# Jackz915/PackPPI

Hardware: AMD Instinct MI355X
Metric: sampled residues/sec at 100 diffusion steps (higher is better)
Workload: dtype f32 (dense layers as split-f16: two f16 per operand, three f16 MFMAs per product, fp32 accumulate); 1 GPU; data/T1124_lig.pdb (L=739, 738 true residues), 1 complex per GPU; diffusion_steps=100, proximal=False, residues_per_gpu=738, residues_rank0=738, residues_total=738, mode=ode

## Files before the change

include/packppi_hip.h:

```cpp
#ifndef PACKPPI_HIP_H
#define PACKPPI_HIP_H

#include <stddef.h>
#include <stdint.h>

#ifdef __cplusplus
extern "C" {
#endif

typedef enum pp_status {
    PP_OK = 0,
    PP_ERR_INVALID = 1,
    PP_ERR_HIP = 2,
    PP_ERR_UNSUPPORTED = 3,
    PP_ERR_NO_DEVICE = 4
} pp_status;

typedef struct pp_plan pp_plan;
typedef struct pp_ctx pp_ctx;

#define PP_N_WEIGHTS 1439172u
#define PP_HIDDEN 128
#define PP_TOP_K 32
#define PP_MODE_ODE 0
// ... 50 lines not shown

pp_status pp_topk_aten_host(const float *values, int n, int k, int32_t *idx_out);

pp_status pp_complex_prepare(pp_plan *plan, const pp_batch *batch, void *stream, pp_ctx **ctx);
void pp_ctx_destroy(pp_ctx *ctx);

pp_status pp_complex_prepare_packed(pp_plan *plan, const pp_batch *batch, const int32_t *seg_offsets, int n_seg,
                                    int min_len, int max_len, void *stream, pp_ctx **ctx);

pp_status pp_ctx_get_graph(pp_ctx *ctx, int64_t *E_idx, float *hE0, void *stream);

pp_status pp_ctx_set_graph(pp_ctx *ctx, const int64_t *E_idx, void *stream);

pp_status pp_score(pp_ctx *ctx, const float *chi, float t, float *score, float *hV, void *stream);

pp_status pp_score_rows(pp_ctx *ctx, const float *chi, const float *t_rows, float *score, float *hV, void *stream);

pp_status pp_sample(pp_ctx *ctx, float *chi, const float *schedule, int n_schedule, int mode,
                    const float *sde_noise, void *stream);

pp_status pp_ctx_set_rng_keys(pp_ctx *ctx, const uint64_t *keys, void *stream);

pp_status pp_noise_seeded(pp_ctx *ctx, uint64_t seed, int step, float *noise, uint32_t *words, void *stream);

pp_status pp_add_noise_seeded(pp_ctx *ctx, const float *chi0, float t, uint64_t seed, float *chi, void *stream);

pp_status pp_sample_seeded(pp_ctx *ctx, float *chi, const float *schedule, int n_schedule, int mode, uint64_t seed,
                           void *stream);

#define PP_FIX_HOLD 0
#define PP_FIX_RENOISE 1
pp_status pp_sample_partial(pp_ctx *ctx, float *chi, const float *chi_ref, const uint8_t *fixed, int fix_mode,
                            const float *schedule, int n_schedule, int mode, uint64_t seed,
                            float *chi_traj , void *stream);

pp_status pp_atom14(pp_ctx *ctx, const float *chi, float *xyz, void *stream);

pp_status pp_clash(pp_ctx *ctx, const float *chi, float *per_res, float *dchi, void *stream);

pp_status pp_proximal(pp_ctx *ctx, const float *chi, float lamda, int num_steps, float *chi_traj,
                      float *chi_last, float *losses, void *stream);

pp_status pp_proximal_packed(pp_ctx *ctx, const float *chi, float lamda, int num_steps, const int32_t *norm_rows,
                             float *chi_traj, float *chi_last, float *chi_accepted, float *losses, void *stream);

pp_status pp_proximal_pinned(pp_ctx *ctx, const float *chi, const uint8_t *fixed , float lamda,
                             int num_steps, const int32_t *norm_rows, float *chi_traj, float *chi_last,
                             float *chi_accepted, float *losses, uint8_t *moved , void *stream);

typedef struct pp_affinity pp_affinity;

#define PP_AFF_N_WEIGHTS 101889u
#define PP_AFF_N_WEIGHTS_LINEAR 33153u

pp_status pp_affinity_create(const float *weights, size_t n_weights, int device, pp_affinity **aff);
void pp_affinity_destroy(pp_affinity *aff);

pp_status pp_affinity_encode(const pp_affinity *aff, pp_ctx *ctx, const int64_t *residue_type, const float *sc_sincos,
                             const int64_t *mut_mask, const float *hV_pret, float *hV, void *stream);

pp_status pp_affinity_predict(const pp_affinity *aff, const float *h_wt, const float *h_mt, const int32_t *seg_offsets,
                              int n_seg, int n_rows, float *ddg, float *ddg_inv, void *stream);

pp_status pp_so2_set_grids(const double *x_grid, const double *sigma_grid, int device);
pp_status pp_so2_score(const float *x, const float *sigma, size_t n, int pi_periodic, float *score, int32_t *idx, int device,
                       void *stream);

pp_status pp_dsm_loss(pp_ctx *ctx, const float *pred_score, const float *target_score, const float *t_rows,
                      const double *score_norm, double *num, double *den, void *stream);

pp_status pp_time_kernel(pp_ctx *ctx, int which, int iters, float *avg_ms, void *stream);

pp_status pp_profile_kernel(pp_ctx *ctx, int which);
pp_status pp_profile_read(pp_ctx *ctx, float *total_ms, int *launches);

int pp_edge_variant(void);

int pp_has_range_check(void);
pp_status pp_range_check(unsigned long long *events, int reset);
pp_status pp_range_check_parts(unsigned long long *edge_events, unsigned long long *node_events, int reset);

pp_status pp_ctx_saturated(pp_ctx *ctx, int *flags, void *stream);

#ifdef PP_DIAG
pp_status pp_debug_edge(pp_ctx *ctx, int layer, void *stream);
pp_status pp_debug_nm(pp_ctx *ctx, int layer, void *stream);
pp_status pp_debug_set_hE(pp_ctx *ctx, const float *src, size_t n);
pp_status pp_debug_buffer(pp_ctx *ctx, int which, float *dst, size_t n);
pp_status pp_debug_score_prefix(pp_ctx *ctx, const float *chi, float t, int n_launches, void *stream);
void pp_debug_set_dbg(float *p);
void pp_debug_set_lds_pad(int bytes);
void pp_debug_set_edge_R(int R);
#endif

#ifdef __cplusplus
}
#endif
#endif
```

packppi_amd/csrc/pp_api.hip:

```cpp
#include <stdio.h>
#include <stdlib.h>

#include <algorithm>
#include <chrono>
#include <cmath>
#include <cstring>
#include <memory>
#include <new>
#include <string>
#include <vector>

#include "pp_internal.h"
#include "pp_pack.h"
#ifdef PP_EDGE_F16
#include "pp_rebalance.h"
#endif
#include "pp_topk_aten.h"

static thread_local std::string g_err;
void pp_set_error(const std::string &msg) { g_err = msg; }

extern "C" const char *pp_last_error(void) { return g_err.c_str(); }
extern "C" int pp_version(void) { return 101; }
#ifndef PP_BUILD_ID
#define PP_BUILD_ID "unstamped-unstamped"
#endif
static const char g_build_id[] = "PP_BUILD_ID=" PP_BUILD_ID;
extern "C" const char *pp_build_id(void) { return g_build_id + 12; }

#define FAIL(code, msg)      \
    do {                     \
        pp_set_error(msg);   \
        return code;         \
    } while (0)

template <typename T>
static pp_status upload(T **dst, const T *src, size_t n) {
    PP_HIP_CHECK(hipMalloc(reinterpret_cast<void **>(dst), n * sizeof(T)));
    PP_HIP_CHECK(hipMemcpy(*dst, src, n * sizeof(T), hipMemcpyHostToDevice));
    return PP_OK;
}

extern "C" int pp_has_range_check(void) {
#ifdef PP_CHECK_RANGE
    return 1;
#else
    return 0;
#endif
}
static pp_status range_check(const char *who, unsigned long long *edge_events, unsigned long long *node_events, int reset) {
#ifdef PP_CHECK_RANGE
    (void)who;
    PP_HIP_CHECK(hipDeviceSynchronize());
    *edge_events = (unsigned long long)pp_edge_range_hits(reset);
    *node_events = (unsigned long long)pp_node_range_hits(reset);
    return PP_OK;
#else
    (void)reset;
    *edge_events = *node_events = 0;
    FAIL(PP_ERR_UNSUPPORTED, std::string(who) + ": this library was built without -DPP_CHECK_RANGE (use libpackppi_hip.chk.so: "
                                                "python -m packppi_amd.rangecheck)");
#endif
}
extern "C" pp_status pp_range_check_parts(unsigned long long *edge_events, unsigned long long *node_events, int reset) {
    if (!edge_events || !node_events) FAIL(PP_ERR_INVALID, "pp_range_check_parts: null argument");
    return range_check("pp_range_check_parts", edge_events, node_events, reset);
}
extern "C" pp_status pp_range_check(unsigned long long *events, int reset) {
    if (!events) FAIL(PP_ERR_INVALID, "pp_range_check: null argument");
    unsigned long long edge = 0, node = 0;
    const pp_status st = range_check("pp_range_check", &edge, &node, reset);
    *events = edge + node;
    return st;
}
__global__ void k_flag_nonfinite(const float *__restrict__ v, int rows, int row_stride, int per_row, const float *__restrict__ rmask,
                                 unsigned *__restrict__ sat) {
    const int i = blockIdx.x * blockDim.x + threadIdx.x;
    if (i >= rows * per_row) return;
    const int r = i / per_row, k = i - r * per_row;
    if (rmask && rmask[r] == 0.f) return;
    const float x = v[(size_t)r * row_stride + k];
    if (!(__builtin_fabsf(x) <= 3.402823466e38f)) atomicOr(sat, 4u);
}
static void flag_nonfinite(pp_ctx *c, const float *v, int row_stride, int per_row, hipStream_t s) {
    const int n = c->N * per_row;
    hipLaunchKernelGGL(k_flag_nonfinite, dim3((n + 255) / 256), dim3(256), 0, s, v, c->N, row_stride, per_row, c->b.residue_mask, c->sat);
}

extern "C" pp_status pp_ctx_saturated(pp_ctx *c, int *flags, void *stream) {
    if (!c || !flags) FAIL(PP_ERR_INVALID, "pp_ctx_saturated: null argument");
    hipStream_t s = static_cast<hipStream_t>(stream);
    unsigned v = 0;
    PP_HIP_CHECK(hipMemcpyAsync(&v, c->sat, sizeof(v), hipMemcpyDeviceToHost, s));
    PP_HIP_CHECK(hipStreamSynchronize(s));
    *flags = (int)v;
    return PP_OK;
}

static void side_chain_extents(const pp_tables *tables, float (&ext)[21]) {
    for (int S = 0; S < 21; S++) {
        float m = 0.f;
        for (int a = 4; a < 14; a++) {
            if (tables->atom14_mask[S * 14 + a] == 0.f) continue;
            const float *lp = tables->lit_positions + (S * 14 + a) * 3;
            float b = std::sqrt(lp[0] * lp[0] + lp[1] * lp[1] + lp[2] * lp[2]);
            const int g = tables->atom14_to_group[S * 14 + a];
            auto tlen = [&](int k) { const float *f = tables->default_frames + ((size_t)S * 8 + k) * 16; return std::sqrt(f[3] * f[3] + f[7] * f[7] + f[11] * f[11]); };
            if (g >= 4) for (int k = 4; k <= g; k++) b += tlen(k);
            else b += tlen(g);
            m = std::max(m, b);
        }
        ext[S] = m * 1.0001f + 1e-3f;
    }
}

struct PlanDeleter { void operator()(pp_plan *p) const { pp_plan_destroy(p); } };
struct CtxDeleter { void operator()(pp_ctx *c) const { pp_ctx_destroy(c); } };

extern "C" pp_status pp_plan_create(const float *weights, size_t n_weights, const pp_tables *tables, int device,
                                    pp_plan **out) {
    if (!tables || !out) FAIL(PP_ERR_INVALID, "pp_plan_create: null argument");
    WeightOff off = pp_weight_offsets();
    const bool has_net = weights != nullptr;
    if (has_net && (n_weights != off.total || off.total != PP_N_WEIGHTS))
        FAIL(PP_ERR_INVALID, "pp_plan_create: expected " + std::to_string(off.total) + " weights, got " +
                                 std::to_string(n_weights));
    if (has_net)
        for (size_t i = 0; i < n_weights; i++)
            if (!(std::fabs(weights[i]) < 65504.f))
                FAIL(PP_ERR_INVALID, "pp_plan_create: weight " + std::to_string(i) + " is not finite or outside the f16 range (" +
                                         std::to_string(weights[i]) + ")");
    int ndev = 0;
    if (hipGetDeviceCount(&ndev) != hipSuccess || ndev <= 0) FAIL(PP_ERR_NO_DEVICE, "pp_plan_create: no HIP device visible");
    if (device < 0 || device >= ndev) FAIL(PP_ERR_INVALID, "pp_plan_create: bad device index");
    PP_HIP_CHECK(hipSetDevice(device));
    hipDeviceProp_t prop;
    PP_HIP_CHECK(hipGetDeviceProperties(&prop, device));
    if (strncmp(prop.gcnArchName, "gfx950", 6) != 0)
        FAIL(PP_ERR_NO_DEVICE, std::string("pp_plan_create: kernels are built for gfx950 only, device is ") + prop.gcnArchName);

    std::unique_ptr<pp_plan, PlanDeleter> p(new (std::nothrow) pp_plan());
    if (!p) FAIL(PP_ERR_INVALID, "out of host memory");
    p->device = device;
    p->off = off;
    p->has_network = has_net;
    p->knn_ties = PP_KNN_TIES_ATEN_CPU;
    p->annealed_temp = 3.0f;
    p->rebalanced_chains = 0;
    pp_status st;
    const float *wpack = weights;
#ifdef PP_EDGE_F16
    std::vector<float> rebalanced, ln_packed;
    if (has_net) {
        LnScales sc;
        p->rebalanced_chains = rewrite_checkpoint(weights, off, rebalanced, ln_packed, sc);
        p->ln_scaled_features = sc.n_scaled;
        for (size_t i = 0; i < off.total; i++)
            if (!(std::fabs(rebalanced[i]) < 65504.f) || !(std::fabs(ln_packed[i]) < 65504.f))
                FAIL(PP_ERR_INVALID, "pp_plan_create: weight " + std::to_string(i) + " leaves the f16 range when its ReLU chain is "
                                     "rebalanced (run this checkpoint on libpackppi_hip.f32.so)");
        weights = rebalanced.data();
        wpack = ln_packed.data();
        if (sc.n_scaled > 0 && (st = upload(&p->ln_scale, &sc.v[0][0], (size_t)5 * 128)) != PP_OK) return st;
    }
#endif
    if (has_net) {
        if ((st = upload(&p->w, weights, off.total)) != PP_OK) return st;
        std::vector<float> arena;
        const PackOff o = pack_network(arena, weights, wpack, off);
        if ((st = upload(&p->wT, arena.data(), arena.size())) != PP_OK) return st;
        const float *wT = p->wT;
        p->node_emb_T = wT + o.node_emb_T;
        p->edge_emb_T = wT + o.edge_emb_T;
        for (int l = 0; l < 3; l++) {
            const LayerPackOff &ol = o.lt[l];
            LayerT &t = p->lt[l];
            t.pts_node_wT = wT + ol.pts_node_wT; t.pts_edge_wT = wT + ol.pts_edge_wT;
            t.nm_A_T = wT + ol.nm_A_T; t.nm_C_T = wT + ol.nm_C_T;
            t.em_A_T = wT + ol.em_A_T; t.em_C_T = wT + ol.em_C_T;
            t.nm_out_T = wT + ol.nm_out_T;
            t.nd_in_T = wT + ol.nd_in_T; t.nd_out_T = wT + ol.nd_out_T;
            t.nm_stream = wT + ol.nm_stream; t.em_stream = wT + ol.em_stream;
            t.em_params = wT + ol.em_params;
            t.nu_stream = wT + ol.nu_stream; t.nu_params = wT + ol.nu_params;
        }
        p->static_stream = wT + o.static_stream;
#ifdef PP_EDGE_F16
        p->embed_stream = wT + o.embed_stream;
#endif
        p->d0_in_T = wT + o.d0_in_T; p->d0_out_T = wT + o.d0_out_T;
        p->d2_in_T = wT + o.d2_in_T; p->d2_out_T = wT + o.d2_out_T;
    }

    if ((st = upload(&p->default_frames, tables->default_frames, 21 * 8 * 16)) != PP_OK) return st;
    if ((st = upload(&p->atom14_to_group, tables->atom14_to_group, 21 * 14)) != PP_OK) return st;
    if ((st = upload(&p->atom14_mask, tables->atom14_mask, 21 * 14)) != PP_OK) return st;
    if ((st = upload(&p->lit_positions, tables->lit_positions, 21 * 14 * 3)) != PP_OK) return st;
    if ((st = upload(&p->between_radius, tables->between_radius, 21 * 14)) != PP_OK) return st;
    float ext[21];
    side_chain_extents(tables, ext);
    if ((st = upload(&p->side_extent, ext, 21)) != PP_OK) return st;
    PP_HIP_CHECK(hipMalloc(reinterpret_cast<void **>(&p->bounds_lower), 21 * 14 * 14 * sizeof(float)));
    PP_HIP_CHECK(hipMalloc(reinterpret_cast<void **>(&p->bounds_upper), 21 * 14 * 14 * sizeof(float)));
    p->clash_params_set = false;
    *out = p.release();
    return PP_OK;
}

extern "C" void pp_plan_destroy(pp_plan *p) {
    if (!p) return;
    void *ptrs[] = {p->w, p->wT, p->default_frames, p->atom14_to_group, p->atom14_mask, p->lit_positions,
                    p->between_radius, p->bounds_lower, p->bounds_upper, p->ln_scale, p->side_extent};
    for (void *q : ptrs) if (q) (void)hipFree(q);
    for (const ArenaSlot &sl : p->arena_pool) {
        (void)hipFree(sl.p);
    }
    delete p;
}

extern "C" pp_status pp_plan_set_knn_ties(pp_plan *p, int mode) {
    if (!p) FAIL(PP_ERR_INVALID, "pp_plan_set_knn_ties: null plan");
    if (mode != PP_KNN_TIES_LOWER_INDEX && mode != PP_KNN_TIES_ATEN_CPU && mode != PP_KNN_TIES_ATEN_MEMBER)
        FAIL(PP_ERR_INVALID, "pp_plan_set_knn_ties: unknown mode " + std::to_string(mode));
    p->knn_ties = mode;
    return PP_OK;
}
// ... 50 lines not shown

extern "C" pp_status pp_plan_set_clash_params(pp_plan *p, float tol, const float *lower, const float *upper, void *stream) {
    if (!p || !lower || !upper) FAIL(PP_ERR_INVALID, "pp_plan_set_clash_params: null argument");
    hipStream_t s = static_cast<hipStream_t>(stream);
    PP_HIP_CHECK(hipStreamSynchronize(s));
    PP_HIP_CHECK(hipMemcpy(p->bounds_lower, lower, 21 * 14 * 14 * sizeof(float), hipMemcpyHostToDevice));
    PP_HIP_CHECK(hipMemcpy(p->bounds_upper, upper, 21 * 14 * 14 * sizeof(float), hipMemcpyHostToDevice));
    p->clash_tol = tol;
    p->clash_params_set = true;
    return PP_OK;
}

extern "C" void pp_ctx_destroy(pp_ctx *c) {
    if (!c) return;
    if (c->arena) {
        pp_plan *p = c->plan;
        std::lock_guard<std::mutex> g(p->pool_mutex);
        if (p->arena_pool.size() < 4) {
            p->arena_pool.push_back({c->arena, c->arena_bytes, c->last_stream});
        } else {
            (void)hipFree(c->arena);
        }
    }
    for (hipEvent_t e : c->prof_ev) (void)hipEventDestroy(e);
    delete c;
}

__global__ void k_seg_uniform(int32_t *__restrict__ off, int n_seg, int L) {
    const int s = blockIdx.x * blockDim.x + threadIdx.x;
    if (s <= n_seg) off[s] = s * L;
}
__global__ void k_fill_seg(int2 *__restrict__ seg, int N, const int32_t *__restrict__ off, int n_seg, int max_len) {
    const int n = blockIdx.x * blockDim.x + threadIdx.x;
    if (n >= N) return;
    int start, len;
    pp_seg_fill(off, n_seg, N, max_len, n, start, len);
    seg[n] = make_int2(start, len);
}

static pp_status prepare_impl(pp_plan *plan, const pp_batch *b, const int32_t *seg_offsets, int n_seg, int min_len,
                              int max_len, void *stream, pp_ctx **out) {
    const bool packed = seg_offsets != nullptr;
    if (!plan || !b || !out) FAIL(PP_ERR_INVALID, "pp_complex_prepare: null argument");
    if (b->B <= 0 || b->L <= 0) FAIL(PP_ERR_INVALID, "pp_complex_prepare: B and L must be positive");
    if ((packed ? max_len : b->L) > 16384) FAIL(PP_ERR_UNSUPPORTED, "pp_complex_prepare: L > 16384 residues per complex is not supported");
    if (packed) {
        if (b->B != 1) FAIL(PP_ERR_INVALID, "pp_complex_prepare_packed: the batch tensors are [1, sum of lengths, ...]");
        if (n_seg < 1 || min_len < 1 || max_len < min_len || (long long)n_seg * min_len > b->L || (long long)n_seg * max_len < b->L)
            FAIL(PP_ERR_INVALID, "pp_complex_prepare_packed: segment count / lengths do not fit the batch");
        if (min_len < PP_TOP_K && min_len != max_len)
            FAIL(PP_ERR_UNSUPPORTED, "pp_complex_prepare_packed: complexes shorter than 32 residues must be prepared on their own");
    }
    if (!b->X || !b->residue_type || !b->BB_D)
        FAIL(PP_ERR_INVALID, "pp_complex_prepare: batch needs at least X, residue_type and BB_D");
    const bool net = plan->has_network;
    if (net && (!b->atom_mask || !b->residue_mask || !b->residue_index || !b->chain_indices || !b->BB_D_sincos ||
                !b->SC_D_mask || !b->chi_1pi_periodic_mask || !b->chi_2pi_periodic_mask))
        FAIL(PP_ERR_INVALID, "pp_complex_prepare: batch has a null tensor pointer");
    PP_HIP_CHECK(hipSetDevice(plan->device));
    std::unique_ptr<pp_ctx, CtxDeleter> owner(new (std::nothrow) pp_ctx());
    if (!owner) FAIL(PP_ERR_INVALID, "out of host memory");
    pp_ctx *c = owner.get();
    c->plan = plan;
    c->b = *b;
    c->packed = packed;
    c->B = packed ? n_seg : b->B;
    c->L = packed ? max_len : b->L;
    c->N = b->B * b->L;
    const int shortest = packed ? min_len : b->L;
    c->K = shortest < PP_TOP_K ? shortest : PP_TOP_K;
    c->shortest = shortest;
    const size_t N = c->N, K = c->K;
    struct Slot { void **p; size_t bytes; };
    std::vector<Slot> slots;
    size_t total = 0;
#define ALLOC(field, n) { const size_t bytes_ = (((n) ? (n) : 1) * sizeof(*c->field) + 255) & ~size_t(255);          \
                          slots.push_back({reinterpret_cast<void **>(&c->field), bytes_}); total += bytes_; }
    if (net) {
        ALLOC(eidx, N * K); ALLOC(mask_att, N * 32); ALLOC(frames, N * 12); ALLOC(bbpos, N * 15);
        ALLOC(hE0, N * K * 128); ALLOC(hE, N * K * 128); ALLOC(Znm, N * K * 128); ALLOC(Zem, N * K * 128); ALLOC(hV, N * 128); ALLOC(hV_alt, N * 128); ALLOC(S, N * 128); ALLOC(msum, N);
        ALLOC(ptsN, N * 48); ALLOC(PAn, N * 128); ALLOC(PCn, N * 128);
        ALLOC(ptsE, N * 48); ALLOC(PAe, N * 128); ALLOC(PCe, N * 128);
        ALLOC(score, N * 4); ALLOC(chi_tmp, N * 4);
    }
    ALLOC(xyz, N * 42); ALLOC(rec, N * 64); ALLOC(axes, N * 24); ALLOC(rec2, N * 64); ALLOC(axes2, N * 24); ALLOC(brad, N); ALLOC(per_res, N); ALLOC(dchi, N * 4);
    ALLOC(px, N * 4); ALLOC(pm, N * 4); ALLOC(pv, N * 4); ALLOC(pz, N * 4); ALLOC(pxeff, N * 4); ALLOC(pmask, N);
    const bool prox = c->B == 1 || packed;
    if (prox) { ALLOC(cand, (size_t)N * 4 * PP_CL_CAP); ALLOC(cand_cnt, N * 4); }
    ALLOC(scal, 64);
    ALLOC(sat, 4);
    ALLOC(seg, N);
    ALLOC(prox_part, (size_t)PP_PROX_CHUNK * N);
    if (prox) { ALLOC(prox_nrows, c->B); ALLOC(prox_seg, c->B); ALLOC(prox_inv, N); }
    ALLOC(seg_off, (size_t)c->B + 1);
    ALLOC(rng_tab, N); ALLOC(rng_keys, c->B);
    c->max_steps = 1 << 20;
#undef ALLOC
    c->last_stream = static_cast<hipStream_t>(stream);
    {
        std::lock_guard<std::mutex> g(plan->pool_mutex);
        int best = -1;
        for (int i = 0; i < (int)plan->arena_pool.size(); i++)
            if (plan->arena_pool[i].bytes >= total && (best < 0 || plan->arena_pool[i].bytes < plan->arena_pool[best].bytes)) best = i;
        if (best >= 0) {
            const ArenaSlot sl = plan->arena_pool[best];
            plan->arena_pool.erase(plan->arena_pool.begin() + best);
            if (sl.stream != c->last_stream) (void)hipStreamSynchronize(sl.stream);
            c->arena = sl.p;
            c->arena_bytes = sl.bytes;
        }
    }
    if (!c->arena && hipMalloc(&c->arena, total) != hipSuccess) {
        c->arena = nullptr;
        FAIL(PP_ERR_HIP, "hipMalloc of the context workspace failed");
    }
    if (!c->arena_bytes) c->arena_bytes = total;
    char *base = static_cast<char *>(c->arena);
    for (const Slot &sl : slots) { *sl.p = base; base += sl.bytes; }
    hipStream_t s_ = static_cast<hipStream_t>(stream);
    if (packed) {
        if (hipMemcpyAsync(c->seg_off, seg_offsets, ((size_t)n_seg + 1) * sizeof(int32_t), hipMemcpyDeviceToDevice, s_) != hipSuccess)
            FAIL(PP_ERR_HIP, "copying the segment offsets failed");
    } else {
        hipLaunchKernelGGL(k_seg_uniform, dim3((c->B + 256) / 256), dim3(256), 0, s_, c->seg_off, c->B, c->L);
    }
    hipLaunchKernelGGL(k_fill_seg, dim3((c->N + 255) / 256), dim3(256), 0, s_, c->seg, c->N, c->seg_off, c->B, c->L);
    if (hipGetLastError() != hipSuccess) FAIL(PP_ERR_HIP, "segment table launch failed");
    if (hipMemsetAsync(c->sat, 0, 4 * sizeof(unsigned), s_) != hipSuccess) FAIL(PP_ERR_HIP, "clearing the saturation word failed");
    if (net) {
        pp_status st;
        flag_nonfinite(c, c->b.X, 42, 12, s_);
        if ((st = pp_launch_prepare(c, s_)) != PP_OK) return st;
        if ((st = pp_launch_edge_static(c, s_)) != PP_OK) return st;
    }
    *out = owner.release();
    return PP_OK;
}

extern "C" pp_status pp_complex_prepare(pp_plan *plan, const pp_batch *b, void *stream, pp_ctx **out) {
    return prepare_impl(plan, b, nullptr, 0, 0, 0, stream, out);
}

extern "C" pp_status pp_complex_prepare_packed(pp_plan *plan, const pp_batch *b, const int32_t *seg_offsets, int n_seg,
                                               int min_len, int max_len, void *stream, pp_ctx **out) {
    if (!seg_offsets) FAIL(PP_ERR_INVALID, "pp_complex_prepare_packed: null segment offsets");
    return prepare_impl(plan, b, seg_offsets, n_seg, min_len, max_len, stream, out);
}

__global__ void k_widen_idx(const int32_t *__restrict__ src, int64_t *__restrict__ dst, size_t n, const int2 *__restrict__ seg, int K) {
    size_t i = (size_t)blockIdx.x * blockDim.x + threadIdx.x;
    if (i < n) {
        size_t node = i / K;
        dst[i] = (int64_t)src[i] - (int64_t)seg[node].x;
    }
}

extern "C" pp_status pp_ctx_get_graph(pp_ctx *c, int64_t *E_idx, float *hE0, void *stream) {
    if (!c) FAIL(PP_ERR_INVALID, "pp_ctx_get_graph: null ctx");
    if (!c->plan->has_network) FAIL(PP_ERR_INVALID, "pp_ctx_get_graph: plan was created without network weights");
    hipStream_t s = static_cast<hipStream_t>(stream);
    size_t n = (size_t)c->N * c->K;
    if (E_idx) hipLaunchKernelGGL(k_widen_idx, dim3((unsigned)((n + 255) / 256)), dim3(256), 0, s, c->eidx, E_idx, n, c->seg, c->K);
    if (hE0) PP_HIP_CHECK(hipMemcpyAsync(hE0, c->hE0, n * 128 * sizeof(float), hipMemcpyDeviceToDevice, s));
    PP_HIP_CHECK(hipGetLastError());
    return PP_OK;
}

extern "C" pp_status pp_ctx_set_graph(pp_ctx *c, const int64_t *E_idx, void *stream) {
    if (c) c->last_stream = static_cast<hipStream_t>(stream);
    if (!c || !E_idx) FAIL(PP_ERR_INVALID, "pp_ctx_set_graph: null argument");
    if (!c->plan->has_network) FAIL(PP_ERR_INVALID, "pp_ctx_set_graph: plan was created without network weights");
    PP_HIP_CHECK(hipSetDevice(c->plan->device));
    hipStream_t s = static_cast<hipStream_t>(stream);
    pp_status st = pp_launch_prepare(c, s, E_idx);
    if (st == PP_OK) st = pp_launch_edge_static(c, s);
    if (st != PP_OK) return st;
    int bad = 0;
    PP_HIP_CHECK(hipMemcpyAsync(&bad, c->scal, sizeof(int), hipMemcpyDeviceToHost, s));
    PP_HIP_CHECK(hipStreamSynchronize(s));
    if (bad) FAIL(PP_ERR_INVALID, "pp_ctx_set_graph: " + std::to_string(bad) + " neighbour indices outside their complex");
    return PP_OK;
}

static float sigma_f32(float t) {
    const double lo = pp_log_sigma_min(), hi = pp_log_sigma_max();
    return expf((float)lo + (float)(hi - lo) * t);
}

static void fill_step(StepParams *sp, float t, float dt, float T) {
    const double PI_D = PP_PI_D, hi = pp_log_sigma_max();
    memset(sp, 0, sizeof(*sp));
    const float ts = t * 10000.0f;
    const float nemb = (float)(-(log(10000.0) / 7.0));
    for (int i = 0; i < 8; i++) {
        float freq = expf((float)i * nemb);
        float arg = ts * freq;
        sp->temb[i] = (float)sin((double)arg);
        sp->temb[8 + i] = (float)cos((double)arg);
    }
    float sigma = sigma_f32(t);
    float g = sigma * (float)sqrt(2.0 * log(PI_D / (0.01 * PI_D)));
    float ratio = sigma / (float)exp(hi);
    float alpha = 1.0f - ratio * ratio;
    sp->w = T != 0.f ? T / (alpha + (1.0f - alpha) * T) : 1.0f;
    sp->c_ode = (0.5f * (g * g)) * dt;
    sp->c_drift = (g * g) * dt;
    sp->c_diff = g * sqrtf(dt);
}

static inline void prof_arm(pp_ctx *c, int which) { c->prof_armed = c->prof_which == which; }
static inline void prof_disarm(pp_ctx *c) { c->prof_armed = false; }
bool pp_prof_take(pp_ctx *c, hipEvent_t *e0, hipEvent_t *e1) {
    c->prof_armed = false;
    while (c->prof_ev.size() < c->prof_n + 2) {
        hipEvent_t e;
        if (hipEventCreate(&e) != hipSuccess) return false;
        c->prof_ev.push_back(e);
    }
    *e0 = c->prof_ev[c->prof_n++];
    *e1 = c->prof_ev[c->prof_n++];
    return true;
}

static pp_status run_network(pp_ctx *c, hipStream_t s, int step, int last_mode, float *chi, int mode, const float *noise,
                             const StepParams *cur, const StepParams *next, const PPRng *rng = nullptr, const PPPin *pin = nullptr) {
    pp_status st;
    for (int l = 0; l < 3; l++) {
        if (l == 0 || !pp_edge_fused()) {
            prof_arm(c, 0);
            st = pp_launch_node_message(c, l, s);
            prof_disarm(c);
            if (st != PP_OK) return st;
        }
        if (l < 2) {
            prof_arm(c, 2);
            st = pp_launch_node_update(c, l, PP_NU_MID, chi, step, mode, noise, nullptr, nullptr, s);
            prof_disarm(c);
            if (st != PP_OK) return st;
            prof_arm(c, 1);
            st = pp_launch_edge_update(c, l, l == 0 || !pp_edge_fused(), s);
            prof_disarm(c);
            if (st != PP_OK) return st;
        } else {
            prof_arm(c, 2);
            st = pp_launch_node_update(c, l, last_mode, chi, step, mode, noise, cur, last_mode == PP_NU_STEP ? next : nullptr, s, rng, pin);
            prof_disarm(c);
            if (st != PP_OK) return st;
        }
    }
    return PP_OK;
}

static pp_status evaluate_and_copy(pp_ctx *c, const StepParams &sp, float *score, float *hV, hipStream_t s) {
    pp_status st;
    if ((st = run_network(c, s, 0, PP_NU_SCORE, nullptr, PP_MODE_ODE, nullptr, &sp, nullptr)) != PP_OK) return st;
    if (score) PP_HIP_CHECK(hipMemcpyAsync(score, c->score, (size_t)c->N * 4 * sizeof(float), hipMemcpyDeviceToDevice, s));
    if (hV) PP_HIP_CHECK(hipMemcpyAsync(hV, c->hV, (size_t)c->N * 128 * sizeof(float), hipMemcpyDeviceToDevice, s));
    return PP_OK;
}

extern "C" pp_status pp_score(pp_ctx *c, const float *chi, float t, float *score, float *hV, void *stream) {
    if (c) c->last_stream = static_cast<hipStream_t>(stream);
    if (!c || !chi || !score) FAIL(PP_ERR_INVALID, "pp_score: null argument");
    if (!c->plan->has_network) FAIL(PP_ERR_INVALID, "pp_score: plan was created without network weights");
    hipStream_t s = static_cast<hipStream_t>(stream);
    PP_HIP_CHECK(hipSetDevice(c->plan->device));
    StepParams sp;
    fill_step(&sp, t, 0.f, c->plan->annealed_temp);
    pp_status st;
    flag_nonfinite(c, chi, 4, 4, s);
    if ((st = pp_launch_node_embed(c, chi, sp, s)) != PP_OK) return st;
    return evaluate_and_copy(c, sp, score, hV, s);
}

extern "C" pp_status pp_score_rows(pp_ctx *c, const float *chi, const float *t_rows, float *score, float *hV, void *stream) {
    if (c) c->last_stream = static_cast<hipStream_t>(stream);
    if (!c || !chi || !t_rows || !score) FAIL(PP_ERR_INVALID, "pp_score_rows: null argument");
    if (!c->plan->has_network) FAIL(PP_ERR_INVALID, "pp_score_rows: plan was created without network weights");
    hipStream_t s = static_cast<hipStream_t>(stream);
    PP_HIP_CHECK(hipSetDevice(c->plan->device));
    StepParams sp;
    fill_step(&sp, 0.f, 0.f, c->plan->annealed_temp);
    pp_status st;
    flag_nonfinite(c, chi, 4, 4, s);
    flag_nonfinite(c, t_rows, 1, 1, s);
    if ((st = pp_launch_node_embed_rows(c, chi, t_rows, s)) != PP_OK) return st;
    return evaluate_and_copy(c, sp, score, hV, s);
}

extern "C" pp_status pp_affinity_encode(const pp_affinity *a, pp_ctx *c, const int64_t *residue_type, const float *sc_sincos,
                                        const int64_t *mut_mask, const float *hV_pret, float *hV, void *stream) {
    if (c) c->last_stream = static_cast<hipStream_t>(stream);
    if (!a || !c || !residue_type || !sc_sincos || !mut_mask || !hV_pret || !hV) FAIL(PP_ERR_INVALID, "pp_affinity_encode: null argument");
    if (!a->network) FAIL(PP_ERR_INVALID, "pp_affinity_encode: the affinity head was created for mode linear (no mutation branch)");
    if (!c->plan->has_network) FAIL(PP_ERR_INVALID, "pp_affinity_encode: plan was created without network weights");
    if (a->device != c->plan->device) FAIL(PP_ERR_INVALID, "pp_affinity_encode: affinity head and ctx are on different devices");
    hipStream_t s = static_cast<hipStream_t>(stream);
    PP_HIP_CHECK(hipSetDevice(c->plan->device));
    StepParams sp;
    fill_step(&sp, 0.f, 0.f, c->plan->annealed_temp);
    pp_status st;
    if ((st = pp_launch_affinity_embed(c, a, residue_type, sc_sincos, mut_mask, hV_pret, s)) != PP_OK) return st;
    return evaluate_and_copy(c, sp, nullptr, hV, s);
}

static pp_status rng_table_ready(pp_ctx *c, hipStream_t s) {
    return c->rng_tab_set ? PP_OK : pp_launch_rng_table(c, false, s);
}

extern "C" pp_status pp_ctx_set_rng_keys(pp_ctx *c, const uint64_t *keys, void *stream) {
    if (c) c->last_stream = static_cast<hipStream_t>(stream);
    if (!c) FAIL(PP_ERR_INVALID, "pp_ctx_set_rng_keys: null ctx");
    hipStream_t s = static_cast<hipStream_t>(stream);
    PP_HIP_CHECK(hipSetDevice(c->plan->device));
    if (keys) PP_HIP_CHECK(hipMemcpyAsync(c->rng_keys, keys, (size_t)c->B * sizeof(uint64_t), hipMemcpyHostToDevice, s));
    return pp_launch_rng_table(c, keys != nullptr, s);
}

extern "C" pp_status pp_noise_seeded(pp_ctx *c, uint64_t seed, int step, float *noise, uint32_t *words, void *stream) {
    if (c) c->last_stream = static_cast<hipStream_t>(stream);
    if (!c || !noise) FAIL(PP_ERR_INVALID, "pp_noise_seeded: null argument");
    if (step < -1 || step >= c->max_steps) FAIL(PP_ERR_INVALID, "pp_noise_seeded: step must be -1 (initial noising) .. 2^20 - 1");
    hipStream_t s = static_cast<hipStream_t>(stream);
    PP_HIP_CHECK(hipSetDevice(c->plan->device));
    pp_status st;
    if ((st = rng_table_ready(c, s)) != PP_OK) return st;
    return pp_launch_noise_seeded(c, seed, step, noise, words, s);
}

extern "C" pp_status pp_add_noise_seeded(pp_ctx *c, const float *chi0, float t, uint64_t seed, float *chi, void *stream) {
    if (c) c->last_stream = static_cast<hipStream_t>(stream);
    if (!c || !chi0 || !chi) FAIL(PP_ERR_INVALID, "pp_add_noise_seeded: null argument");
    if (!c->b.chi_1pi_periodic_mask || !c->b.chi_2pi_periodic_mask) FAIL(PP_ERR_INVALID, "pp_add_noise_seeded: batch lacks the periodic masks");
    hipStream_t s = static_cast<hipStream_t>(stream);
    PP_HIP_CHECK(hipSetDevice(c->plan->device));
    pp_status st;
    if ((st = rng_table_ready(c, s)) != PP_OK) return st;
    return pp_launch_add_noise_seeded(c, chi0, sigma_f32(t), seed, chi, s);
}

struct PartialArgs {
    const float *chi_ref;
    const uint8_t *fixed;
    int fix_mode;
    float *chi_traj;
};

static pp_status sample_impl(const char *who, pp_ctx *c, float *chi, const float *schedule, int n_schedule, int mode,
                             const float *sde_noise, const PPRng *rng, hipStream_t s, const PartialArgs *part = nullptr);

extern "C" pp_status pp_sample(pp_ctx *c, float *chi, const float *schedule, int n_schedule, int mode,
                               const float *sde_noise, void *stream) {
    if (c) c->last_stream = static_cast<hipStream_t>(stream);
    if (c && mode == PP_MODE_SDE && !sde_noise) FAIL(PP_ERR_INVALID, "pp_sample: sde mode needs the per-step noise tensor");
    return sample_impl("pp_sample", c, chi, schedule, n_schedule, mode, sde_noise, nullptr, static_cast<hipStream_t>(stream));
}

extern "C" pp_status pp_sample_seeded(pp_ctx *c, float *chi, const float *schedule, int n_schedule, int mode, uint64_t seed,
                                      void *stream) {
    if (c) c->last_stream = static_cast<hipStream_t>(stream);
    hipStream_t s = static_cast<hipStream_t>(stream);
    if (!c || mode != PP_MODE_SDE)
        return sample_impl("pp_sample_seeded", c, chi, schedule, n_schedule, mode, nullptr, nullptr, s);
    PP_HIP_CHECK(hipSetDevice(c->plan->device));
    pp_status st;
    if ((st = rng_table_ready(c, s)) != PP_OK) return st;
    const PPRng rng = {c->rng_tab, (uint32_t)seed, (uint32_t)(seed >> 32)};
    return sample_impl("pp_sample_seeded", c, chi, schedule, n_schedule, mode, nullptr, &rng, s);
}

extern "C" pp_status pp_sample_partial(pp_ctx *c, float *chi, const float *chi_ref, const uint8_t *fixed, int fix_mode,
                                       const float *schedule, int n_schedule, int mode, uint64_t seed, float *chi_traj,
                                       void *stream) {
    if (c) c->last_stream = static_cast<hipStream_t>(stream);
    hipStream_t s = static_cast<hipStream_t>(stream);
    if (!c || !chi || !chi_ref || !fixed || !schedule) FAIL(PP_ERR_INVALID, "pp_sample_partial: null argument");
    if (chi_ref == chi) FAIL(PP_ERR_INVALID, "pp_sample_partial: chi_ref and chi must be distinct buffers");
    if (fix_mode != PP_FIX_HOLD && fix_mode != PP_FIX_RENOISE) FAIL(PP_ERR_INVALID, "pp_sample_partial: unknown fix_mode");
    if (mode != PP_MODE_ODE && mode != PP_MODE_SDE) FAIL(PP_ERR_INVALID, "pp_sample_partial: unknown mode");
    if (!c->b.chi_1pi_periodic_mask || !c->b.chi_2pi_periodic_mask) FAIL(PP_ERR_INVALID, "pp_sample_partial: batch lacks the periodic masks");
    PP_HIP_CHECK(hipSetDevice(c->plan->device));
    pp_status st;
    if ((st = rng_table_ready(c, s)) != PP_OK) return st;
    const PPRng rng = {c->rng_tab, (uint32_t)seed, (uint32_t)(seed >> 32)};
    const PartialArgs part = {chi_ref, fixed, fix_mode, chi_traj};
    return sample_impl("pp_sample_partial", c, chi, schedule, n_schedule, mode, nullptr, &rng, s, &part);
}

static pp_status sample_impl(const char *who, pp_ctx *c, float *chi, const float *schedule, int n_schedule, int mode,
                             const float *sde_noise, const PPRng *rng, hipStream_t s, const PartialArgs *part) {
    const std::string w(who);
    if (!c || !chi || !schedule) FAIL(PP_ERR_INVALID, w + ": null argument");
    if (!c->plan->has_network) FAIL(PP_ERR_INVALID, w + ": plan was created without network weights");
    if (n_schedule < 2) FAIL(PP_ERR_INVALID, w + ": schedule needs at least 2 times");
    if (n_schedule - 1 > c->max_steps) FAIL(PP_ERR_UNSUPPORTED, w + ": more than 2^20 steps");
    if (mode != PP_MODE_ODE && mode != PP_MODE_SDE) FAIL(PP_ERR_INVALID, w + ": unknown mode");
    PP_HIP_CHECK(hipSetDevice(c->plan->device));
    const int nsteps = n_schedule - 1;
    std::vector<StepParams> steps((size_t)nsteps);
    for (int j = 0; j < nsteps; j++) fill_step(&steps[j], schedule[j], schedule[j] - schedule[j + 1], c->plan->annealed_temp);
    pp_status st;
    flag_nonfinite(c, chi, 4, 4, s);
    if ((st = pp_launch_node_embed(c, chi, steps[0], s)) != PP_OK) return st;
    static const bool dbg = PP_GETENV("PP_DEBUG") != nullptr;
    const auto h0 = std::chrono::steady_clock::now();
    for (int j = 0; j < nsteps; j++) {
        PPPin pin = {nullptr, nullptr, nullptr, 0.f, 0};
        if (part) {
            pin.fixed = part->fixed;
            pin.chi_ref = part->chi_ref;
            pin.traj = part->chi_traj ? part->chi_traj + (size_t)j * c->N * 4 : nullptr;
            pin.sigma = sigma_f32(schedule[j + 1]);
            pin.renoise = part->fix_mode == PP_FIX_RENOISE && j + 1 < nsteps ? 1 : 0;
        }
        if ((st = run_network(c, s, j, PP_NU_STEP, chi, mode, sde_noise, &steps[j], j + 1 < nsteps ? &steps[j + 1] : nullptr, rng,
                              part ? &pin : nullptr)) != PP_OK) return st;
    }
    if (dbg) {
        const double us = std::chrono::duration<double, std::micro>(std::chrono::steady_clock::now() - h0).count();
        fprintf(stderr, "[pp] pp_sample: host enqueue of %d steps took %.0f us (%.1f us per step)\n", nsteps, us, us / nsteps);
    }
    return PP_OK;
}

extern "C" pp_status pp_atom14(pp_ctx *c, const float *chi, float *xyz, void *stream) {
    if (c) c->last_stream = static_cast<hipStream_t>(stream);
    if (!c || !chi || !xyz) FAIL(PP_ERR_INVALID, "pp_atom14: null argument");
    PP_HIP_CHECK(hipSetDevice(c->plan->device));
    return pp_launch_atom14(c, chi, xyz, static_cast<hipStream_t>(stream));
}

extern "C" pp_status pp_clash(pp_ctx *c, const float *chi, float *per_res, float *dchi, void *stream) {
    if (c) c->last_stream = static_cast<hipStream_t>(stream);
    if (!c || !chi || !per_res) FAIL(PP_ERR_INVALID, "pp_clash: null argument");
    if (!c->plan->clash_params_set) FAIL(PP_ERR_INVALID, "pp_clash: call pp_plan_set_clash_params first");
    if (!c->b.atom_mask || !c->b.residue_index) FAIL(PP_ERR_INVALID, "pp_clash: batch lacks atom_mask / residue_index");
    PP_HIP_CHECK(hipSetDevice(c->plan->device));
    hipStream_t s = static_cast<hipStream_t>(stream);
    pp_status st;
    if ((st = pp_launch_atom14(c, chi, c->xyz, s)) != PP_OK) return st;
    return pp_launch_clash(c, c->xyz, per_res, dchi, s);
}

extern "C" pp_status pp_proximal(pp_ctx *c, const float *chi, float lamda, int num_steps, float *chi_traj,
                                 float *chi_last, float *losses, void *stream) {
    if (c) c->last_stream = static_cast<hipStream_t>(stream);
    if (!c || !chi || !losses) FAIL(PP_ERR_INVALID, "pp_proximal: null argument");
    if (c->B != 1) FAIL(PP_ERR_INVALID, "pp_proximal: batch.num_proteins must be 1 (optimize.py:27); optimise the complexes of a packed or padded batch one by one");
    if (num_steps < 1) FAIL(PP_ERR_INVALID, "pp_proximal: num_steps must be >= 1");
    if (!c->plan->clash_params_set) FAIL(PP_ERR_INVALID, "pp_proximal: call pp_plan_set_clash_params first");
    if (!c->b.atom_mask || !c->b.residue_index) FAIL(PP_ERR_INVALID, "pp_proximal: batch lacks atom_mask / residue_index");
    PP_HIP_CHECK(hipSetDevice(c->plan->device));
    return pp_launch_proximal(c, chi, lamda, num_steps, chi_traj, chi_last, losses, static_cast<hipStream_t>(stream));
}

static pp_status proximal_packed_impl(const char *who, pp_ctx *c, const float *chi, const uint8_t *fixed, float lamda, int num_steps,
                                      const int32_t *norm_rows, float *chi_traj, float *chi_last, float *chi_accepted, float *losses,
                                      uint8_t *moved, void *stream) {
    const std::string w(who);
    if (!c->packed && c->B != 1)
        FAIL(PP_ERR_INVALID, w + ": needs a context from pp_complex_prepare_packed (or a B = 1 one), not a padded B > 1 batch");
    if (num_steps < 1) FAIL(PP_ERR_INVALID, w + ": num_steps must be >= 1");
    if (!c->plan->clash_params_set) FAIL(PP_ERR_INVALID, w + ": call pp_plan_set_clash_params first");
    if (!c->b.atom_mask || !c->b.residue_index) FAIL(PP_ERR_INVALID, w + ": batch lacks atom_mask / residue_index");
    const int shortest = c->shortest;
    if (norm_rows)
        for (int s = 0; s < c->B; s++)
            if (norm_rows[s] < shortest)
                FAIL(PP_ERR_INVALID, w + ": norm_rows[" + std::to_string(s) + "] = " + std::to_string(norm_rows[s]) +
                                         " is below the shortest complex (" + std::to_string(shortest) + " rows)");
    PP_HIP_CHECK(hipSetDevice(c->plan->device));
    hipStream_t s = static_cast<hipStream_t>(stream);
    if (norm_rows) PP_HIP_CHECK(hipMemcpyAsync(c->prox_nrows, norm_rows, (size_t)c->B * sizeof(int32_t), hipMemcpyHostToDevice, s));
    return pp_launch_proximal_packed(c, chi, lamda, num_steps, norm_rows != nullptr, chi_traj, chi_last, chi_accepted, losses, s, fixed,
                                     moved);
}

extern "C" pp_status pp_proximal_packed(pp_ctx *c, const float *chi, float lamda, int num_steps, const int32_t *norm_rows,
                                        float *chi_traj, float *chi_last, float *chi_accepted, float *losses, void *stream) {
    if (c) c->last_stream = static_cast<hipStream_t>(stream);
    if (!c || !chi || !chi_last || !chi_accepted || !losses) FAIL(PP_ERR_INVALID, "pp_proximal_packed: null argument");
    return proximal_packed_impl("pp_proximal_packed", c, chi, nullptr, lamda, num_steps, norm_rows, chi_traj, chi_last, chi_accepted,
                                losses, nullptr, stream);
}

extern "C" pp_status pp_proximal_pinned(pp_ctx *c, const float *chi, const uint8_t *fixed, float lamda, int num_steps,
                                        const int32_t *norm_rows, float *chi_traj, float *chi_last, float *chi_accepted,
                                        float *losses, uint8_t *moved, void *stream) {
    if (c) c->last_stream = static_cast<hipStream_t>(stream);
    if (!c || !chi || !fixed || !chi_last || !chi_accepted || !losses) FAIL(PP_ERR_INVALID, "pp_proximal_pinned: null argument");
    return proximal_packed_impl("pp_proximal_pinned", c, chi, fixed, lamda, num_steps, norm_rows, chi_traj, chi_last, chi_accepted,
                                losses, moved, stream);
}

extern "C" pp_status pp_time_kernel(pp_ctx *c, int which, int iters, float *avg_ms, void *stream) {
    if (!c || !avg_ms || iters < 1) FAIL(PP_ERR_INVALID, "pp_time_kernel: bad argument");
    if (!c->plan->has_network) FAIL(PP_ERR_INVALID, "pp_time_kernel: plan was created without network weights");
    hipStream_t s = static_cast<hipStream_t>(stream);
    PP_HIP_CHECK(hipSetDevice(c->plan->device));
// ... 95 lines not shown
```

packppi_amd/csrc/pp_edge.hip:

```cpp
#include "pp_internal.h"

unsigned int pp_edge_range_hits(int) { return 0; }

#include "pp_edge_tile.h"

#define ET 256
#define CH32 (128 * 32)
#define XBUF_FLOATS (4 * 4 * 64 * 4)
#define PARAM_FLOATS 1152

#define MFMA(a, b, c) __builtin_amdgcn_mfma_f32_32x32x2f32((a), (b), (c), 0, 0, 0)

struct EdgeArgs {
    int N, K;
    float inv_K;
    const float *rmask;
    const int32_t *eidx;
    const float *mask_att;
    const float *frames;
    const float *pts;
    const float *PA, *PC;
    const float *hE_in;
    float *hE_out;
    float *S, *msum;
    const float *wstream;
    const float *params;
    const float *g3, *be3;
    const float *b_mid;
    const float *Z;
    const float *pts2, *PA2, *PC2, *b_mid2;
    float *Znm, *Zem;
};
enum { P_BMID = 0, P_BOUT = 128, P_FOB = 256, P_G2 = 384, P_BE2 = 512, P_FIB = 640 };

__device__ __forceinline__ void dma_chunk(const float *sbase, unsigned &laneoff, unsigned lds_dst) {
    asm volatile("s_waitcnt lgkmcnt(0)\n\t"
                 "s_mov_b32 m0, %2\n\t"
                 "s_mov_b64 s[98:99], %1\n\ts_nop 0\n\t"
                 "global_load_lds_dwordx4 %0, s[98:99]\n\t"
                 "global_load_lds_dwordx4 %0, s[98:99] offset:1024\n\t"
                 "global_load_lds_dwordx4 %0, s[98:99] offset:2048\n\t"
                 "global_load_lds_dwordx4 %0, s[98:99] offset:3072"
                 : "+v"(laneoff) : "s"(sbase), "s"(lds_dst) : "memory", "s98", "s99");
}
__device__ __forceinline__ void dma_tile(const float *sbase, unsigned &rowoff, unsigned lds_dst) {
    asm volatile("s_waitcnt lgkmcnt(0)\n\t"
                 "s_mov_b32 m0, %2\n\t"
                 "s_mov_b64 s[90:91], %1\n\t"
                 "s_sub_u32 s92, s90, 992\n\ts_subb_u32 s93, s91, 0\n\t"
                 "s_sub_u32 s94, s90, 1984\n\ts_subb_u32 s95, s91, 0\n\t"
                 "s_sub_u32 s96, s90, 2976\n\ts_subb_u32 s97, s91, 0\n\ts_nop 0\n\t"
                 "global_load_lds_dwordx4 %0, s[90:91]\n\t"
                 "global_load_lds_dwordx4 %0, s[92:93] offset:1024\n\t"
                 "global_load_lds_dwordx4 %0, s[94:95] offset:2048\n\t"
                 "global_load_lds_dwordx4 %0, s[96:97] offset:3072"
                 : "+v"(rowoff) : "s"(sbase), "s"(lds_dst)
                 : "memory", "scc", "s90", "s91", "s92", "s93", "s94", "s95", "s96", "s97");
}
template <int N>
__device__ __forceinline__ void wait_vm(unsigned laneoff, unsigned rowoff) {
    asm volatile("s_waitcnt vmcnt(%0)" ::"n"(N), "v"(laneoff), "v"(rowoff) : "memory");
}

template <bool SWAP>
__device__ __forceinline__ void mfma_tile32(const float *wslot, const f32x16 &x, f32x16 &acc, int lane) {
#pragma unroll
    for (int q = 0; q < 4; q++) {
        f32x4v a = *reinterpret_cast<const f32x4v *>(wslot + (q * 64 + lane) * 4);
#pragma unroll
        for (int p = 0; p < 4; p++) {
            if (SWAP) acc = MFMA(x[4 * q + p], a[p], acc);
            else acc = MFMA(a[p], x[4 * q + p], acc);
        }
    }
}

__device__ __forceinline__ void mfma_tile24(const float *wslot, const float (&g)[12], f32x16 &acc, int lane) {
#pragma unroll
    for (int q = 0; q < 3; q++) {
        f32x4v a = *reinterpret_cast<const f32x4v *>(wslot + (q * 64 + lane) * 4);
#pragma unroll
        for (int p = 0; p < 4; p++) acc = MFMA(a[p], g[4 * q + p], acc);
    }
}

__device__ __forceinline__ void edge_geometry(const float *__restrict__ pts_i, const float *__restrict__ fr,
                                              const float *__restrict__ pts_j, int h, float (&g)[3][12]) {
    float geom[72];
    float R[9], tr[3];
#pragma unroll
    for (int k = 0; k < 9; k++) R[k] = fr[k];
#pragma unroll
    for (int k = 0; k < 3; k++) tr[k] = fr[9 + k];
#pragma unroll
    for (int q = 0; q < 8; q++) {
        float lx = pts_i[3 * q], ly = pts_i[3 * q + 1], lz = pts_i[3 * q + 2];
        float gx = pts_i[24 + 3 * q], gy = pts_i[24 + 3 * q + 1], gz = pts_i[24 + 3 * q + 2];
        float jx = pts_j[24 + 3 * q], jy = pts_j[24 + 3 * q + 1], jz = pts_j[24 + 3 * q + 2];
        geom[3 * q] = lx; geom[3 * q + 1] = ly; geom[3 * q + 2] = lz;
// ... 59 lines not shown
__global__ void __launch_bounds__(ET, 3)
k_node_message(EdgeArgs A) {
    extern __shared__ __attribute__((aligned(16))) float smem[];
    float *xbuf = smem + 4 * S * 1024;
    const int tid = threadIdx.x, lane = tid & 63;
    const int wave = __builtin_amdgcn_readfirstlane(tid >> 6);
    const int j = lane & 31, h = lane >> 5;
    const int n = blockIdx.x;
    const int K = A.K;
    if (A.rmask[n] == 0.f) {
        if (tid < 128) A.S[(size_t)n * 128 + tid] = 0.f;
        if (tid == 0) A.msum[n] = 0.f;
        return;
    }
    constexpr int C0 = ST0 ? 0 : 4;
    constexpr int NCH = C0 + 7;
    PROLOGUE_PIPE()

    f32x16 x[4], acc;
    float g[3][12];
    const int jj = j < K ? j : K - 1;
    const int nbr = A.eidx[(size_t)n * K + jj];
    const float bmid = A.b_mid[32 * wave + j];
    float m16[16];
    {
        const float *mrow = A.mask_att + (size_t)n * 32;
#pragma unroll
        for (int q = 0; q < 4; q++) {
            f32x4v mm = *reinterpret_cast<const f32x4v *>(mrow + 8 * q + 4 * h);
            m16[4 * q] = mm[0]; m16[4 * q + 1] = mm[1]; m16[4 * q + 2] = mm[2]; m16[4 * q + 3] = mm[3];
        }
    }
    edge_geometry(A.pts + (size_t)n * 48, A.frames + (size_t)n * 12, A.pts + (size_t)nbr * 48, h, g);
    {
        const float *hrow = A.hE_in + ((size_t)n * K + jj) * 128;
        if constexpr (!ST0) {
#pragma unroll
            for (int t = 0; t < 4; t++) load_tile(hrow + 32 * t, h, x[t]);
        }
        load_tile(A.PA + (size_t)n * 128 + 32 * wave, h, acc);
        add_tile(A.PC + (size_t)nbr * 128 + 32 * wave, h, acc);
        if constexpr (ST0) add_tile(A.Z + ((size_t)n * K + jj) * 128 + 32 * wave, h, acc);
    }
    FIRST_LAYER(NCH)
    {
#pragma unroll
        for (int t = 0; t < 4; t++) xbuf_get(xbuf, t, lane, x[t]);
#pragma unroll
        for (int r = 0; r < 16; r++) acc[r] = bmid;
    }
    WSTAGE(C0 + 3, NCH, mfma_tile32<true>(wslot, x[0], acc, lane))
    WSTAGE(C0 + 4, NCH, mfma_tile32<true>(wslot, x[1], acc, lane))
    WSTAGE(C0 + 5, NCH, mfma_tile32<true>(wslot, x[2], acc, lane))
    WSTAGE(C0 + 6, NCH, mfma_tile32<true>(wslot, x[3], acc, lane))
    {
        float s = 0.f, ms = 0.f;
#pragma unroll
        for (int r = 0; r < 16; r++) {
            s = fmaf(fmaxf(acc[r], 0.f), m16[r], s);
            ms += m16[r];
        }
        s += __shfl_xor(s, 32);
        ms += __shfl_xor(ms, 32);
        if (h == 0) A.S[(size_t)n * 128 + 32 * wave + j] = s * A.inv_K;
        if (tid == 0) A.msum[n] = ms * A.inv_K;
    }
}

#define FFN_BLOCK(c)                                                                                         \
    load_tile(prm + P_FIB + 128 * (c) + 32 * wave, h, acc);                                                  \
    WSTAGE(C0 + 11 + 8 * (c) + 0, NCH, mfma_tile32<false>(wslot, x[0], acc, lane))                                \
    WSTAGE(C0 + 11 + 8 * (c) + 1, NCH, mfma_tile32<false>(wslot, x[1], acc, lane))                                \
    WSTAGE(C0 + 11 + 8 * (c) + 2, NCH, mfma_tile32<false>(wslot, x[2], acc, lane))                                \
    WSTAGE(C0 + 11 + 8 * (c) + 3, NCH, mfma_tile32<false>(wslot, x[3], acc, lane))                                \
    relu_tile(acc);                                                                                          \
    __syncthreads();                                  \
    xbuf_put(xbuf, wave, lane, acc);                                                                         \
    __syncthreads();                                                                                         \
    WSTAGE(C0 + 11 + 8 * (c) + 4, NCH, xbuf_get(xbuf, 0, lane, acc); mfma_tile32<false>(wslot, acc, out, lane))   \
    WSTAGE(C0 + 11 + 8 * (c) + 5, NCH, xbuf_get(xbuf, 1, lane, acc); mfma_tile32<false>(wslot, acc, out, lane))   \
    WSTAGE(C0 + 11 + 8 * (c) + 6, NCH, xbuf_get(xbuf, 2, lane, acc); mfma_tile32<false>(wslot, acc, out, lane))   \
    WSTAGE(C0 + 11 + 8 * (c) + 7, NCH, xbuf_get(xbuf, 3, lane, acc); mfma_tile32<false>(wslot, acc, out, lane))

template <int S, bool ST0, bool FUSE, bool WB = true>
__global__ void __launch_bounds__(ET, PP_EU_WGS)
k_edge_update(EdgeArgs A) {
    extern __shared__ __attribute__((aligned(16))) float smem[];
    float *xbuf = smem + 4 * S * 1024, *prm = xbuf + XBUF_FLOATS;
    const int tid = threadIdx.x, lane = tid & 63;
    const int wave = __builtin_amdgcn_readfirstlane(tid >> 6);
    const int j = lane & 31, h = lane >> 5;
    const int n = blockIdx.x;
    const int K = A.K;
    const int jj = j < K ? j : K - 1;
    if (A.rmask[n] == 0.f) {
        if (WB && j < K) {
            f32x4v z = {0.f, 0.f, 0.f, 0.f};
            float *orow = A.hE_out + ((size_t)n * K + j) * 128 + 32 * wave;
#pragma unroll
            for (int q = 0; q < 4; q++) *reinterpret_cast<f32x4v *>(orow + 8 * q + 4 * h) = z;
        }
        if constexpr (FUSE) {
            if (tid < 128) A.S[(size_t)n * 128 + tid] = 0.f;
            if (tid == 0) A.msum[n] = 0.f;
        }
        return;
    }
    constexpr int C0 = ST0 ? 0 : 4;
    constexpr int NEU = C0 + 43;
    constexpr int NCH = NEU + (FUSE ? 11 : 0);
    PROLOGUE_PIPE()

    f32x16 x[4], acc, out;
    float g[3][12];
    const float *hrow = A.hE_in + ((size_t)n * K + jj) * 128;
    const int nbr = A.eidx[(size_t)n * K + jj];
    const float me = A.mask_att[(size_t)n * 32 + jj];
#pragma unroll
    for (int it = 0; it < (PARAM_FLOATS / 4 + ET - 1) / ET; it++) {
        const int i = min(tid + it * ET, PARAM_FLOATS / 4 - 1);
        *reinterpret_cast<f32x4v *>(prm + 4 * i) = *reinterpret_cast<const f32x4v *>(A.params + 4 * i);
    }
    edge_geometry(A.pts + (size_t)n * 48, A.frames + (size_t)n * 12, A.pts + (size_t)nbr * 48, h, g);
    __builtin_amdgcn_sched_barrier(0);
    {
        if constexpr (!ST0) {
#pragma unroll
            for (int t = 0; t < 4; t++) load_tile(hrow + 32 * t, h, x[t]);
        }
        load_tile(A.PA + (size_t)n * 128 + 32 * wave, h, acc);
        add_tile(A.PC + (size_t)nbr * 128 + 32 * wave, h, acc);
        if constexpr (ST0) add_tile(A.Z + ((size_t)n * K + jj) * 128 + 32 * wave, h, acc);
    }
    FIRST_LAYER(NCH)
    {
#pragma unroll
        for (int t = 0; t < 4; t++) xbuf_get(xbuf, t, lane, x[t]);
        load_tile(prm + P_BMID + 32 * wave, h, acc);
    }
    WSTAGE(C0 + 3, NCH, mfma_tile32<false>(wslot, x[0], acc, lane))
    WSTAGE(C0 + 4, NCH, mfma_tile32<false>(wslot, x[1], acc, lane))
    WSTAGE(C0 + 5, NCH, mfma_tile32<false>(wslot, x[2], acc, lane))
    WSTAGE(C0 + 6, NCH, mfma_tile32<false>(wslot, x[3], acc, lane))
    relu_tile(acc);
    __syncthreads();
    xbuf_put(xbuf, wave, lane, acc);
    __syncthreads();
    {
#pragma unroll
        for (int t = 0; t < 4; t++) xbuf_get(xbuf, t, lane, x[t]);
        load_tile(prm + P_BOUT + 32 * wave, h, acc);
    }
    __syncthreads();
    rowoff = (unsigned)((((size_t)n * K + jj) * 128 + 32 * wave + 4 * h) * sizeof(float));
    dma_tile(A.hE_in, rowoff, (unsigned)(size_t)(xbuf + wave * 1024));
    WSTAGE(C0 + 7, NCH, mfma_tile32<false>(wslot, x[0], acc, lane))
    WSTAGE(C0 + 8, NCH, mfma_tile32<false>(wslot, x[1], acc, lane))
    WSTAGE(C0 + 9, NCH, mfma_tile32<false>(wslot, x[2], acc, lane))
    WSTAGE(C0 + 10, NCH, mfma_tile32<false>(wslot, x[3], acc, lane))
    xbuf_get(xbuf, wave, lane, out);
#pragma unroll
    for (int r = 0; r < 16; r++) out[r] = fmaf(acc[r], me, out[r]);
    xbuf_put(xbuf, wave, lane, out);
    __syncthreads();
    {
#pragma unroll
        for (int t = 0; t < 4; t++) xbuf_get(xbuf, t, lane, x[t]);
        float mean;
        float rstd = ln_center(x, mean);
#pragma unroll
        for (int t = 0; t < 4; t++) {
            if (t == 0) asm volatile("" : "+v"(rstd) : : "memory");
            else asm volatile("" : "+v"(x[t > 0 ? t - 1 : 0][15]) : : "memory");
            ln_affine_tile(x[t], rstd, prm + P_G2 + 32 * t, prm + P_BE2 + 32 * t, h);
        }
        load_tile(prm + P_FOB + 32 * wave, h, out);
    }
    FFN_BLOCK(0)
// ... 61 lines not shown
                sacc = fmaf(fmaxf(acc[4 * q + pq], 0.f), mm[pq], sacc);
                ms += mm[pq];
            }
        }
        sacc += __shfl_xor(sacc, 32);
        ms += __shfl_xor(ms, 32);
        if (h == 0) A.S[(size_t)n * 128 + 32 * wave + j] = sacc * A.inv_K;
        if (tid == 0) A.msum[n] = ms * A.inv_K;
    }
}

template <int S>
__global__ void __launch_bounds__(ET, 3)
k_edge_static(EdgeArgs A) {
    extern __shared__ __attribute__((aligned(16))) float smem[];
    const int tid = threadIdx.x, lane = tid & 63;
    const int wave = __builtin_amdgcn_readfirstlane(tid >> 6);
    const int j = lane & 31, h = lane >> 5;
    const int n = blockIdx.x;
    const int K = A.K;
    if (A.rmask[n] == 0.f) return;
    constexpr int NCH = 8;
    PROLOGUE_PIPE()
    f32x16 x[4], acc;
    const int jj = j < K ? j : K - 1;
    const float *hrow = A.hE_in + ((size_t)n * K + jj) * 128;
#pragma unroll
    for (int t = 0; t < 4; t++) load_tile(hrow + 32 * t, h, x[t]);
#pragma unroll
    for (int r = 0; r < 16; r++) acc[r] = 0.f;
    WSTAGE(0, NCH, mfma_tile32<false>(wslot, x[0], acc, lane))
    WSTAGE(1, NCH, mfma_tile32<false>(wslot, x[1], acc, lane))
    WSTAGE(2, NCH, mfma_tile32<false>(wslot, x[2], acc, lane))
    WSTAGE(3, NCH, mfma_tile32<false>(wslot, x[3], acc, lane))
    store_tile(A.Znm + ((size_t)n * K + jj) * 128 + 32 * wave, h, acc);
#pragma unroll
    for (int r = 0; r < 16; r++) acc[r] = 0.f;
    WSTAGE(4, NCH, mfma_tile32<false>(wslot, x[0], acc, lane))
    WSTAGE(5, NCH, mfma_tile32<false>(wslot, x[1], acc, lane))
    WSTAGE(6, NCH, mfma_tile32<false>(wslot, x[2], acc, lane))
    WSTAGE(7, NCH, mfma_tile32<false>(wslot, x[3], acc, lane))
    store_tile(A.Zem + ((size_t)n * K + jj) * 128 + 32 * wave, h, acc);
}

static EdgeArgs edge_args(pp_ctx *c, int layer, bool edge) {
    const pp_plan *p = c->plan;
    const LayerOff &o = p->off.layer[layer];
    EdgeArgs A;
    A.N = c->N; A.K = c->K; A.inv_K = 1.0f / (float)c->K;
    A.rmask = c->b.residue_mask;
    A.eidx = c->eidx; A.mask_att = c->mask_att; A.frames = c->frames;
    A.pts = edge ? c->ptsE : c->ptsN;
    A.PA = edge ? c->PAe : c->PAn;
    A.PC = edge ? c->PCe : c->PCn;
    A.hE_in = layer == 0 ? c->hE0 : c->hE;
    A.hE_out = c->hE;
    A.S = c->S; A.msum = c->msum;
    A.wstream = edge ? p->lt[layer].em_stream : p->lt[layer].nm_stream;
    A.params = p->lt[layer].em_params;
    A.g3 = p->w + o.norm_g[3]; A.be3 = p->w + o.norm_b[3];
    A.b_mid = p->w + o.nm_mid_b;
    A.Z = edge ? c->Zem : c->Znm;
    A.Znm = c->Znm; A.Zem = c->Zem;
    A.pts2 = c->ptsN; A.PA2 = c->PAn; A.PC2 = c->PCn;
    A.b_mid2 = p->w + p->off.layer[layer < 2 ? layer + 1 : 2].nm_mid_b;
    return A;
}

static const size_t NM_SMEM = (4 * PP_NM_SLOTS * 1024 + XBUF_FLOATS) * sizeof(float);
static const size_t EU_SMEM = (4 * PP_EU_SLOTS * 1024 + XBUF_FLOATS + PARAM_FLOATS) * sizeof(float);
static const size_t ST_SMEM = (4 * 2 * 1024) * sizeof(float);

static bool edge_attrs() {
    static bool done = false, ok = false;
    if (!done) {
        done = true;
        auto set = [](const void *f, size_t bytes) {
            return hipFuncSetAttribute(f, hipFuncAttributeMaxDynamicSharedMemorySize, (int)bytes) == hipSuccess;
        };
        ok = set(reinterpret_cast<const void *>(k_node_message<PP_NM_SLOTS, false>), NM_SMEM) &&
             set(reinterpret_cast<const void *>(k_node_message<PP_NM_SLOTS, true>), NM_SMEM) &&
             set(reinterpret_cast<const void *>(k_edge_update<PP_EU_SLOTS, false, true>), EU_SMEM) &&
             set(reinterpret_cast<const void *>(k_edge_update<PP_EU_SLOTS, true, true>), EU_SMEM) &&
             set(reinterpret_cast<const void *>(k_edge_update<PP_EU_SLOTS, false, true, false>), EU_SMEM);
    }
    return ok;
}

void pp_edge_occupancy(int *node_msg, int *edge_upd) {
    edge_attrs();
    (void)hipOccupancyMaxActiveBlocksPerMultiprocessor(node_msg, reinterpret_cast<const void *>(k_node_message<PP_NM_SLOTS, false>), ET, NM_SMEM);
    (void)hipOccupancyMaxActiveBlocksPerMultiprocessor(edge_upd, reinterpret_cast<const void *>(k_edge_update<PP_EU_SLOTS, false, true>), ET, EU_SMEM);
}

#define EDGE_ATTR_CHECK()                                                                                   \
    if (!edge_attrs()) {                                                                                    \
        pp_set_error("hipFuncSetAttribute(MaxDynamicSharedMemorySize) failed for the edge kernels");        \
        return PP_ERR_HIP;                                                                                  \
    }

extern "C" int pp_edge_variant(void) { return 0; }
bool pp_edge_fused() { return true; }

pp_status pp_launch_edge_static(pp_ctx *c, hipStream_t s) {
    EDGE_ATTR_CHECK()
    EdgeArgs A = edge_args(c, 0, false);
    A.wstream = c->plan->static_stream;
    hipLaunchKernelGGL(k_edge_static<2>, dim3(c->N), dim3(ET), ST_SMEM, s, A);
    PP_HIP_CHECK(hipGetLastError());
    return PP_OK;
}

pp_status pp_launch_node_message(pp_ctx *c, int layer, hipStream_t s) {
    EDGE_ATTR_CHECK()
    EdgeArgs A = edge_args(c, layer, false);
    if (layer == 0) PP_LAUNCH(c, (k_node_message<PP_NM_SLOTS, true>), dim3(c->N), dim3(ET), NM_SMEM, s, A);
    else PP_LAUNCH(c, (k_node_message<PP_NM_SLOTS, false>), dim3(c->N), dim3(ET), NM_SMEM, s, A);
    PP_HIP_CHECK(hipGetLastError());
    return PP_OK;
}

pp_status pp_launch_edge_update(pp_ctx *c, int layer, bool keep_hE, hipStream_t s) {
    EDGE_ATTR_CHECK()
    if (layer < 0 || layer > 1) { pp_set_error("pp_launch_edge_update: layer must be 0 or 1"); return PP_ERR_INVALID; }
    EdgeArgs A = edge_args(c, layer, true);
    if (layer == 0) PP_LAUNCH(c, (k_edge_update<PP_EU_SLOTS, true, true>), dim3(c->N), dim3(ET), EU_SMEM, s, A);
    else if (keep_hE) PP_LAUNCH(c, (k_edge_update<PP_EU_SLOTS, false, true>), dim3(c->N), dim3(ET), EU_SMEM, s, A);
    else PP_LAUNCH(c, (k_edge_update<PP_EU_SLOTS, false, true, false>), dim3(c->N), dim3(ET), EU_SMEM, s, A);
    PP_HIP_CHECK(hipGetLastError());
    return PP_OK;
}
```

packppi_amd/csrc/pp_edge_f16.hip:

```cpp
#include "pp_internal.h"

PP_RANGE_COUNTER
PP_RANGE_READER(pp_edge_range_hits)

#include "pp_edge_tile.h"
typedef _Float16 h8 __attribute__((ext_vector_type(8)));

struct HT {
    h8 hi[2], lo[2];
};
typedef float f32x2v __attribute__((ext_vector_type(2)));
typedef _Float16 h2v __attribute__((ext_vector_type(2)));
typedef __fp16 fp16x2_t __attribute__((ext_vector_type(2)));
__device__ __forceinline__ h2v cvt2(f32x2v x) {
    const fp16x2_t r = __builtin_amdgcn_cvt_pkrtz(x[0], x[1]);
    return __builtin_bit_cast(h2v, r);
}
__device__ __forceinline__ f32x2v split_residual(h2v hh, f32x2v x) {
    const unsigned hp = __builtin_bit_cast(unsigned, hh);
    float d0, d1;
    asm("v_fma_mix_f32 %0, %1, -1.0, %2 op_sel_hi:[1,0,0]" : "=v"(d0) : "v"(hp), "v"(x[0]));
    asm("v_fma_mix_f32 %0, %1, -1.0, %2 op_sel:[1,0,0] op_sel_hi:[1,0,0]" : "=v"(d1) : "v"(hp), "v"(x[1]));
    return f32x2v{d0, d1};
}
typedef unsigned short us2v __attribute__((ext_vector_type(2)));
template <bool RELU>
__device__ __forceinline__ void split_tile(const f32x16 &v, HT &o, unsigned &sat) {
#pragma unroll
    for (int s = 0; s < 2; s++)
#pragma unroll
        for (int i = 0; i < 8; i += 2) {
            f32x2v x = {v[8 * s + i], v[8 * s + i + 1]};
            PP_RANGE(RELU ? fmaxf(x[0], 0.f) : x[0]) PP_RANGE(RELU ? fmaxf(x[1], 0.f) : x[1])
            if (RELU) {
                x[0] = __builtin_amdgcn_fmed3f(x[0], 0.f, 65504.f);
                x[1] = __builtin_amdgcn_fmed3f(x[1], 0.f, 65504.f);
            }
            const h2v hh = cvt2(x);
#ifndef PP_X_NOSAT
            if (RELU)
#else
            if (false)
#endif
                sat = __builtin_bit_cast(unsigned, __builtin_elementwise_max(__builtin_bit_cast(us2v, sat), __builtin_bit_cast(us2v, hh)));
            const f32x2v d = split_residual(hh, x);
            const h2v ll = cvt2(d);
            o.hi[s][i] = hh[0]; o.hi[s][i + 1] = hh[1];
            o.lo[s][i] = ll[0]; o.lo[s][i + 1] = ll[1];
        }
}
__device__ __forceinline__ void join_tile(const HT &t, f32x16 &v) {
#pragma unroll
    for (int s = 0; s < 2; s++)
#pragma unroll
        for (int i = 0; i < 8; i++) v[8 * s + i] = (float)t.hi[s][i] + (float)t.lo[s][i];
}

#define ET 256
#define CH32 (128 * 32)
#define XBUF_FLOATS (4 * 4 * 64 * 4)
#define PARAM_FLOATS 1152
#define PARAM_LDS 640

#define MFMA(a, b, c) __builtin_amdgcn_mfma_f32_32x32x2f32((a), (b), (c), 0, 0, 0)

struct EdgeArgs {
    int N, K;
    float inv_K;
    const float *rmask;
    const int32_t *eidx;
    const float *mask_att;
    const float *frames;
    const float *pts;
    const float *PA, *PC;
    const float *hE_in;
    float *hE_out;
    float *S, *msum;
    const float *wstream;
    const float *params;
    const float *g3, *be3;
    const float *b_mid;
    const float *Z;
    const float *pts2, *PA2, *PC2, *b_mid2;
    float *Znm, *Zem;
    const float *ls_in, *ls_x1, *ls_out;
    unsigned *sat;
    float *dbg;
    int n_pairs;
    int mix_mode;
};
enum { P_BMID = 0, P_BOUT = 128, P_FOB = 256, P_G2 = 384, P_BE2 = 512, P_FIB = 640 };

#ifndef PP_WDEPTH
#define PP_WDEPTH 2
#endif
#ifndef PP_WDEPTH_R1
#define PP_WDEPTH_R1 2
#endif
#define WDEPTH_ (R == 1 ? PP_WDEPTH_R1 : PP_WDEPTH)
#if defined(PP_X_TS) && defined(PP_X_TS_FINE)
#define TSF(k) if constexpr ((k) >= PP_X_TS_FINE && (k) < PP_X_TS_FINE + 16) tsf[(k) - PP_X_TS_FINE] = (int)(__builtin_readcyclecounter() - ts0f);
#else
#define TSF(k)
#endif
#ifndef PP_WGS2
#define PP_WGS2 2
#endif
#ifndef PP_WGS
#define PP_WGS 3
#endif
#define NRING (WDEPTH_ + 1)
#ifdef PP_X_NOWLOAD
#define PP_X_NOWLOAD_ true
#else
#define PP_X_NOWLOAD_ false
#endif

#ifdef PP_X_E_NOMFMA
#define MFMA16(a, b, c) (c)
#else
#define MFMA16(a, b, c) __builtin_amdgcn_mfma_f32_32x32x16_f16((a), (b), (c), 0, 0, 0)
#endif

struct AOp {
    h8 r[4];
};
__device__ __forceinline__ void gload_A(const h8 *__restrict__ wq, int chunk, AOp &a) {
    int off = chunk * 1024;
    asm volatile("" : "+s"(off));
    const h8 *p = wq + off;
    a.r[0] = p[0]; a.r[1] = p[64]; a.r[2] = p[128]; a.r[3] = p[192];
}
template <int R, int T, bool SWAP>
__device__ __forceinline__ void mfma_x(const AOp &a, const HT (&x)[R][4], f32x16 (&acc)[R]) {
#pragma unroll
    for (int s = 0; s < 2; s++) {
        if (SWAP) {
#pragma unroll
            for (int r = 0; r < R; r++) acc[r] = MFMA16(x[r][T].hi[s], a.r[2 * s], acc[r]);
#pragma unroll
            for (int r = 0; r < R; r++) acc[r] = MFMA16(x[r][T].lo[s], a.r[2 * s], acc[r]);
#pragma unroll
            for (int r = 0; r < R; r++) acc[r] = MFMA16(x[r][T].hi[s], a.r[2 * s + 1], acc[r]);
        } else {
#pragma unroll
            for (int r = 0; r < R; r++) acc[r] = MFMA16(a.r[2 * s], x[r][T].hi[s], acc[r]);
#pragma unroll
            for (int r = 0; r < R; r++) acc[r] = MFMA16(a.r[2 * s], x[r][T].lo[s], acc[r]);
#pragma unroll
            for (int r = 0; r < R; r++) acc[r] = MFMA16(a.r[2 * s + 1], x[r][T].hi[s], acc[r]);
        }
    }
// ... 111 lines not shown
    h8 vh, vl;
    h2v dh, dl;
#pragma unroll
    for (int i = 0; i < 10; i += 2) {
        const f32x2v x = {v[i], v[i + 1]};
        PP_RANGE(x[0]) PP_RANGE(x[1])
        const h2v hh = cvt2(x);
        const f32x2v d = split_residual(hh, x);
        const h2v ll = cvt2(d);
        if (i < 8) { vh[i] = hh[0]; vh[i + 1] = hh[1]; vl[i] = ll[0]; vl[i + 1] = ll[1]; }
        else { dh = hh; dl = ll; }
    }
    h8 *gv = reinterpret_cast<h8 *>(gbuf);
    gv[(2 * q) * 64 + lane] = vh;
    gv[(2 * q + 1) * 64 + lane] = vl;
    _Float16 *gh = reinterpret_cast<_Float16 *>(gbuf);
    gh[((2 * 4) * 64 + lane) * 8 + q] = dh[0];
    gh[((2 * 4 + 1) * 64 + lane) * 8 + q] = dl[0];
    if (wave == 0) {
        const f32x2v z = {0.f, 0.f};
        *reinterpret_cast<f32x2v *>(gh + ((2 * 4) * 64 + lane) * 8 + 4) = z;
        *reinterpret_cast<f32x2v *>(gh + ((2 * 4 + 1) * 64 + lane) * 8 + 4) = z;
    }
}

#define WSTAGE(k, NCH, ACC, BODY)                                                                              \
    {                                                                                                          \
        __builtin_amdgcn_sched_barrier(0);                                                                     \
        if constexpr ((k) + WDEPTH_ < (NCH) && !PP_X_NOWLOAD_)                                                 \
            gload_A(wq, (k) + WDEPTH_, AR[((k) + WDEPTH_) % NRING]);                                           \
        const AOp &AK = AR[(k) % NRING];                                                                       \
        BODY;                                                                                                  \
        _Pragma("unroll") for (int r_ = 0; r_ < R; r_++) asm volatile("" ::"v"(ACC[r_][0]));                   \
        TSF(k)                                                                                                 \
    }

#define ROT(p) ((wave + (p)) & 3)
#define BT_FETCH(BUF, t, set)                                                     \
    _Pragma("unroll") for (int r = 0; r < R; r++) xbuf_get_h((BUF) + r * XBUF_FLOATS, t, lane, bt[set][r]);
#define ACC_FENCE(ACC) _Pragma("unroll") for (int r_ = 0; r_ < R; r_++) asm volatile("" ::"v"(ACC[r_][0]));
#define RSTAGE(k, NCH, ACC, BUF, P, SWAP, BAR, FETCH_LATE)                                                  \
    WSTAGE(k, NCH, ACC, {                                                                                   \
        if constexpr ((P) < 3 && !(FETCH_LATE)) { BT_FETCH(BUF, ROT((P) + 1), ((P) + 1) & 1) }   \
        (mfma_hs<R, SWAP, 0>(AK, bt[(P) & 1], ACC));                                                        \
        if constexpr (BAR) { ACC_FENCE(ACC) __syncthreads(); }                                              \
        if constexpr ((P) < 3 && (FETCH_LATE)) { BT_FETCH(BUF, ROT((P) + 1), ((P) + 1) & 1) }    \
        (mfma_hs<R, SWAP, 1>(AK, bt[(P) & 1], ACC));                                                        \
    })
#define RLAYER_OWN(k0, NCH, ACC, BUF, SWAP, BAR_A)                                \
    RSTAGE((k0) + 0, NCH, ACC, BUF, 0, SWAP, true, true)                          \
    RSTAGE((k0) + 1, NCH, ACC, BUF, 1, SWAP, false, false)                        \
    RSTAGE((k0) + 2, NCH, ACC, BUF, 2, SWAP, false, false)                        \
    RSTAGE((k0) + 3, NCH, ACC, BUF, 3, SWAP, BAR_A, false)
#define RLAYER_BUF(k0, NCH, ACC, BUF, SWAP, BAR_A)                                \
    BT_FETCH(BUF, ROT(0), 0)                                                      \
    RSTAGE((k0) + 0, NCH, ACC, BUF, 0, SWAP, false, false)                        \
    RSTAGE((k0) + 1, NCH, ACC, BUF, 1, SWAP, false, false)                        \
    RSTAGE((k0) + 2, NCH, ACC, BUF, 2, SWAP, false, false)                        \
    RSTAGE((k0) + 3, NCH, ACC, BUF, 3, SWAP, BAR_A, false)
#define PUBLISH_OWN(RELU, SRC, BUF)                                               \
    _Pragma("unroll") for (int r = 0; r < R; r++) {                               \
        split_tile<RELU>(SRC[r], bt[0][r], sat);                                  \
        xbuf_put_h((BUF) + r * XBUF_FLOATS, wave, lane, bt[0][r]);                \
    }

#define FIRST_LAYER(K0, NCH)                                                      \
    if constexpr (!ST0) {                                                         \
        RLAYER_OWN((K0) + 0, NCH, acc, xbuf, false, false)                        \
    }                                                                             \
    WSTAGE((K0) + C0 + 0, NCH, acc, (mfma_geo<R, 0>(AK, gbuf, lane, acc)))        \
    WSTAGE((K0) + C0 + 1, NCH, acc, (mfma_geo<R, 1>(AK, gbuf, lane, acc)))        \
    if constexpr (!ST0) { __syncthreads(); }                                      \
    WSTAGE((K0) + C0 + 2, NCH, acc, (mfma_geo<R, 2>(AK, gbuf, lane, acc)))        \
    PUBLISH_OWN(true, acc, xbuf)

#define PROLOGUE_PIPE(NCH)                                                                                     \
    const h8 *wq = reinterpret_cast<const h8 *>(A.wstream) + wave * 256 + lane;     \
    AOp AR[NRING];                                                                                             \
    _Pragma("unroll") for (int pk = 0; pk < WDEPTH_ && pk < (NCH); pk++) gload_A(wq, pk, AR[pk]);

#define GROUP_SETUP()                                                                          \
    int n[R];                                                                                  \
    bool live[R], inr[R];                                                                      \
    float rm_[R];                                                                              \
    int first = -1;                                                                            \
    _Pragma("unroll") for (int r = 0; r < R; r++) {                                            \
        const int nr = res0 + r;                                                               \
        inr[r] = nr < A.N;                                                                     \
        n[r] = inr[r] ? nr : A.N - 1;                                                          \
        rm_[r] = A.rmask[n[r]];                                                                \
    }                                                                                          \
    _Pragma("unroll") for (int r = 0; r < R; r++) {                                            \
        live[r] = inr[r] && rm_[r] != 0.f;                                                     \
        if (live[r] && first < 0) first = n[r];                                                \
    }

__device__ __forceinline__ void ln_partial(const f32x16 &v, float *st, int wave, int j, int h) {
    float s = 0.f;
#pragma unroll
    for (int q = 0; q < 16; q++) s += v[q];
    s += __shfl_xor(s, 32);
    const float m = s * (1.f / 32.f);
    float q2 = 0.f;
#pragma unroll
    for (int q = 0; q < 16; q++) {
        const float d = v[q] - m;
        q2 = fmaf(d, d, q2);
    }
    q2 += __shfl_xor(q2, 32);
    if (h == 0) {
        f32x2v o = {m, q2};
        *reinterpret_cast<f32x2v *>(st + (wave * 32 + j) * 2) = o;
    }
}
__device__ __forceinline__ float ln_merge(const float *st, int j, float &mean_out) {
    f32x2v p[4];
#pragma unroll
    for (int w = 0; w < 4; w++) p[w] = *reinterpret_cast<const f32x2v *>(st + (w * 32 + j) * 2);
    const float mean = 0.25f * ((p[0][0] + p[1][0]) + (p[2][0] + p[3][0]));
    float m2 = (p[0][1] + p[1][1]) + (p[2][1] + p[3][1]);
#pragma unroll
    for (int w = 0; w < 4; w++) {
        const float d = p[w][0] - mean;
        m2 = fmaf(32.f * d, d, m2);
    }
    mean_out = mean;
    return 1.f / sqrtf(m2 * (1.f / 128.f) + 1e-5f);
}
#define STAT_FLOATS 256

template <int R, bool ST0>
__device__ __forceinline__ void node_message_body(const EdgeArgs &A, const int res0, float *smem) {
    float *const xbuf = smem;
    const int tid = threadIdx.x, lane = tid & 63;
    const int wave = __builtin_amdgcn_readfirstlane(tid >> 6);
    const int j = lane & 31, h = lane >> 5;
    const int K = A.K;
    unsigned sat = 0;
    GROUP_SETUP()
#pragma unroll
    for (int r = 0; r < R; r++)
        if (inr[r] && !live[r]) {
            if (tid < 128) A.S[(size_t)n[r] * 128 + tid] = 0.f;
            if (tid == 0) A.msum[n[r]] = 0.f;
        }
    if (first < 0) return;
#pragma unroll
    for (int r = 0; r < R; r++)
        if (!live[r]) n[r] = first;
    constexpr int C0 = ST0 ? 0 : 4;
    constexpr int NCH = C0 + 7;
#if defined(PP_X_TS) && defined(PP_X_TS_FINE)
    const unsigned long long ts0f = __builtin_readcyclecounter();
    int tsf[16] = {0};
#endif
    HT bt[2][R];
    f32x16 acc[R];
    float *gbuf = smem + R * XBUF_FLOATS;
    const int jj = j < K ? j : K - 1;
    int nbr[R];
#pragma unroll
    for (int r = 0; r < R; r++) nbr[r] = A.eidx[(size_t)n[r] * K + jj];
    GeoI gi0[R];
    float pj[R][3];
    f32x16 hin[R];
#pragma unroll
    for (int r = 0; r < R; r++) {
        geo_load_i(A.pts + (size_t)n[r] * 48, A.frames + (size_t)n[r] * 12, h, wave, gi0[r]);
        if constexpr (!ST0) load_tile(A.hE_in + ((size_t)n[r] * K + jj) * 128 + 32 * wave, h, hin[r]);
    }
    const float bmid = A.b_mid[32 * wave + j];
    PROLOGUE_PIPE(NCH)
    TileQ pc[R], zt[R];
#pragma unroll
    for (int r = 0; r < R; r++) {
        geo_load_j(A.pts + (size_t)nbr[r] * 48, h, wave, pj[r]);
        load_tile(A.PA + (size_t)n[r] * 128 + 32 * wave, h, acc[r]);
        load_tile_q(A.PC + (size_t)nbr[r] * 128 + 32 * wave, h, pc[r]);
        if constexpr (ST0) load_tile_q(A.Z + ((size_t)n[r] * K + jj) * 128 + 32 * wave, h, zt[r]);
    }
    if constexpr (!ST0) { PUBLISH_OWN(false, hin, xbuf) }
#pragma unroll
    for (int r = 0; r < R; r++) {
        geometry_put(gi0[r], pj[r], wave, lane, gbuf + r * GBUF_FLOATS);
        add_tile_q(pc[r], acc[r]);
        if constexpr (ST0) add_tile_q(zt[r], acc[r]);
    }
    if constexpr (ST0) __syncthreads();
    FIRST_LAYER(0, NCH)
    f32x4v mmv[R][4];
#pragma unroll
    for (int r = 0; r < R; r++) {
        const float *mrow = A.mask_att + (size_t)n[r] * 32 + 4 * h;
#pragma unroll
        for (int q = 0; q < 4; q++) mmv[r][q] = *reinterpret_cast<const f32x4v *>(mrow + 8 * q);
    }
#pragma unroll
    for (int r = 0; r < R; r++)
#pragma unroll
        for (int q = 0; q < 16; q++) acc[r][q] = bmid;
    RLAYER_OWN(C0 + 3, NCH, acc, xbuf, true, false)
#pragma unroll
    for (int r = 0; r < R; r++) {
        float s = 0.f, ms = 0.f;
#pragma unroll
        for (int q = 0; q < 4; q++) {
            const f32x4v mm = mmv[r][q];
#pragma unroll
            for (int pq = 0; pq < 4; pq++) {
                s = fmaf(fmaxf(acc[r][4 * q + pq], 0.f), mm[pq], s);
                ms += mm[pq];
            }
        }
        s += __shfl_xor(s, 32);
        ms += __shfl_xor(ms, 32);
        if (live[r]) {
            if (h == 0) A.S[(size_t)n[r] * 128 + 32 * wave + j] = s * A.inv_K;
            if (tid == 0) A.msum[n[r]] = ms * A.inv_K;
        }
    }
    if (pp_sat_hit(sat)) atomicOr(A.sat, 1u);
}

#ifndef PP_NM_WGS2
#define PP_NM_WGS2 3
#endif
template <int R, bool ST0>
__global__ void __launch_bounds__(ET, R == 1 ? PP_WGS : PP_NM_WGS2)
k_node_message(EdgeArgs A) {
    extern __shared__ __attribute__((aligned(16))) float smem[];
    node_message_body<R, ST0>(A, blockIdx.x * R, smem);
}

#define FFN_BIAS_FETCH(c) load_tile(A.params + P_FIB + 128 * (c) + 32 * wave, h, fib);
#define FFN_BLOCK(c)                                                                                         \
    _Pragma("unroll") for (int r = 0; r < R; r++) acc[r] = fib;                                              \
    if constexpr ((c) == 0) { RLAYER_OWN(C0 + 11 + 8 * (c), NCH, acc, x1buf, false, false) }                 \
    else { RLAYER_BUF(C0 + 11 + 8 * (c), NCH, acc, x1buf, false, true) }                                     \
    PUBLISH_OWN(true, acc, xbuf)                                                                             \
    if constexpr ((c) < 3) { FFN_BIAS_FETCH((c) + 1) }                                                       \
    RLAYER_OWN(C0 + 11 + 8 * (c) + 4, NCH, out, xbuf, false, false)

#ifdef PP_X_TS
#define TS(i) { tsv[i] = (int)(__builtin_readcyclecounter() - ts0); }
#else
#define TS(i)
#endif
template <int R, bool ST0, bool FUSE, bool LNS = false, bool WB = true>
__device__ __forceinline__ void edge_update_body(const EdgeArgs &A, const int res0, float *smem) {
    float *const xbuf = smem, *const x1buf = smem + R * XBUF_FLOATS, *const stat = x1buf + R * XBUF_FLOATS,
                 *const prm = stat + R * STAT_FLOATS;
    const int tid = threadIdx.x, lane = tid & 63;
    const int wave = __builtin_amdgcn_readfirstlane(tid >> 6);
    const int j = lane & 31, h = lane >> 5;
    const int K = A.K;
    const int jj = j < K ? j : K - 1;
    unsigned sat = 0;
    GROUP_SETUP()
#pragma unroll
    for (int r = 0; r < R; r++)
        if (inr[r] && !live[r]) {
            if (WB && j < K) {
                f32x4v z = {0.f, 0.f, 0.f, 0.f};
                float *orow = A.hE_out + ((size_t)n[r] * K + j) * 128 + 32 * wave;
#pragma unroll
                for (int q = 0; q < 4; q++) *reinterpret_cast<f32x4v *>(orow + 8 * q + 4 * h) = z;
            }
            if constexpr (FUSE) {
                if (tid < 128) A.S[(size_t)n[r] * 128 + tid] = 0.f;
                if (tid == 0) A.msum[n[r]] = 0.f;
            }
        }
    if (first < 0) return;
#pragma unroll
    for (int r = 0; r < R; r++)
        if (!live[r]) n[r] = first;
    constexpr int C0 = ST0 ? 0 : 4;
    constexpr int NEU = C0 + 43;
    constexpr int NCH = NEU + (FUSE ? 11 : 0);
#ifdef PP_X_TS
    const unsigned long long ts0 = __builtin_readcyclecounter();
    int tsv[24];
#endif
#if defined(PP_X_TS) && defined(PP_X_TS_FINE)
    const unsigned long long ts0f = __builtin_readcyclecounter();
    int tsf[16] = {0};
#endif
    HT bt[2][R];
    f32x16 acc[R], out[R];
    float *gbuf = x1buf;
    int nbr[R];
    float me[R];
    GeoI gi0[R];
    float pj[R][3];
#pragma unroll
    for (int r = 0; r < R; r++) {
        nbr[r] = A.eidx[(size_t)n[r] * K + jj];
        me[r] = A.mask_att[(size_t)n[r] * 32 + jj];
    }
    constexpr int PRM_IT = (PARAM_LDS / 4 + ET - 1) / ET;
    f32x4v prv[PRM_IT], prg;
#pragma unroll
    for (int it = 0; it < PRM_IT; it++) prv[it] = *reinterpret_cast<const f32x4v *>(A.params + 4 * min(tid + it * ET, PARAM_LDS / 4 - 1));
    {
        const int t64 = min(tid, 63);
        prg = *reinterpret_cast<const f32x4v *>((t64 < 32 ? A.g3 + 4 * t64 : A.be3 + 4 * (t64 - 32)));
    }
#pragma unroll
    for (int r = 0; r < R; r++) {
        geo_load_i(A.pts + (size_t)n[r] * 48, A.frames + (size_t)n[r] * 12, h, wave, gi0[r]);
        load_tile(A.hE_in + ((size_t)n[r] * K + jj) * 128 + 32 * wave, h, out[r]);
    }
    PROLOGUE_PIPE(NCH)
#pragma unroll
    for (int r = 0; r < R; r++) geo_load_j(A.pts + (size_t)nbr[r] * 48, h, wave, pj[r]);
    TileQ pc[R], zt[R];
#pragma unroll
    for (int r = 0; r < R; r++) {
        load_tile(A.PA + (size_t)n[r] * 128 + 32 * wave, h, acc[r]);
        load_tile_q(A.PC + (size_t)nbr[r] * 128 + 32 * wave, h, pc[r]);
        if constexpr (ST0) load_tile_q(A.Z + ((size_t)n[r] * K + jj) * 128 + 32 * wave, h, zt[r]);
    }
#pragma unroll
    for (int it = 0; it < PRM_IT; it++) *reinterpret_cast<f32x4v *>(prm + 4 * min(tid + it * ET, PARAM_LDS / 4 - 1)) = prv[it];
    if (tid < 64) *reinterpret_cast<f32x4v *>(prm + PARAM_LDS + 4 * tid) = prg;
#pragma unroll
    for (int r = 0; r < R; r++) geometry_put(gi0[r], pj[r], wave, lane, gbuf + r * GBUF_FLOATS);
    if constexpr (!ST0) { PUBLISH_OPERAND(out, xbuf, A.ls_in) }
#pragma unroll
    for (int r = 0; r < R; r++) {
        add_tile_q(pc[r], acc[r]);
        if constexpr (ST0) add_tile_q(zt[r], acc[r]);
    }
    if constexpr (ST0) __syncthreads();
    TS(0)
    FIRST_LAYER(0, NCH)
    TS(1)
#pragma unroll
    for (int r = 0; r < R; r++) load_tile(prm + P_BMID + 32 * wave, h, acc[r]);
    RLAYER_OWN(C0 + 3, NCH, acc, xbuf, false, true)
    TS(2)
    PUBLISH_OWN(true, acc, xbuf)
    TS(3)
#pragma unroll
// ... 42 lines not shown
        for (int q = 0; q < 16; q++) out[r][q] -= mean3;
        ln_affine_tile(out[r], rstd, prm + PARAM_LDS + 32 * wave, prm + PARAM_LDS + 128 + 32 * wave, h);
#pragma unroll
        for (int q = 0; q < 16; q++) out[r][q] *= me[r];
        if (WB && live[r]) store_tile(A.hE_out + ((size_t)n[r] * K + jj) * 128 + 32 * wave, h, out[r]);
    }
    TS(12)
    if constexpr (FUSE) {
        GeoI gi_[R];
        float pj2[R][3];
#pragma unroll
        for (int r = 0; r < R; r++) {
            asm volatile("" : "+v"(nbr[r]));
            geo_load_i(A.pts2 + (size_t)n[r] * 48, A.frames + (size_t)n[r] * 12, h, wave, gi_[r]);
            geo_load_j(A.pts2 + (size_t)nbr[r] * 48, h, wave, pj2[r]);
            load_tile(A.PA2 + (size_t)n[r] * 128 + 32 * wave, h, acc[r]);
        }
        __builtin_amdgcn_sched_barrier(0);
        PUBLISH_OPERAND(out, xbuf, A.ls_out)
        __builtin_amdgcn_sched_barrier(0);
        TileQ pc2[R];
#pragma unroll
        for (int r = 0; r < R; r++) load_tile_q(A.PC2 + (size_t)nbr[r] * 128 + 32 * wave, h, pc2[r]);
#pragma unroll
        for (int r = 0; r < R; r++) geometry_put(gi_[r], pj2[r], wave, lane, gbuf + r * GBUF_FLOATS);
        const float bmid = A.b_mid2[32 * wave + j];
        TS(13)
        RLAYER_OWN(NEU + 0, NCH, acc, xbuf, false, false)
        WSTAGE(NEU + 4, NCH, acc, (mfma_geo<R, 0>(AK, gbuf, lane, acc)))
        WSTAGE(NEU + 5, NCH, acc, (mfma_geo<R, 1>(AK, gbuf, lane, acc)))
        __syncthreads();
        WSTAGE(NEU + 6, NCH, acc, (mfma_geo<R, 2>(AK, gbuf, lane, acc)))
#pragma unroll
        for (int r = 0; r < R; r++) add_tile_q(pc2[r], acc[r]);
        TS(14)
        PUBLISH_OWN(true, acc, xbuf)
        f32x4v mmv[R][4];
#pragma unroll
        for (int r = 0; r < R; r++) {
            const float *mrow = A.mask_att + (size_t)n[r] * 32 + 4 * h;
#pragma unroll
            for (int q = 0; q < 4; q++) mmv[r][q] = *reinterpret_cast<const f32x4v *>(mrow + 8 * q);
        }
#pragma unroll
        for (int r = 0; r < R; r++)
#pragma unroll
            for (int q = 0; q < 16; q++) acc[r][q] = bmid;
        TS(15)
        RLAYER_OWN(NEU + 7, NCH, acc, xbuf, true, false)
        TS(16)
#pragma unroll
        for (int r = 0; r < R; r++) {
            float sacc = 0.f, ms = 0.f;
#pragma unroll
            for (int q = 0; q < 4; q++) {
                const f32x4v mm = mmv[r][q];
#pragma unroll
                for (int pq = 0; pq < 4; pq++) {
                    sacc = fmaf(fmaxf(acc[r][4 * q + pq], 0.f), mm[pq], sacc);
                    ms += mm[pq];
                }
            }
            sacc += __shfl_xor(sacc, 32);
            ms += __shfl_xor(ms, 32);
            if (live[r]) {
                if (h == 0) A.S[(size_t)n[r] * 128 + 32 * wave + j] = sacc * A.inv_K;
                if (tid == 0) A.msum[n[r]] = ms * A.inv_K;
            }
        }
    }
    if (pp_sat_hit(sat)) atomicOr(A.sat, 1u);
#ifdef PP_X_TS
    TS(17)
    if (A.dbg && tid == 0)
        for (int q = 0; q < 18; q++) A.dbg[(size_t)n[0] * 24 + q] = (float)tsv[q];
    if (A.dbg && tid == 0) A.dbg[(size_t)n[0] * 24 + 18] = (float)((ts0 >> 6) & 0xFFFFF);
#ifdef PP_X_TS_FINE
    if (A.dbg && tid == 0)
        for (int q = 0; q < 16; q++) A.dbg[(size_t)n[0] * 24 + q] = (float)tsf[q];
#endif
#endif
}

template <int R, bool ST0, bool FUSE, bool LNS = false, bool WB = true>
__global__ void __launch_bounds__(ET, R == 1 ? PP_WGS : PP_WGS2)
k_edge_update(EdgeArgs A) {
    extern __shared__ __attribute__((aligned(16))) float smem[];
    edge_update_body<R, ST0, FUSE, LNS, WB>(A, blockIdx.x * R, smem);
}

template <bool ST0, bool FUSE, bool LNS = false, bool WB = true>
__global__ void __launch_bounds__(ET, 2)
k_edge_update_mix(EdgeArgs A) {
    extern __shared__ __attribute__((aligned(16))) float smem[];
    const int b = blockIdx.x;
    int pair = -1, single = -1;
    if (A.mix_mode == 2) {
        const int ns = gridDim.x - A.n_pairs;
        if (b < 2 * ns) { if (b & 1) single = b >> 1; else pair = b >> 1; }
        else pair = b - ns;
    } else if (A.mix_mode == 3) {
        const int ns = gridDim.x - A.n_pairs;
        if (b < ns) single = b; else pair = b - ns;
    } else {
        if (b < A.n_pairs) pair = b; else single = b - A.n_pairs;
    }
    if (pair >= 0) edge_update_body<2, ST0, FUSE, LNS, WB>(A, 2 * pair, smem);
    else edge_update_body<1, ST0, FUSE, LNS, WB>(A, 2 * A.n_pairs + single, smem);
}

template <bool ST0>
__global__ void __launch_bounds__(ET, 2)
k_node_message_mix(EdgeArgs A) {
    extern __shared__ __attribute__((aligned(16))) float smem[];
    const int b = blockIdx.x;
    const int ns = gridDim.x - A.n_pairs;
    if (b < ns) node_message_body<1, ST0>(A, 2 * A.n_pairs + b, smem);
    else node_message_body<2, ST0>(A, 2 * (b - ns), smem);
}

template <bool LNS>
__global__ void __launch_bounds__(ET, 1)
k_edge_static(EdgeArgs A) {
    extern __shared__ __attribute__((aligned(16))) float smem[];
    constexpr int R = 1;
    const int tid = threadIdx.x, lane = tid & 63;
    const int wave = __builtin_amdgcn_readfirstlane(tid >> 6);
    const int j = lane & 31, h = lane >> 5;
    const int n = blockIdx.x;
    const int K = A.K;
    if (A.rmask[n] == 0.f) return;
    constexpr int NCH = 8;
#if defined(PP_X_TS) && defined(PP_X_TS_FINE)
    const unsigned long long ts0f = __builtin_readcyclecounter();
    int tsf[16] = {0};
#endif
    PROLOGUE_PIPE(NCH)
    HT x[1][4];
    f32x16 acc[1];
    const int jj = j < K ? j : K - 1;
    const float *hrow = A.hE_in + ((size_t)n * K + jj) * 128;
#pragma unroll
    for (int t = 0; t < 4; t++) {
        load_tile(hrow + 32 * t, h, acc[0]);
        if constexpr (LNS) scale_tile(A.ls_in + 32 * t, h, acc[0], acc[0]);
        unsigned nosat = 0;
        split_tile<false>(acc[0], x[0][t], nosat);
    }
#pragma unroll
    for (int r = 0; r < 16; r++) acc[0][r] = 0.f;
    WSTAGE(0, NCH, acc, (mfma_x<1, 0, false>(AK, x, acc)))
    WSTAGE(1, NCH, acc, (mfma_x<1, 1, false>(AK, x, acc)))
    WSTAGE(2, NCH, acc, (mfma_x<1, 2, false>(AK, x, acc)))
    WSTAGE(3, NCH, acc, (mfma_x<1, 3, false>(AK, x, acc)))
    store_tile(A.Znm + ((size_t)n * K + jj) * 128 + 32 * wave, h, acc[0]);
#pragma unroll
    for (int r = 0; r < 16; r++) acc[0][r] = 0.f;
    WSTAGE(4, NCH, acc, (mfma_x<1, 0, false>(AK, x, acc)))
    WSTAGE(5, NCH, acc, (mfma_x<1, 1, false>(AK, x, acc)))
    WSTAGE(6, NCH, acc, (mfma_x<1, 2, false>(AK, x, acc)))
    WSTAGE(7, NCH, acc, (mfma_x<1, 3, false>(AK, x, acc)))
    store_tile(A.Zem + ((size_t)n * K + jj) * 128 + 32 * wave, h, acc[0]);
}

__device__ __forceinline__ float dist_eps_nc(const float *a, const float *b, float eps) {
#pragma clang fp contract(off)
    float dx = a[0] - b[0], dy = a[1] - b[1], dz = a[2] - b[2];
    float s = dx * dx;
    s = s + dy * dy;
    s = s + dz * dz;
    return sqrtf(s + eps);
}
template <int C>
__device__ __forceinline__ void emb_step(const AOp &a, const float *gb, int lane, f32x16 &acc) {
#pragma unroll
    for (int s2 = 0; s2 < 2; s2++) {
        if (2 * C + s2 < 25) {
            const h8 *gp = reinterpret_cast<const h8 *>(gb) + (2 * (2 * C + s2)) * 64 + lane;
// ... 105 lines not shown
}
static const size_t EMB_SMEM = (EMB_GB_FLOATS + STAT_FLOATS) * sizeof(float);
pp_status pp_launch_edge_embed_f16(pp_ctx *c, hipStream_t s) {
    static bool attr_done = false;
    if (!attr_done) {
        PP_HIP_CHECK(hipFuncSetAttribute(reinterpret_cast<const void *>(k_edge_embed_f16),
                                         hipFuncAttributeMaxDynamicSharedMemorySize, (int)EMB_SMEM));
        attr_done = true;
    }
    const pp_plan *p = c->plan;
    EmbedArgs A;
    A.N = c->N; A.K = c->K;
    A.bbpos = c->bbpos; A.eidx = c->eidx; A.res_index = c->b.residue_index; A.chain = c->b.chain_indices;
    A.WT = p->edge_emb_T; A.bias = p->w + p->off.edge_emb_b;
    A.ln_g = p->w + p->off.norm_edges_g; A.ln_b = p->w + p->off.norm_edges_b;
    A.wstream = p->embed_stream; A.hE0 = c->hE0;
    hipLaunchKernelGGL(k_edge_embed_f16, dim3(c->N), dim3(ET), EMB_SMEM, s, A);
    PP_HIP_CHECK(hipGetLastError());
    return PP_OK;
}

static float *g_dbg = nullptr;
#ifdef PP_DIAG
extern "C" void pp_debug_set_dbg(float *p) { g_dbg = p; }
#endif
static EdgeArgs edge_args(pp_ctx *c, int layer, bool edge) {
    const pp_plan *p = c->plan;
    const LayerOff &o = p->off.layer[layer];
    EdgeArgs A;
    A.N = c->N; A.K = c->K; A.inv_K = 1.0f / (float)c->K;
    A.n_pairs = 0;
    A.mix_mode = 0;
    A.rmask = c->b.residue_mask;
    A.eidx = c->eidx; A.mask_att = c->mask_att; A.frames = c->frames;
    A.pts = edge ? c->ptsE : c->ptsN;
    A.PA = edge ? c->PAe : c->PAn;
    A.PC = edge ? c->PCe : c->PCn;
    A.hE_in = layer == 0 ? c->hE0 : c->hE;
    A.hE_out = c->hE;
    A.S = c->S; A.msum = c->msum;
    A.wstream = edge ? p->lt[layer].em_stream : p->lt[layer].nm_stream;
    A.params = p->lt[layer].em_params;
    A.g3 = p->w + o.norm_g[3]; A.be3 = p->w + o.norm_b[3];
    A.b_mid = p->w + o.nm_mid_b;
    A.Z = edge ? c->Zem : c->Znm;
    A.Znm = c->Znm; A.Zem = c->Zem;
    A.pts2 = c->ptsN; A.PA2 = c->PAn; A.PC2 = c->PCn;
    A.b_mid2 = p->w + p->off.layer[layer < 2 ? layer + 1 : 2].nm_mid_b;
    A.dbg = g_dbg;
    A.sat = c->sat;
    const float *ls = p->ln_scale;
    A.ls_in = ls ? ls + 128 * (layer == 0 ? PP_LN_E0 : PP_LN_E(layer - 1)) : nullptr;
    A.ls_x1 = ls ? ls + 128 * PP_LN_X1(layer < 2 ? layer : 1) : nullptr;
    A.ls_out = ls ? ls + 128 * PP_LN_E(layer < 2 ? layer : 1) : nullptr;
    return A;
}

#ifdef PP_NO_FUSE_NM
#define PP_FUSED false
#else
#define PP_FUSED true
#endif
#define PP_RMAX 2

#ifndef PP_LDS_PAD
#define PP_LDS_PAD 0
#endif
static size_t g_lds_pad = PP_LDS_PAD;
#ifdef PP_DIAG
extern "C" void pp_debug_set_lds_pad(int bytes) { g_lds_pad = (size_t)bytes; }
#endif
static size_t pad_smem(size_t b) { return b > g_lds_pad ? b : g_lds_pad; }
static size_t nm_smem(int R) { return pad_smem((R * XBUF_FLOATS + R * GBUF_FLOATS) * sizeof(float)); }
static size_t eu_smem(int R) {
    return pad_smem((2 * R * XBUF_FLOATS + R * STAT_FLOATS + PARAM_LDS + 256) * sizeof(float));
}
#define ST_SMEM pad_smem(0)
#define MAX_SMEM (160 * 1024)

typedef void (*edge_kernel_t)(EdgeArgs);
template <int R> static edge_kernel_t nm_kernel(bool st0) {
    return st0 ? k_node_message<R, true> : k_node_message<R, false>;
}
template <int R> static edge_kernel_t eu_kernel(bool st0, bool lns, bool wb) {
    if (!wb && !st0) return lns ? k_edge_update<R, false, PP_FUSED, true, false> : k_edge_update<R, false, PP_FUSED, false, false>;
    if (lns) return st0 ? k_edge_update<R, true, PP_FUSED, true> : k_edge_update<R, false, PP_FUSED, true>;
    return st0 ? k_edge_update<R, true, PP_FUSED> : k_edge_update<R, false, PP_FUSED>;
}
static edge_kernel_t mix_kernel(bool st0, bool lns, bool wb) {
    if (!wb && !st0) return lns ? k_edge_update_mix<false, PP_FUSED, true, false> : k_edge_update_mix<false, PP_FUSED, false, false>;
    if (lns) return st0 ? k_edge_update_mix<true, PP_FUSED, true> : k_edge_update_mix<false, PP_FUSED, true>;
    return st0 ? k_edge_update_mix<true, PP_FUSED> : k_edge_update_mix<false, PP_FUSED>;
}

static edge_kernel_t nm_kernel_r(int R, bool st0) {
    return R == 1 ? nm_kernel<1>(st0) : nm_kernel<2>(st0);
}
static edge_kernel_t eu_kernel_r(int R, bool st0, bool lns = false, bool wb = true) {
    return R == 1 ? eu_kernel<1>(st0, lns, wb) : eu_kernel<2>(st0, lns, wb);
}


static int g_num_cu = 0;
static bool edge_attrs() {
    static bool done = false, ok = false;
    if (!done) {
        done = true;
        auto set = [](const void *f, size_t bytes) {
            return hipFuncSetAttribute(f, hipFuncAttributeMaxDynamicSharedMemorySize, (int)bytes) == hipSuccess;
        };
        ok = set(reinterpret_cast<const void *>(k_edge_static<false>), MAX_SMEM) && set(reinterpret_cast<const void *>(k_edge_static<true>), MAX_SMEM);
        for (int R = 1; R <= PP_RMAX && ok; R++)
            for (int st0 = 0; st0 < 2 && ok; st0++)
                ok = set(reinterpret_cast<const void *>(nm_kernel_r(R, st0)), MAX_SMEM) &&
                     set(reinterpret_cast<const void *>(eu_kernel_r(R, st0, false, true)), MAX_SMEM) &&
                     set(reinterpret_cast<const void *>(eu_kernel_r(R, st0, true, true)), MAX_SMEM) &&
                     set(reinterpret_cast<const void *>(eu_kernel_r(R, st0, false, false)), MAX_SMEM) &&
                     set(reinterpret_cast<const void *>(eu_kernel_r(R, st0, true, false)), MAX_SMEM);
        for (int st0 = 0; st0 < 2 && ok; st0++)
            for (int lns = 0; lns < 2 && ok; lns++)
                ok = set(reinterpret_cast<const void *>(mix_kernel(st0, lns, true)), MAX_SMEM) &&
                     set(reinterpret_cast<const void *>(mix_kernel(st0, lns, false)), MAX_SMEM);
        ok = ok && set(reinterpret_cast<const void *>(k_node_message_mix<true>), MAX_SMEM) &&
             set(reinterpret_cast<const void *>(k_node_message_mix<false>), MAX_SMEM);
        int dev = 0;
        hipDeviceProp_t prop;
        if (hipGetDevice(&dev) == hipSuccess && hipGetDeviceProperties(&prop, dev) == hipSuccess)
            g_num_cu = prop.multiProcessorCount;
        if (g_num_cu <= 0) g_num_cu = 256;
    }
    return ok;
}

static int g_forced_R = -1;
#ifdef PP_DIAG
extern "C" void pp_debug_set_edge_R(int R) { g_forced_R = R; }
#endif
static int pick_R(int N) {
    if (g_forced_R < 0) {
        const char *e = PP_GETENV("PP_EDGE_R");
        g_forced_R = e ? atoi(e) : 0;
    }
    if (g_forced_R >= 1 && g_forced_R <= PP_RMAX) return g_forced_R;
    return N > PP_WGS * g_num_cu ? 2 : 1;
}

static int g_mix = -1;
static bool use_mix(int N) {
    if (g_mix < 0) {
        const char *e = PP_GETENV("PP_EDGE_MIX");
        g_mix = e ? atoi(e) : 3;
    }
    if (g_forced_R >= 1 || !g_mix) return false;
    return N > 2 * g_num_cu && N <= 3 * g_num_cu;
}

void pp_edge_occupancy(int *node_msg, int *edge_upd) {
    edge_attrs();
    (void)hipOccupancyMaxActiveBlocksPerMultiprocessor(node_msg, reinterpret_cast<const void *>(nm_kernel_r(1, false)), ET, nm_smem(1));
    (void)hipOccupancyMaxActiveBlocksPerMultiprocessor(edge_upd, reinterpret_cast<const void *>(eu_kernel_r(1, false)), ET, eu_smem(1));
}

#define EDGE_ATTR_CHECK()                                                                                   \
    if (!edge_attrs()) {                                                                                    \
        pp_set_error("hipFuncSetAttribute(MaxDynamicSharedMemorySize) failed for the edge kernels");        \
        return PP_ERR_HIP;                                                                                  \
    }

pp_status pp_launch_edge_static(pp_ctx *c, hipStream_t s) {
    EDGE_ATTR_CHECK()
    EdgeArgs A = edge_args(c, 0, false);
    A.wstream = c->plan->static_stream;
    if (c->plan->ln_scale) hipLaunchKernelGGL(k_edge_static<true>, dim3(c->N), dim3(ET), ST_SMEM, s, A);
    else hipLaunchKernelGGL(k_edge_static<false>, dim3(c->N), dim3(ET), ST_SMEM, s, A);
    PP_HIP_CHECK(hipGetLastError());
    return PP_OK;
}

pp_status pp_launch_node_message(pp_ctx *c, int layer, hipStream_t s) {
    EDGE_ATTR_CHECK()
    EdgeArgs A = edge_args(c, layer, false);
    static const char *nm_env = PP_GETENV("PP_NM_R");
    static const int nm_R = nm_env ? atoi(nm_env) : 0;
    const int R = (nm_R >= 1 && nm_R <= PP_RMAX) ? nm_R : pick_R(c->N);
    static const char *nmix_env = PP_GETENV("PP_NM_MIX");
    static const bool nmix = !(nmix_env && atoi(nmix_env) == 0);
    if (nmix && !(nm_R >= 1 && nm_R <= PP_RMAX) && use_mix(c->N)) {
        A.n_pairs = (c->N + 2) / 3;
        const int singles = c->N - 2 * A.n_pairs > 0 ? c->N - 2 * A.n_pairs : 0;
        PP_LAUNCH(c, (layer == 0 ? k_node_message_mix<true> : k_node_message_mix<false>), dim3(A.n_pairs + singles), dim3(ET),
                  nm_smem(2), s, A);
        PP_HIP_CHECK(hipGetLastError());
        return PP_OK;
    }
    PP_LAUNCH(c, nm_kernel_r(R, layer == 0), dim3((c->N + R - 1) / R), dim3(ET), nm_smem(R), s, A);
    PP_HIP_CHECK(hipGetLastError());
    return PP_OK;
}

extern "C" int pp_edge_variant(void) { return 1; }
bool pp_edge_fused() { return PP_FUSED; }

pp_status pp_launch_edge_update(pp_ctx *c, int layer, bool keep_hE, hipStream_t s) {
    EDGE_ATTR_CHECK()
    if (layer < 0 || layer > 1) { pp_set_error("pp_launch_edge_update: layer must be 0 or 1"); return PP_ERR_INVALID; }
    EdgeArgs A = edge_args(c, layer, true);
    const int R = pick_R(c->N);
    const bool lns = c->plan->ln_scale != nullptr;
    if (lns && !PP_FUSED) { pp_set_error("pp_launch_edge_update: a plan with LayerNorm operand scales needs the fused build"); return PP_ERR_UNSUPPORTED; }
    if (use_mix(c->N)) {
        A.n_pairs = (c->N + 2) / 3;
        A.mix_mode = g_mix;
        const int singles = c->N - 2 * A.n_pairs > 0 ? c->N - 2 * A.n_pairs : 0;
        PP_LAUNCH(c, mix_kernel(layer == 0, lns, keep_hE), dim3(A.n_pairs + singles), dim3(ET), eu_smem(2) > eu_smem(1) ? eu_smem(2) : eu_smem(1), s, A);
        PP_HIP_CHECK(hipGetLastError());
        return PP_OK;
    }
    PP_LAUNCH(c, eu_kernel_r(R, layer == 0, lns, keep_hE), dim3((c->N + R - 1) / R), dim3(ET), eu_smem(R), s, A);
    PP_HIP_CHECK(hipGetLastError());
    return PP_OK;
}
```

packppi_amd/csrc/pp_internal.h:

```cpp
#pragma once
#include <hip/hip_runtime.h>
#include <hip/hip_ext.h>
#include <cmath>
#include <vector>
#include <mutex>
#include <stdint.h>
#include <string>

#include "../../include/packppi_hip.h"

#if defined(PP_LAB) && !defined(PP_DIAG)
#define PP_DIAG
#endif
#if !defined(PP_LAB) &&                                                                                                       \
    (defined(PP_X_TS) || defined(PP_X_TS_FINE) || defined(PP_X_NOWLOAD) || defined(PP_X_E_NOMFMA) || defined(PP_X_NOSAT) ||      \
     defined(PP_WDEPTH) || defined(PP_WDEPTH_R1) || defined(PP_NXB_R1) || defined(PP_WGS2) || defined(PP_WGS) ||                 \
     defined(PP_NM_WGS2) ||                                                                                                  \
     defined(PP_LDS_PAD) || defined(PP_NO_FUSE_NM) || defined(PP_NU_DEPTH))
#error "PP_X_* / tuning switches compile laboratory variants (most give wrong results): add -DPP_LAB and build a TAGGED library (python -m packppi_amd.build --tag NAME -DPP_LAB -DPP_X_...)"
#endif
#ifdef PP_DIAG
#define PP_GETENV(name) getenv(name)
#else
#define PP_GETENV(name) ((const char *)nullptr)
#endif

#define PP_H 128
#define PP_MSG_IN 456
#define PP_NPTS 8
#define PP_PROX_CHUNK 64
#define PP_CL_CAP 96

#include "pp_weights.h"
#include "pp_rng.h"
#include "pp_segments.h"

struct LayerT {
    const float *pts_node_wT, *pts_edge_wT;
    const float *nm_A_T, *nm_C_T, *em_A_T, *em_C_T;
    const float *nm_out_T;
    const float *nd_in_T;
    const float *nd_out_T;
    const float *nm_stream, *em_stream;
    const float *em_params;
    const float *nu_stream;
    const float *nu_params;
};

#define PP_NU_WAVES 8
#define PP_NU_SLOT_FLOATS 512
#define PP_NU_SLOTS_MID 56
#define PP_NU_SLOTS_LAST 59
#define PP_NU_LO_SCALE 2048.0f
enum {
    NU_P_OUTB = 0, NU_P_G0 = 128, NU_P_B0 = 256, NU_P_FIB = 384, NU_P_FOB = 896, NU_P_G1 = 1024, NU_P_B1 = 1152,
    NU_P_PAE_B = 1280, NU_P_PAN_B = 1408, NU_P_PTS_B = 1536, NU_P_MID_TOTAL = 1600,
    NU_P_DB0 = 1280, NU_P_DB1 = 1344, NU_P_DB2 = 1376, NU_P_DB3 = 1392, NU_P_PAN0_B = 1408, NU_P_PTS0_B = 1536,
    NU_P_EMB_B = 1568, NU_P_EMB_G = 1696, NU_P_EMB_BETA = 1824, NU_P_LAST_TOTAL = 1952
};

struct ArenaSlot {
    void *p;
    size_t bytes;
    hipStream_t stream;
};
struct pp_plan {
    int device;
    std::vector<ArenaSlot> arena_pool;
    std::mutex pool_mutex;
    bool has_network;
    int knn_ties;
    float annealed_temp;
    int rebalanced_chains;
    float *ln_scale = nullptr;
    int ln_scaled_features = 0;
    float *w;
    WeightOff off;
    float *wT;
    LayerT lt[3];
    const float *node_emb_T;
    const float *edge_emb_T;
    const float *d0_in_T, *d0_out_T, *d2_in_T, *d2_out_T;
    const float *static_stream;
    const float *embed_stream;
    float *default_frames;
    int32_t *atom14_to_group;
    float *atom14_mask;
    float *lit_positions;
    float *between_radius;
    float *side_extent;
    float *bounds_lower, *bounds_upper;
    float clash_tol;
    bool clash_params_set;
};

#define PP_PI_D 3.14159265358979323846
static inline double pp_log_sigma_min() { return log(0.01 * PP_PI_D); }
static inline double pp_log_sigma_max() { return log(PP_PI_D); }

struct StepParams {
    float temb[16];
    float c_ode;
    float w;
    float c_drift;
    float c_diff;
    float pad[12];
};

struct pp_ctx {
    pp_plan *plan;
    pp_batch b;
    int B, L, K, N;
    bool packed = false;
    int shortest = 0;
    int32_t *seg_off;
    int2 *seg;
    int32_t *eidx;
    float *mask_att;
    float *frames;
    float *bbpos;
    float *hE0;
    float *Znm, *Zem;
    float *hE;
    float *hV;
    float *hV_alt;
    float *S;
    float *msum;
    float *ptsN, *PAn, *PCn;
    float *ptsE, *PAe, *PCe;
    float *score;
    float *chi_tmp;
    void *arena = nullptr;
    size_t arena_bytes = 0;
    hipStream_t last_stream = nullptr;
    int max_steps;
    float *xyz;
    float *rec;
    float *axes;
    float *rec2, *axes2;
    float *brad;
    float *per_res;
    float *dchi;
    float *px, *pm, *pv, *pz, *pxeff;
    uint8_t *pmask;
    int32_t *cand;
    int32_t *cand_cnt;
    float *prox_part;
    int32_t *prox_nrows;
    float2 *prox_seg;
    float *prox_inv;
    float *scal;
    pp_rng_row *rng_tab;
    uint64_t *rng_keys;
    bool rng_tab_set = false;
    unsigned *sat;
    int prof_which = -1;
    bool prof_armed = false;
    std::vector<hipEvent_t> prof_ev;
    size_t prof_n = 0;
};

void pp_set_error(const std::string &msg);
#define PP_HIP_CHECK(expr)                                                                   \
    do {                                                                                     \
        hipError_t _e = (expr);                                                              \
        if (_e != hipSuccess) {                                                              \
            pp_set_error(std::string(#expr) + ": " + hipGetErrorString(_e));                 \
            return PP_ERR_HIP;                                                               \
        }                                                                                    \
    } while (0)

#ifdef PP_CHECK_RANGE
#define PP_RANGE_COUNTER static __device__ unsigned int g_range_hits;
#define PP_RANGE(x)                                                                                    \
    {                                                                                                  \
        const float rx_ = (x);                                                                         \
        if (!(__builtin_fabsf(rx_) < 65504.f)) atomicAdd(&g_range_hits, 1u);                           \
    }
#define PP_RANGE_READER(name)                                                                          \
    unsigned int name(int reset) {                                                                     \
        unsigned int v = 0, z = 0;                                                                     \
        (void)hipMemcpyFromSymbol(&v, HIP_SYMBOL(g_range_hits), sizeof(v));                            \
        if (reset) (void)hipMemcpyToSymbol(HIP_SYMBOL(g_range_hits), &z, sizeof(z));                   \
        return v;                                                                                      \
    }
#else
#define PP_RANGE_COUNTER
#define PP_RANGE(x)
#define PP_RANGE_READER(name) \
    unsigned int name(int) { return 0; }
#endif
__device__ __forceinline__ bool pp_sat_hit(unsigned packed_max) {
    return (packed_max & 0xffffu) >= 0x7bffu || (packed_max >> 16) >= 0x7bffu;
}
unsigned int pp_edge_range_hits(int reset);
unsigned int pp_node_range_hits(int reset);

bool pp_prof_take(pp_ctx *c, hipEvent_t *e0, hipEvent_t *e1);
#define PP_LAUNCH(c, kernel, grid, block, shmem, s, ...)                                              \
    do {                                                                                               \
        hipEvent_t e0_ = nullptr, e1_ = nullptr;                                                       \
        if ((c)->prof_armed && pp_prof_take((c), &e0_, &e1_))                                          \
            hipExtLaunchKernelGGL(kernel, grid, block, shmem, s, e0_, e1_, 0, __VA_ARGS__);            \
        else                                                                                           \
            hipLaunchKernelGGL(kernel, grid, block, shmem, s, __VA_ARGS__);                            \
    } while (0)

#ifdef __HIPCC__
__device__ __forceinline__ void pp_cross_t(const float *a, const float *b, float *o) {
#pragma clang fp contract(off)
    const float q0 = a[2] * b[1], q1 = a[0] * b[2], q2 = a[1] * b[0];
    o[0] = __builtin_fmaf(a[1], b[2], -q0);
    o[1] = __builtin_fmaf(a[2], b[0], -q1);
    o[2] = __builtin_fmaf(a[0], b[1], -q2);
}
__device__ __forceinline__ float pp_dot_t(const float *a, const float *b) {
#pragma clang fp contract(off)
    const float p0 = a[0] * b[0], p1 = a[1] * b[1], p2 = a[2] * b[2];
    return (p0 + p1) + p2;
}
__device__ __forceinline__ void pp_unit_t(float *v) {
#pragma clang fp contract(off)
    const float x2 = v[0] * v[0];
    const float n = sqrtf(__builtin_fmaf(v[2], v[2], __builtin_fmaf(v[1], v[1], x2)));
    for (int k = 0; k < 3; k++) {
        const float q = v[k] / n;
        v[k] = (q != q) ? 0.f : q;
    }
}
__device__ __forceinline__ float pp_pair_dihedral_t(const float *p0, const float *p1, const float *p2, const float *p3) {
#pragma clang fp contract(off)
    float u0[3], u1[3], u2[3], n1[3], n2[3], c12[3];
    for (int k = 0; k < 3; k++) { u0[k] = p2[k] - p1[k]; u1[k] = p0[k] - p1[k]; u2[k] = p3[k] - p2[k]; }
    pp_cross_t(u0, u1, n1); pp_unit_t(n1);
    pp_cross_t(u0, u2, n2); pp_unit_t(n2);
    pp_cross_t(u1, u2, c12);
    const float sg = pp_dot_t(c12, u0);
    const float sgn = (sg > 0.f) ? 1.f : ((sg < 0.f) ? -1.f : 0.f);
    const float ang = sgn * acosf(pp_dot_t(n1, n2));
    return (ang != ang) ? 0.f : ang;
}
#endif

struct pp_affinity {
    int device;
    bool network;
    float *buf;
    const float *mut_bias, *seq_emb;
    const float *f0T, *f0_b, *f2T, *f2_b;
    const float *d0T, *d0_b, *d2T, *d2_b, *d4_w, *d4_b;
};

struct PPRng {
    const pp_rng_row *tab;
    uint32_t seed_lo, seed_hi;
};

struct PPPin {
    const uint8_t *fixed;
    const float *chi_ref;
    float *traj;
    float sigma;
    int renoise;
};

pp_status pp_launch_rng_table(pp_ctx *c, bool keys_set, hipStream_t s);
pp_status pp_launch_noise_seeded(pp_ctx *c, uint64_t seed, int step, float *noise, uint32_t *words, hipStream_t s);
pp_status pp_launch_add_noise_seeded(pp_ctx *c, const float *chi0, float sigma, uint64_t seed, float *chi, hipStream_t s);
pp_status pp_launch_affinity_embed(pp_ctx *c, const pp_affinity *a, const int64_t *rtype, const float *sc_sincos,
                                   const int64_t *mut_mask, const float *hV_pret, hipStream_t s);
pp_status pp_launch_prepare(pp_ctx *c, hipStream_t s, const int64_t *E_idx = nullptr);
pp_status pp_launch_node_embed(pp_ctx *c, const float *chi, const StepParams &sp, hipStream_t s);
pp_status pp_launch_node_embed_rows(pp_ctx *c, const float *chi, const float *t_rows, hipStream_t s);
pp_status pp_launch_node_update(pp_ctx *c, int layer, int last_mode, float *chi, int step, int mode,
                                const float *noise, const StepParams *cur, const StepParams *next, hipStream_t s,
                                const PPRng *rng = nullptr, const PPPin *pin = nullptr);
pp_status pp_launch_edge_static(pp_ctx *c, hipStream_t s);
#ifdef PP_EDGE_F16
pp_status pp_launch_edge_embed_f16(pp_ctx *c, hipStream_t s);
#endif
pp_status pp_launch_node_message(pp_ctx *c, int layer, hipStream_t s);
bool pp_edge_fused();
pp_status pp_launch_edge_update(pp_ctx *c, int layer, bool keep_hE, hipStream_t s);
pp_status pp_launch_atom14(pp_ctx *c, const float *chi, float *xyz, hipStream_t s);
pp_status pp_launch_clash(pp_ctx *c, const float *xyz, float *per_res, float *dchi, hipStream_t s, bool use_candidates = false);
pp_status pp_launch_proximal(pp_ctx *c, const float *chi, float lamda, int nsteps, float *traj,
                             float *chi_last, float *losses, hipStream_t s);
pp_status pp_launch_proximal_packed(pp_ctx *c, const float *chi, float lamda, int nsteps, bool norm_given, float *traj,
                                    float *chi_last, float *chi_accepted, float *losses, hipStream_t s,
                                    const uint8_t *fixed = nullptr, uint8_t *moved = nullptr);

void pp_edge_occupancy(int *node_msg, int *edge_upd);

#define PP_NU_MID 0
#define PP_NU_SCORE 1
#define PP_NU_STEP 2
```

packppi_amd/csrc/pp_node.hip:

```cpp
#include <string.h>

#include "pp_internal.h"
#include <utility>

PP_RANGE_COUNTER
PP_RANGE_READER(pp_node_range_hits)

#define NT 512
#ifndef PP_NODE_GROUPS
#define PP_NODE_GROUPS 1
#endif
#define NG PP_NODE_GROUPS
#define NB (4 * NG)

struct NodeArgs {
    int N;
    const float *rmask;
    const int64_t *rtype;
    const float *bb_sincos;
    const float *sc_mask;
    const uint8_t *m1pi, *m2pi;
    const float *frames;
    const float *embT, *emb_b, *emb_g, *emb_beta;
    float *hV, *S, *msum;
// ... 482 lines not shown
            rrow = rng.tab[nc];
        } else if (sde) {
            const size_t NN = (size_t)N * 4;
            const float *nz = noise + (size_t)step * 2 * NN + (size_t)nc * 4 + g;
            nz1 = nz[0];
            nz2 = nz[NN];
        }
        rt = (int)A.rtype[nc];
    }
    nf4 tailv = {0.f, 0.f, 0.f, 0.f};
    nf4 ev[4] = {tailv, tailv, tailv, tailv};
    const int erow = tid & 15, ern = n0 + erow < N ? n0 + erow : N - 1;
    const bool e_bb = MODE == PP_NU_STEP && tid >= 128 && tid < 144, e_te = MODE == PP_NU_STEP && tid >= 192 && tid < 208;
    {
        const int t48 = tid % 48, row = t48 / 3, rn = n0 + row < N ? n0 + row : N - 1;
        tailv = *reinterpret_cast<const nf4 *>(A.frames + (size_t)rn * 12 + 4 * (t48 - 3 * row));
    }
    nf2 bb0 = {0.f, 0.f}, bb1 = bb0, bb2 = bb0;
    if constexpr (MODE == PP_NU_STEP) {
        const nf2 *bp = reinterpret_cast<const nf2 *>(A.bb_sincos + (size_t)ern * 6);
        bb0 = bp[0]; bb1 = bp[1]; bb2 = bp[2];
    }
    constexpr int NPV = (NPAR / 4 + 511) / 512;
    nf4 pv[NPV];
#pragma unroll
    for (int i = 0; i < NPV; i++) {
        const int q = tid + 512 * i;
        pv[i] = reinterpret_cast<const nf4 *>(A.params)[q < NPAR / 4 ? q : 0];
    }
    const nh8 *wq = reinterpret_cast<const nh8 *>(A.wstream) + (size_t)wv * NSLOT * 128 + lane;
    AOpN AR[NU_NRING];
#pragma unroll
    for (int k = 0; k < NU_ND; k++) gload_N(wq, k, AR[k]);
    __builtin_amdgcn_sched_barrier(0);
    if constexpr (SEEDED) {
        if (wv == 0) {
            const pp_rng_words w = pp_rng_draw(rng.seed_lo, rng.seed_hi, rrow, g, step);
            nz1 = pp_rng_normal(w.o[0], w.o[1]);
            nz2 = pp_rng_normal(w.o[2], w.o[3]);
            if constexpr (PINNED) {
                if (pin.renoise) cref = pp_noised_angle(cref, nz1, nz2, pin.sigma, m1raw != 0, m2raw != 0);
                const bool fx = fixraw != 0;
                chi1 = fx ? cref : chi1;
                m1raw = fx ? 2 : (m1raw != 0 ? 1 : 0);
                m2raw = fx ? 0 : m2raw;
            }
        }
        asm volatile("" : "+v"(nz1), "+v"(nz2));
        if constexpr (PINNED) {
            unsigned mw = m1raw | ((unsigned)m2raw << 8);
            asm volatile("" : "+v"(chi1), "+v"(mw));
            m1raw = (unsigned char)mw;
            m2raw = (unsigned char)(mw >> 8);
        }
    }
#pragma unroll
    for (int i = 0; i < NPV; i++) {
        const int q = tid + 512 * i;
        if (q < NPAR / 4) reinterpret_cast<nf4 *>(sm.par)[q] = pv[i];
    }
    nf4 oh4 = {0.f, 0.f, 0.f, 0.f};
    if constexpr (MODE == PP_NU_STEP) {
        oh4 = *reinterpret_cast<const nf4 *>(A.embT + (size_t)rt * 128 + fc);
    }
    if (e_te) {
#pragma unroll
        for (int k = 0; k < 16; k++) ev[k >> 2][k & 3] = te_next.v[k];
    } else {
        ev[0] = nf4{bb0[0], bb0[1], bb1[0], bb1[1]};
        ev[1] = nf4{bb2[0], bb2[1], 0.f, 0.f};
    }
    if (tid < 48) reinterpret_cast<nf4 *>(&sm.fr[0][0])[tid] = tailv;
    else if (e_bb) {
        publish4(sm.e_hi, sm.e_lo, erow * NU_S32, ev[0]);
        publish4(sm.e_hi, sm.e_lo, erow * NU_S32 + 4, ev[1]);
    } else if (e_te) {
        publish4(sm.e_hi, sm.e_lo, erow * NU_S32 + 12, nf4{0.f, 0.f, ev[0][0], ev[0][1]});
        publish4(sm.e_hi, sm.e_lo, erow * NU_S32 + 16, nf4{ev[0][2], ev[0][3], ev[1][0], ev[1][1]});
        publish4(sm.e_hi, sm.e_lo, erow * NU_S32 + 20, nf4{ev[1][2], ev[1][3], ev[2][0], ev[2][1]});
        publish4(sm.e_hi, sm.e_lo, erow * NU_S32 + 24, nf4{ev[2][2], ev[2][3], ev[3][0], ev[3][1]});
        publish4(sm.e_hi, sm.e_lo, erow * NU_S32 + 28, nf4{ev[3][2], ev[3][3], 0.f, 0.f});
    }
    publish4(sm.a_hi, sm.a_lo, srow * NU_S128 + scol, s4);
    __syncthreads();

    nh8 bh[4], bl[4];
    nf4 cH, cL;
    float satm = 0.f;
    const nf4 zero4 = zero4i;
    LDB4(sm.a_hi, sm.a_lo)
    cH = zero4; cL = zero4;
    NTILE4(0, cH, cL)
    nf4 x = fold(cH, cL) + *reinterpret_cast<const nf4 *>(par + NU_P_OUTB + fc) * ms + hv4;
    const nf4 h1 = ln128(sm.stats[0], wv, r, g, x, *reinterpret_cast<const nf4 *>(par + NU_P_G0 + fc),
                         *reinterpret_cast<const nf4 *>(par + NU_P_B0 + fc));
    publish4(sm.b_hi, sm.b_lo, r * NU_S128 + fc, h1);
    __syncthreads();
    LDB4(sm.b_hi, sm.b_lo)
#define FFN_IN_TILE(c)                                                                                     \
    cH = zero4; cL = zero4;                                                                                \
    NTILE4(4 + 4 * (c), cH, cL)                                                                            \
    publish4(sm.c_hi, sm.c_lo, r * NU_S512 + 16 * (4 * wv + (c)) + 4 * g,                                  \
             relu_sat(fold(cH, cL) + *reinterpret_cast<const nf4 *>(par + NU_P_FIB + 16 * (4 * wv + (c)) + 4 * g), satm));
    FFN_IN_TILE(0) FFN_IN_TILE(1) FFN_IN_TILE(2) FFN_IN_TILE(3)
    if (!(satm < 65504.f)) atomicOr(A.sat, 2u);
    __syncthreads();
    nh8 fh[2], fl[2];
    ldB(sm.c_hi, sm.c_lo, r * NU_S512 + 8 * g, 0, fh[0], fl[0]);
    cH = zero4; cL = zero4;
    FOSTAGE(0) FOSTAGE(1) FOSTAGE(2) FOSTAGE(3) FOSTAGE(4) FOSTAGE(5) FOSTAGE(6) FOSTAGE(7)
    FOSTAGE(8) FOSTAGE(9) FOSTAGE(10) FOSTAGE(11) FOSTAGE(12) FOSTAGE(13) FOSTAGE(14) FOSTAGE(15)
    x = fold(cH, cL) + *reinterpret_cast<const nf4 *>(par + NU_P_FOB + fc) + h1;
    const nf4 h2 = ln128(sm.stats[1], wv, r, g, x, *reinterpret_cast<const nf4 *>(par + NU_P_G1 + fc),
                         *reinterpret_cast<const nf4 *>(par + NU_P_B1 + fc)) * rm;
    if (live && clq == 0 && (MODE != PP_NU_STEP || !embed_next)) *reinterpret_cast<nf4 *>(A.hV_out + (size_t)n * 128 + fc) = h2;
    publish4(sm.a_hi, sm.a_lo, r * NU_S128 + fc, h2);
    __syncthreads();
    LDB4(sm.a_hi, sm.a_lo)

    if constexpr (!LAST) {
        constexpr int NPJ = 4 / CL;
#define NU_PROJ(i)                                                                                                     \
        if constexpr ((i) < NPJ) {                                                                                     \
            cH = zero4; cL = zero4;                                                                                    \
            NTILE4(36 + 4 * (i), cH, cL)                                                                               \
            const int pj = NPJ * clq + (i);                                                                            \
            float *dst = pj == 0 ? A.PAe : pj == 1 ? A.PCe : pj == 2 ? A.PAn : A.PCn;                                  \
            nf4 v = fold(cH, cL);                                                                                      \
            if (pj == 0) v = v + *reinterpret_cast<const nf4 *>(par + NU_P_PAE_B + fc);                                \
            else if (pj == 2) v = v + *reinterpret_cast<const nf4 *>(par + NU_P_PAN_B + fc);                           \
            if (live) *reinterpret_cast<nf4 *>(dst + (size_t)n * 128 + fc) = v;                                        \
        }
        NU_PROJ(0) NU_PROJ(1) NU_PROJ(2) NU_PROJ(3)
#undef NU_PROJ
        if (CL > 1 && clq != 0) return;
        cH = zero4; cL = zero4;
        NTILE4_IF(36 + 4 * NPJ, wv < 3, cH, cL)
        if (wv < 3) {
            const nf4 p = fold(cH, cL) + *reinterpret_cast<const nf4 *>(par + NU_P_PTS_B + fc);
            *reinterpret_cast<nf4 *>(&sm.pts[r][fc]) = p;
            if (live) {
                if (fc < 24) *reinterpret_cast<nf4 *>(A.ptsE + (size_t)n * 48 + fc) = p;
                else *reinterpret_cast<nf4 *>(A.ptsN + (size_t)n * 48 + fc - 24) = p;
            }
        }
        __syncthreads();
        if (tid < 256) {
            const int mm = tid >> 7, q = (tid >> 4) & 7, i = tid & 15, ni = n0 + i;
            if (ni < N) {
                float *pts = mm == 0 ? A.ptsE : A.ptsN;
                const float *fr = sm.fr[i];
                const float px = sm.pts[i][24 * mm + 3 * q], py = sm.pts[i][24 * mm + 3 * q + 1], pz = sm.pts[i][24 * mm + 3 * q + 2];
#pragma unroll
                for (int rr = 0; rr < 3; rr++)
                    pts[(size_t)ni * 48 + 24 + 3 * q + rr] = (fr[3 * rr] * px + fr[3 * rr + 1] * py + fr[3 * rr + 2] * pz) + fr[9 + rr];
            }
        }
        return;
    } else {
        cH = zero4; cL = zero4;
        NTILE4_IF(36, wv < 4, cH, cL)
        if (wv < 4) {
            publish4(sm.c_hi, sm.c_lo, r * NU_S512 + fc, relu_sat(fold(cH, cL) + *reinterpret_cast<const nf4 *>(par + NU_P_DB0 + fc), satm));
        }
        __syncthreads();
        const bool w0 = wv == 0;
        {
            nh8 dh[2], dl[2];
            if (w0) {
                ldB(sm.c_hi, sm.c_lo, r * NU_S512 + 8 * g, 0, dh[0], dl[0]);
                ldB(sm.c_hi, sm.c_lo, r * NU_S512 + 8 * g, 1, dh[1], dl[1]);
            }
            nf4 eH = zero4, eL = zero4;
            cH = zero4; cL = zero4;
            NSTAGE_IF(40, w0, cH, mm3(AK, dh[0], dl[0], cH, cL))
            NSTAGE_IF(41, w0, cH, mm3(AK, dh[1], dl[1], cH, cL))
            NSTAGE_IF(42, w0, eH, mm3(AK, dh[0], dl[0], eH, eL))
            NSTAGE_IF(43, w0, eH, mm3(AK, dh[1], dl[1], eH, eL))
            if (w0) {
                publish4(sm.c_hi, sm.c_lo, r * NU_S512 + 64 + 4 * g, relu_sat(fold(cH, cL) + *reinterpret_cast<const nf4 *>(par + NU_P_DB1 + 4 * g), satm));
                publish4(sm.c_hi, sm.c_lo, r * NU_S512 + 80 + 4 * g, relu_sat(fold(eH, eL) + *reinterpret_cast<const nf4 *>(par + NU_P_DB1 + 16 + 4 * g), satm));
                asm volatile("s_waitcnt lgkmcnt(0)" ::: "memory");
                ldB(sm.c_hi, sm.c_lo, r * NU_S512 + 8 * g, 2, dh[0], dl[0]);
            }
            cH = zero4; cL = zero4;
            NSTAGE_IF(44, w0, cH, mm3(AK, dh[0], dl[0], cH, cL))
            if (w0) {
                publish4(sm.c_hi, sm.c_lo, r * NU_S512 + 96 + 4 * g, relu_sat(fold(cH, cL) + *reinterpret_cast<const nf4 *>(par + NU_P_DB2 + 4 * g), satm));
                asm volatile("s_waitcnt lgkmcnt(0)" ::: "memory");
                ldB(sm.c_hi, sm.c_lo, r * NU_S512 + 8 * g, 3, dh[0], dl[0]);
            }
            cH = zero4; cL = zero4;
            NSTAGE_IF(45, w0, cH, mm3(AK, dh[0], dl[0], cH, cL))
        }
        if (w0) {
            if (!(satm < 65504.f)) atomicOr(A.sat, 2u);
            const nf4 sc = fold(cH, cL) + *reinterpret_cast<const nf4 *>(par + NU_P_DB3);
            if (g == 0 && live) *reinterpret_cast<nf4 *>(A.score + (size_t)n * 4) = sc;
            if constexpr (MODE == PP_NU_STEP) {
                const float s0 = __shfl(sc[0], r), s1 = __shfl(sc[1], r), s2 = __shfl(sc[2], r), s3 = __shfl(sc[3], r);
                const float sg = g == 0 ? s0 : g == 1 ? s1 : g == 2 ? s2 : s3;
                const float sp_c_ode = spv[0], sp_w = spv[1], sp_c_drift = spv[2], sp_c_diff = spv[3];
                const float sw = sg * sp_w;
#define NU_M1ON (PINNED ? m1raw == 1 : m1raw != 0)
                float yk = chi1;
                if (!sde) {
                    if (NU_M1ON || m2raw != 0) yk = chi1 + sp_c_ode * sw;
                } else {
                    if (NU_M1ON) yk = chi1 + (sp_c_drift * sw + sp_c_diff * nz1);
                    if (m2raw != 0) yk = yk + (sp_c_drift * sw + sp_c_diff * nz2);
                }
#undef NU_M1ON
                float y = wrap_pi(yk) * scm1;
                if constexpr (PINNED) {
                    if (m1raw == 2) y = chi1;
                }
                if (live) chi[(size_t)n * 4 + g] = y;
                if constexpr (PINNED) {
                    if (pin.traj != nullptr && live) pin.traj[(size_t)n * 4 + g] = y;
                }
                if (embed_next) {
                    unsigned hp, lp;
                    split2(sinf(y) * scm1, cosf(y) * scm1, hp, lp);
                    *reinterpret_cast<unsigned *>(sm.e_hi + r * NU_S32 + 6 + 2 * g) = hp;
                    *reinterpret_cast<unsigned *>(sm.e_lo + r * NU_S32 + 6 + 2 * g) = lp;
                }
            }
        }
        if constexpr (MODE != PP_NU_STEP) return;
        if (!embed_next) return;
        __syncthreads();
        nh8 eh, el;
        eh = *reinterpret_cast<const nh8 *>(sm.e_hi + r * NU_S32 + 8 * g);
        el = *reinterpret_cast<const nh8 *>(sm.e_lo + r * NU_S32 + 8 * g);
        cH = zero4; cL = zero4;
        NSTAGE(46, cH, mm3(AK, eh, el, cH, cL))
        const nf4 e0 = fold(cH, cL) + (*reinterpret_cast<const nf4 *>(par + NU_P_EMB_B + fc) + oh4);
        const nf4 h0 = ln128(sm.stats[2], wv, r, g, e0, *reinterpret_cast<const nf4 *>(par + NU_P_EMB_G + fc),
                             *reinterpret_cast<const nf4 *>(par + NU_P_EMB_BETA + fc));
        if (live) *reinterpret_cast<nf4 *>(A.hV_out + (size_t)n * 128 + fc) = h0;
        publish4(sm.b_hi, sm.b_lo, r * NU_S128 + fc, h0);
        __syncthreads();
        LDB4(sm.b_hi, sm.b_lo)
        cH = zero4; cL = zero4;
        NTILE4(47, cH, cL)
        if (live) *reinterpret_cast<nf4 *>(A.PAn + (size_t)n * 128 + fc) = fold(cH, cL) + *reinterpret_cast<const nf4 *>(par + NU_P_PAN0_B + fc);
        cH = zero4; cL = zero4;
        NTILE4(51, cH, cL)
        if (live) *reinterpret_cast<nf4 *>(A.PCn + (size_t)n * 128 + fc) = fold(cH, cL);
        if (wv < 2) {
            cH = zero4; cL = zero4;
            NTILE4(55, cH, cL)
            if (fc < 24) {
                const nf4 p = fold(cH, cL) + *reinterpret_cast<const nf4 *>(par + NU_P_PTS0_B + fc);
                *reinterpret_cast<nf4 *>(&sm.pts[r][fc]) = p;
                if (live) *reinterpret_cast<nf4 *>(A.ptsN + (size_t)n * 48 + fc) = p;
            }
        }
        __syncthreads();
        if (tid < 128) {
            const int q = tid >> 4, i = tid & 15, ni = n0 + i;
            if (ni < N) {
                const float *fr = sm.fr[i];
                const float px = sm.pts[i][3 * q], py = sm.pts[i][3 * q + 1], pz = sm.pts[i][3 * q + 2];
#pragma unroll
                for (int rr = 0; rr < 3; rr++)
                    A.ptsN[(size_t)ni * 48 + 24 + 3 * q + rr] = (fr[3 * rr] * px + fr[3 * rr + 1] * py + fr[3 * rr + 2] * pz) + fr[9 + rr];
            }
        }
    }
}

#ifndef PP_EDGE_F16
struct UpdW {
    const float *outT, *out_b;
    const float *g0, *b0, *g1, *b1;
    const float *ffn_inT, *ffn_in_b, *ffn_outT, *ffn_out_b;
    PreW pre_edge, pre_next;
    const float *d0_inT, *d0_in_b, *d0_outT, *d0_out_b, *d2_inT, *d2_in_b, *d2_outT, *d2_out_b;
// ... 684 lines not shown
```

packppi_amd/csrc/pp_prepare.hip:

```cpp
#include "pp_internal.h"
#include "pp_topk_aten.h"

#define KNN_THREADS 256
#define KNN_PAR_MAX 2047

#pragma clang fp contract(off)

__device__ __forceinline__ float dist_eps(const float *a, const float *b, float eps) {
    float dx = a[0] - b[0], dy = a[1] - b[1], dz = a[2] - b[2];
    float s = dx * dx;
    s = s + dy * dy;
    s = s + dz * dz;
    return sqrtf(s + eps);
}

__global__ void k_frames(const float *__restrict__ X, int N, float *__restrict__ frames,
                         float *__restrict__ bbpos) {
    int n = blockIdx.x * blockDim.x + threadIdx.x;
    if (n >= N) return;
    const float *x = X + (size_t)n * 42;
    float Nn[3], CA[3], C[3], O[3];
    for (int k = 0; k < 3; k++) { Nn[k] = x[k]; CA[k] = x[3 + k]; C[k] = x[6 + k]; O[k] = x[9 + k]; }
    float a[3], b[3];
    for (int k = 0; k < 3; k++) { a[k] = C[k] - CA[k]; b[k] = Nn[k] - CA[k]; }
// ... 246 lines not shown
#pragma unroll
        for (int e = 0; e < 32; e++) {
            float4 r = *reinterpret_cast<const float4 *>(rbf + e * EF_STRIDE + m);
            acc[e] = fmaf(w0, r.x, acc[e]);
            acc[e] = fmaf(w1, r.y, acc[e]);
            acc[e] = fmaf(w2, r.z, acc[e]);
            acc[e] = fmaf(w3, r.w, acc[e]);
        }
    }
    __syncthreads();
    float *pre = rbf;
    const float bf = bias[f], w465 = WT[(size_t)465 * 128 + f], w466 = WT[(size_t)466 * 128 + f],
                w467 = WT[(size_t)467 * 128 + f];
#pragma unroll
    for (int e = 0; e < 32; e++) {
        if (e < K) {
            int rp = (int)s_extra[e][0];
            float v = acc[e] + bf + WT[(size_t)rp * 128 + f];
            v = fmaf(w465, s_extra[e][1], v);
            v = fmaf(w466, s_extra[e][2], v);
            v = fmaf(w467, s_extra[e][3], v);
            pre[e * 128 + f] = v;
        }
    }
    __syncthreads();
    const int lane = tid & 63, wid = tid >> 6;
    for (int e = wid; e < K; e += EF_THREADS / 64) {
        float v0 = pre[e * 128 + lane], v1 = pre[e * 128 + 64 + lane];
        float s = v0 + v1;
        for (int o = 32; o > 0; o >>= 1) s += __shfl_xor(s, o);
        float mean = s * (1.f / 128.f);
        float d0 = v0 - mean, d1 = v1 - mean;
        float q = d0 * d0 + d1 * d1;
        for (int o = 32; o > 0; o >>= 1) q += __shfl_xor(q, o);
        float rstd = 1.f / sqrtf(q * (1.f / 128.f) + 1e-5f);
        float *o = hE0 + ((size_t)n * K + e) * 128;
        o[lane] = d0 * rstd * ln_g[lane] + ln_b[lane];
        o[64 + lane] = d1 * rstd * ln_g[64 + lane] + ln_b[64 + lane];
    }
}

__global__ void k_import_graph(const int64_t *__restrict__ E_idx, const int2 *__restrict__ seg,
                               const float *__restrict__ rmask, int N, int K, int32_t *__restrict__ eidx,
                               float *__restrict__ mask_att, int *__restrict__ bad) {
    const int t = blockIdx.x * blockDim.x + threadIdx.x;
    if (t >= N * 32) return;
    const int n = t >> 5, k = t & 31;
    if (k >= K) { mask_att[(size_t)n * 32 + k] = 0.f; return; }
    const int64_t j = E_idx[(size_t)n * K + k];
    const int2 sg = seg[n];
    if (j < 0 || j >= sg.y) { atomicAdd(bad, 1); eidx[(size_t)n * K + k] = n; mask_att[(size_t)n * 32 + k] = 0.f; return; }
    eidx[(size_t)n * K + k] = sg.x + (int)j;
    mask_att[(size_t)n * 32 + k] = rmask[n] * rmask[sg.x + (int)j];
}

pp_status pp_launch_prepare(pp_ctx *c, hipStream_t s, const int64_t *E_idx) {
    const int N = c->N;
    if (E_idx) {
        PP_HIP_CHECK(hipMemsetAsync(c->scal, 0, sizeof(int), s));
        hipLaunchKernelGGL(k_import_graph, dim3((N * 32 + 255) / 256), dim3(256), 0, s, E_idx, c->seg, c->b.residue_mask, N, c->K,
                           c->eidx, c->mask_att, reinterpret_cast<int *>(c->scal));
    } else {
    hipLaunchKernelGGL(k_frames, dim3((N + 127) / 128), dim3(128), 0, s, c->b.X, N, c->frames, c->bbpos);
    const size_t smem = (size_t)c->L * sizeof(pp_tk_pair) + 2 * (KNN_PAR_MAX + 1) * sizeof(short);
    if (smem > 64 * 1024) {
        PP_HIP_CHECK(hipFuncSetAttribute(reinterpret_cast<const void *>(k_knn),
                                         hipFuncAttributeMaxDynamicSharedMemorySize, (int)smem));
    }
    hipLaunchKernelGGL(k_knn, dim3(N), dim3(KNN_THREADS), smem, s, c->b.X, c->b.residue_mask, c->seg, c->K,
                       c->plan->knn_ties, c->L, c->eidx, c->mask_att);
    }
#ifdef PP_EDGE_F16
    return pp_launch_edge_embed_f16(c, s);
#else
    const pp_plan *p = c->plan;
    size_t smem2 = (size_t)32 * EF_STRIDE * sizeof(float);
    hipLaunchKernelGGL(k_edge_embed, dim3(N), dim3(EF_THREADS), smem2, s, c->bbpos, c->eidx, c->b.residue_index,
                       c->b.chain_indices, c->K, p->edge_emb_T, p->w + p->off.edge_emb_b,
                       p->w + p->off.norm_edges_g, p->w + p->off.norm_edges_b, c->hE0);
    PP_HIP_CHECK(hipGetLastError());
    return PP_OK;
#endif
}
```

packppi_amd/lib.py:

```python
import ctypes as C
import os

import numpy as np
import torch

from . import constants as rc
from .weights import check_state_dict

_LIB_PATH = os.environ.get("PACKPPI_LIB") or os.path.join(os.path.dirname(os.path.abspath(__file__)), "csrc", "libpackppi_hip.so")
_lib = None

SYMBOLS = ("pp_version", "pp_last_error", "pp_build_id", "pp_plan_set_knn_ties", "pp_plan_set_annealed_temp", "pp_plan_rebalanced_chains", "pp_rebalance_weights_host", "pp_plan_ln_scaled_features", "pp_ln_operand_scales_host", "pp_topk_aten_host", "pp_plan_create", "pp_plan_destroy", "pp_plan_set_clash_params",
           "pp_complex_prepare", "pp_complex_prepare_packed", "pp_ctx_destroy", "pp_ctx_get_graph", "pp_ctx_set_graph", "pp_score", "pp_sample", "pp_atom14",
           "pp_clash", "pp_proximal", "pp_proximal_packed", "pp_time_kernel", "pp_profile_kernel", "pp_profile_read", "pp_edge_variant", "pp_has_range_check", "pp_range_check", "pp_range_check_parts", "pp_ctx_saturated",
           "pp_affinity_create", "pp_affinity_destroy", "pp_affinity_encode", "pp_affinity_predict",
           "pp_score_rows", "pp_so2_set_grids", "pp_so2_score", "pp_dsm_loss",
           "pp_ctx_set_rng_keys", "pp_noise_seeded", "pp_add_noise_seeded", "pp_sample_seeded",
           "pp_sample_partial", "pp_proximal_pinned")


FIX_MODES = {"hold": 0, "renoise": 1}
KNN_TIES = {"lower_index": 0, "aten_cpu": 1, "aten_member": 2}


class PPTables(C.Structure):
    _fields_ = [("default_frames", C.c_void_p), ("atom14_to_group", C.c_void_p), ("atom14_mask", C.c_void_p),
                ("lit_positions", C.c_void_p), ("between_radius", C.c_void_p)]


class PPBatch(C.Structure):
    _fields_ = [("B", C.c_int32), ("L", C.c_int32), ("X", C.c_void_p), ("atom_mask", C.c_void_p),
                ("residue_type", C.c_void_p), ("residue_mask", C.c_void_p), ("residue_index", C.c_void_p),
                ("chain_indices", C.c_void_p), ("BB_D", C.c_void_p), ("BB_D_sincos", C.c_void_p),
                ("SC_D", C.c_void_p), ("SC_D_mask", C.c_void_p), ("chi_1pi_periodic_mask", C.c_void_p),
                ("chi_2pi_periodic_mask", C.c_void_p)]


def load():
    global _lib
    if _lib is not None:
        return _lib
    if not os.path.exists(_LIB_PATH):
        raise RuntimeError(f"{_LIB_PATH} is missing: build it with `python -m packppi_amd.build` "
                           "(hipcc --offload-arch=gfx950); there is no CPU fallback")
    lib = C.CDLL(_LIB_PATH)
    vp, f, i = C.c_void_p, C.c_float, C.c_int
    try:
        lib.pp_build_id.restype = C.c_char_p
    except AttributeError:
        raise RuntimeError(f"{_LIB_PATH} is stale: it predates the build stamp (no pp_build_id); rebuild with "
                           "`python -m packppi_amd.build` (or `python __graft_entry__.py`)") from None
    if not os.environ.get("PACKPPI_SKIP_BUILD_CHECK"):
        from .build import product_flag_stamps, source_hash
        have, _, have_flags = lib.pp_build_id().decode().partition("-")
        want = source_hash()
        if have != want:
            raise RuntimeError(f"{_LIB_PATH} is stale: built from sources {have}, csrc/ is now {want}; rebuild with "
                               "`python -m packppi_amd.build` (or `python __graft_entry__.py`)")
        if have_flags not in product_flag_stamps() and not os.environ.get("PACKPPI_ALLOW_LAB_LIBRARY"):
            raise RuntimeError(f"{_LIB_PATH} was built with flags (stamp {have_flags}) that are none of the product sets "
                               f"{sorted(product_flag_stamps().values())}: a laboratory variant; set PACKPPI_ALLOW_LAB_LIBRARY=1 "
                               "to load it for a measurement")
    lib.pp_plan_set_knn_ties.argtypes = [vp, i]
    lib.pp_plan_set_annealed_temp.argtypes = [vp, f]
    lib.pp_plan_rebalanced_chains.argtypes = [vp]
    lib.pp_rebalance_weights_host.argtypes = [vp, C.c_size_t, vp, C.POINTER(C.c_int)]
    lib.pp_plan_rebalanced_chains.restype = C.c_int
    lib.pp_plan_ln_scaled_features.argtypes = [vp]
    lib.pp_plan_ln_scaled_features.restype = C.c_int
    lib.pp_ln_operand_scales_host.argtypes = [vp, C.c_size_t, vp, C.POINTER(C.c_int)]
    lib.pp_topk_aten_host.argtypes = [vp, i, i, vp]
    lib.pp_version.restype = C.c_int
    lib.pp_last_error.restype = C.c_char_p
    lib.pp_plan_create.argtypes = [vp, C.c_size_t, C.POINTER(PPTables), i, C.POINTER(vp)]
    lib.pp_plan_destroy.argtypes = [vp]
    lib.pp_plan_destroy.restype = None
    lib.pp_plan_set_clash_params.argtypes = [vp, f, vp, vp, vp]
    lib.pp_complex_prepare.argtypes = [vp, C.POINTER(PPBatch), vp, C.POINTER(vp)]
    lib.pp_complex_prepare_packed.argtypes = [vp, C.POINTER(PPBatch), vp, i, i, i, vp, C.POINTER(vp)]
    lib.pp_ctx_destroy.argtypes = [vp]
    lib.pp_ctx_destroy.restype = None
    lib.pp_ctx_get_graph.argtypes = [vp, vp, vp, vp]
    lib.pp_ctx_set_graph.argtypes = [vp, vp, vp]
    lib.pp_score.argtypes = [vp, vp, f, vp, vp, vp]
    lib.pp_sample.argtypes = [vp, vp, vp, i, i, vp, vp]
    lib.pp_atom14.argtypes = [vp, vp, vp, vp]
    lib.pp_clash.argtypes = [vp, vp, vp, vp, vp]
    lib.pp_proximal.argtypes = [vp, vp, f, i, vp, vp, vp, vp]
    lib.pp_proximal_packed.argtypes = [vp, vp, f, i, vp, vp, vp, vp, vp, vp]
    lib.pp_time_kernel.argtypes = [vp, i, i, C.POINTER(C.c_float), vp]
    lib.pp_profile_kernel.argtypes = [vp, i]
    lib.pp_profile_read.argtypes = [vp, C.POINTER(C.c_float), C.POINTER(C.c_int)]
    lib.pp_edge_variant.argtypes = []
    lib.pp_has_range_check.argtypes = []
    lib.pp_has_range_check.restype = C.c_int
    lib.pp_range_check.argtypes = [C.POINTER(C.c_ulonglong), i]
    lib.pp_range_check_parts.argtypes = [C.POINTER(C.c_ulonglong), C.POINTER(C.c_ulonglong), i]
    lib.pp_ctx_saturated.argtypes = [vp, C.POINTER(C.c_int), vp]
    lib.pp_edge_variant.restype = C.c_int
    lib.pp_affinity_create.argtypes = [vp, C.c_size_t, i, C.POINTER(vp)]
    lib.pp_affinity_destroy.argtypes = [vp]
    lib.pp_affinity_destroy.restype = None
    lib.pp_affinity_encode.argtypes = [vp, vp, vp, vp, vp, vp, vp, vp]
    lib.pp_affinity_predict.argtypes = [vp, vp, vp, vp, i, i, vp, vp, vp]
    lib.pp_score_rows.argtypes = [vp, vp, vp, vp, vp, vp]
    lib.pp_so2_set_grids.argtypes = [vp, vp, i]
    lib.pp_so2_score.argtypes = [vp, vp, C.c_size_t, i, vp, vp, i, vp]
    lib.pp_dsm_loss.argtypes = [vp, vp, vp, vp, vp, vp, vp, vp]
    lib.pp_ctx_set_rng_keys.argtypes = [vp, vp, vp]
    lib.pp_noise_seeded.argtypes = [vp, C.c_uint64, i, vp, vp, vp]
    lib.pp_add_noise_seeded.argtypes = [vp, vp, f, C.c_uint64, vp, vp]
    lib.pp_sample_seeded.argtypes = [vp, vp, vp, i, i, C.c_uint64, vp]
    lib.pp_sample_partial.argtypes = [vp, vp, vp, vp, i, vp, i, i, C.c_uint64, vp, vp]
    lib.pp_proximal_pinned.argtypes = [vp, vp, vp, f, i, vp, vp, vp, vp, vp, vp, vp]
    _lib = lib
    return lib


def _check(status, what):
    if status != 0:
        msg = load().pp_last_error()
        raise RuntimeError(f"{what} failed (pp_status {status}): {msg.decode() if msg else ''}")


def _stream(device):
    return C.c_void_p(torch.cuda.current_stream(device).cuda_stream)


def _ptr(t):
    return C.c_void_p(t.data_ptr()) if t is not None else C.c_void_p(0)


def _seed64(seed) -> int:
    return int(seed) & 0xFFFFFFFFFFFFFFFF


def ln_operand_scales(state_dict):
    lib = load()
    sd = check_state_dict(state_dict)
    flat = np.ascontiguousarray(torch.cat([v.reshape(-1) for v in sd.values()]).numpy(), dtype=np.float32)
    out = np.empty((5, 128), np.float32)
    n = C.c_int(0)
    _check(lib.pp_ln_operand_scales_host(flat.ctypes.data, flat.size, out.ctypes.data, C.byref(n)), "pp_ln_operand_scales_host")
    return torch.from_numpy(out), int(n.value)


def rebalanced_state_dict(state_dict):
    lib = load()
    sd = check_state_dict(state_dict)
    flat = np.ascontiguousarray(torch.cat([v.reshape(-1) for v in sd.values()]).numpy(), dtype=np.float32)
    out = np.empty_like(flat)
    n = C.c_int(0)
    _check(lib.pp_rebalance_weights_host(flat.ctypes.data, flat.size, out.ctypes.data, C.byref(n)), "pp_rebalance_weights_host")
    res, at = {}, 0
    for k, v in sd.items():
        res[k] = torch.from_numpy(out[at:at + v.numel()].reshape(tuple(v.shape)).copy())
        at += v.numel()
    return res, int(n.value)


class Plan:

    def __init__(self, state_dict, device):
        lib = load()
        self.device = torch.device(device)
        if self.device.type != "cuda":
            raise RuntimeError("packppi_amd runs on an MI355X HIP device only (got device '%s')" % device)
        if self.device.index is None:
            self.device = torch.device("cuda", torch.cuda.current_device())
        self.has_network = state_dict is not None
        if self.has_network:
            sd = check_state_dict(state_dict)
            flat = np.ascontiguousarray(torch.cat([v.reshape(-1) for v in sd.values()]).numpy(), dtype=np.float32)
            wptr, wn = flat.ctypes.data, flat.size
        else:
            wptr, wn = None, 0
        self._keep = [
            np.ascontiguousarray(rc.default_frames, np.float32), np.ascontiguousarray(rc.atom14_to_group, np.int32),
            np.ascontiguousarray(rc.atom14_mask, np.float32), np.ascontiguousarray(rc.lit_positions, np.float32),
            np.ascontiguousarray(rc.between_radius, np.float32)]
        tab = PPTables(*[a.ctypes.data for a in self._keep])
        h = C.c_void_p()
        _check(lib.pp_plan_create(wptr, wn, C.byref(tab), self.device.index, C.byref(h)), "pp_plan_create")
        self.handle = h
        self._clash_params = None
        self.knn_ties = "aten_cpu"
        if os.environ.get("PACKPPI_KNN_TIES"):
            self.set_knn_ties(os.environ["PACKPPI_KNN_TIES"])

    def set_knn_ties(self, mode):
        if mode not in KNN_TIES:
            raise ValueError(f"knn ties mode must be one of {sorted(KNN_TIES)}")
        _check(load().pp_plan_set_knn_ties(self.handle, KNN_TIES[mode]), "pp_plan_set_knn_ties")
        self.knn_ties = mode

    def rebalanced_chains(self) -> int:
        return int(load().pp_plan_rebalanced_chains(self.handle))
# ... 199 lines not shown
                                _ptr(nz), _stream(self.plan.device)), "pp_sample")
        return chi

    def sample_partial(self, chi, chi_ref, fixed, schedule, mode, seed, fix_mode="renoise", trajectory=False):
        if mode not in ("ode", "sde"):
            raise NotImplementedError(mode)
        if fix_mode not in FIX_MODES:
            raise ValueError(f"fix_mode must be one of {sorted(FIX_MODES)}")
        chi = self._chi(chi).clone()
        ref = self._chi(chi_ref)
        fx = torch.as_tensor(fixed).to(device=self.plan.device)
        if fx.numel() != self.n_rows:
            raise ValueError(f"fixed has {fx.numel()} elements, this context has {self.n_rows} rows")
        fx = (fx != 0).to(torch.uint8).reshape(-1).contiguous()
        sched = np.ascontiguousarray(torch.as_tensor(schedule, dtype=torch.float32).cpu().numpy())
        traj = self._new(max(len(sched) - 1, 0), self.B, self.L, 4) if trajectory else None
        _check(load().pp_sample_partial(self.handle, _ptr(chi), _ptr(ref), _ptr(fx), FIX_MODES[fix_mode], sched.ctypes.data,
                                        int(len(sched)), 0 if mode == "ode" else 1, _seed64(seed), _ptr(traj),
                                        _stream(self.plan.device)), "pp_sample_partial")
        return (chi, traj) if trajectory else chi

    def atom14(self, chi):
        chi = self._chi(chi)
        xyz = self._new(self.B, self.L, 14, 3)
        _check(load().pp_atom14(self.handle, _ptr(chi), _ptr(xyz), _stream(self.plan.device)), "pp_atom14")
        return xyz

    def clash(self, chi, vtf=12.0, tol=0.5, need_grad=False):
        self.plan.set_clash_params(vtf, tol)
        chi = self._chi(chi)
        per_res = self._new(self.B, self.L)
        dchi = self._new(self.B, self.L, 4) if need_grad else None
        _check(load().pp_clash(self.handle, _ptr(chi), _ptr(per_res), _ptr(dchi), _stream(self.plan.device)), "pp_clash")
        return (per_res, dchi) if need_grad else per_res

    def proximal(self, chi, vtf, tol, lamda, num_steps, want_traj=True):
        self.plan.set_clash_params(vtf, tol)
        chi = self._chi(chi)
        traj = self._new(num_steps, self.B, self.L, 4) if want_traj else None
        last = self._new(self.B, self.L, 4)
        losses = self._new(num_steps)
        _check(load().pp_proximal(self.handle, _ptr(chi), float(lamda), int(num_steps), _ptr(traj), _ptr(last),
                                  _ptr(losses), _stream(self.plan.device)), "pp_proximal")
        return traj, last, losses

    def proximal_packed(self, chi, vtf, tol, lamda, num_steps, norm_rows=None, want_traj=False, fixed=None, return_moved=False):
        if return_moved and fixed is None:
            raise ValueError("return_moved needs fixed: the unpinned call does not report its mask (functional.find_clash_mask does)")
        self.plan.set_clash_params(vtf, tol)
        offs, n_seg = self.seg_offsets_host, self.n_segments
        nr = None
        if norm_rows is not None:
            nr = np.ascontiguousarray([int(x) for x in norm_rows], dtype=np.int32)
            if nr.size != n_seg:
                raise ValueError(f"norm_rows has {nr.size} entries for {n_seg} complexes")
            lens = [b - a for a, b in zip(offs[:-1], offs[1:])]
            short = [(k, int(r), n) for k, (r, n) in enumerate(zip(nr, lens)) if r < n]
            if self.B == 1 and short:
                k, r, n = short[0]
                raise ValueError(f"norm_rows[{k}] = {r} is shorter than complex {k} ({n} rows)")
        chi = self._chi(chi)
        traj = self._new(num_steps, self.B, self.L, 4) if want_traj else None
        last, accepted = self._new(self.B, self.L, 4), self._new(self.B, self.L, 4)
        losses = self._new(n_seg, max(int(num_steps), 1))
        nrp = C.c_void_p(nr.ctypes.data) if nr is not None else C.c_void_p(0)
        if fixed is None:
            _check(load().pp_proximal_packed(self.handle, _ptr(chi), float(lamda), int(num_steps), nrp, _ptr(traj), _ptr(last),
                                             _ptr(accepted), _ptr(losses), _stream(self.plan.device)), "pp_proximal_packed")
            return traj, last, accepted, losses
        fx = torch.as_tensor(fixed).to(device=self.plan.device)
        if fx.numel() != self.n_rows:
            raise ValueError(f"fixed has {fx.numel()} elements, this context has {self.n_rows} rows")
        fx = (fx != 0).to(torch.uint8).reshape(-1).contiguous()
        moved = self._new(self.B, self.L, dtype=torch.uint8) if return_moved else None
        _check(load().pp_proximal_pinned(self.handle, _ptr(chi), _ptr(fx), float(lamda), int(num_steps), nrp, _ptr(traj), _ptr(last),
                                         _ptr(accepted), _ptr(losses), _ptr(moved), _stream(self.plan.device)), "pp_proximal_pinned")
        return (traj, last, accepted, losses, moved.bool()) if return_moved else (traj, last, accepted, losses)

    def saturated(self) -> int:
        v = C.c_int(0)
        _check(load().pp_ctx_saturated(self.handle, C.byref(v), _stream(self.plan.device)), "pp_ctx_saturated")
        return int(v.value)

    def time_kernel(self, which: int, iters: int = 20) -> float:
        ms = C.c_float(0.0)
        _check(load().pp_time_kernel(self.handle, int(which), int(iters), C.byref(ms), _stream(self.plan.device)),
               "pp_time_kernel")
        return float(ms.value)

    def profile_kernel(self, which: int):
        _check(load().pp_profile_kernel(self.handle, int(which)), "pp_profile_kernel")

    def profile_read(self):
        ms, n = C.c_float(0.0), C.c_int(0)
        _check(load().pp_profile_read(self.handle, C.byref(ms), C.byref(n)), "pp_profile_read")
        return (float(ms.value) / max(n.value, 1), int(n.value))

    def __del__(self):
        h = getattr(self, "handle", None)
        if h and _lib is not None:
            _lib.pp_ctx_destroy(h)
            self.handle = None


SO2_GRID = 5001
_so2_grids_on = set()


def so2_grids():
    X_MIN, X_N, SIGMA_MIN, SIGMA_MAX, SIGMA_N = 1e-5, 5000, 3e-3, 2, 5000
    xs, ss = [], []
    for PI in (1 / 2 * np.pi, np.pi):
        xs.append(10 ** np.linspace(np.log10(X_MIN), 0, X_N + 1) * PI)
        ss.append(10 ** np.linspace(np.log10(SIGMA_MIN), np.log10(SIGMA_MAX), SIGMA_N + 1) * PI)
    return np.ascontiguousarray(np.stack(xs)), np.ascontiguousarray(np.stack(ss))


def so2_score(x, sigma, pi_periodic: bool, want_idx: bool = False):
    if x.device.type != "cuda":
        raise RuntimeError(f"so2_score needs tensors on the HIP device, got {x.device}")
    lib, dev = load(), x.device
    idx_dev = dev.index if dev.index is not None else torch.cuda.current_device()
    if idx_dev not in _so2_grids_on:
        xg, sg = so2_grids()
        _check(lib.pp_so2_set_grids(xg.ctypes.data, sg.ctypes.data, idx_dev), "pp_so2_set_grids")
        _so2_grids_on.add(idx_dev)
    xf = x.to(torch.float32).contiguous()
    sf = sigma.to(device=dev, dtype=torch.float32).expand_as(xf).contiguous()
    score = torch.empty_like(xf)
    idx = torch.empty(*xf.shape, 2, dtype=torch.int32, device=dev) if want_idx else None
    _check(lib.pp_so2_score(_ptr(xf), _ptr(sf), xf.numel(), 1 if pi_periodic else 0, _ptr(score), _ptr(idx), idx_dev, _stream(dev)),
           "pp_so2_score")
    return (score, idx) if want_idx else score


class AffinityHead:

    def __init__(self, state_dict, device, mode="network"):
        from .weights import affinity_head_spec
        lib = load()
        self.device = torch.device(device)
        if self.device.index is None:
            self.device = torch.device("cuda", torch.cuda.current_device())
        self.mode = mode
        flat = np.ascontiguousarray(torch.cat([torch.as_tensor(state_dict[n]).detach().float().cpu().reshape(-1)
                                               for n, _ in affinity_head_spec(mode)]).numpy(), dtype=np.float32)
        h = C.c_void_p()
        _check(lib.pp_affinity_create(flat.ctypes.data, flat.size, self.device.index, C.byref(h)), "pp_affinity_create")
        self.handle = h

    def encode(self, ctx: "Context", residue_type, sc_sincos, mut_mask, hV_pret):
        dev = self.device
        rt = residue_type.to(device=dev, dtype=torch.int64).contiguous()
        sc = sc_sincos.to(device=dev, dtype=torch.float32).contiguous()
        mm = mut_mask.to(device=dev, dtype=torch.int64).contiguous()
        hp = hV_pret.to(device=dev, dtype=torch.float32).contiguous()
        n = ctx.n_rows
        if rt.numel() != n or sc.numel() != 8 * n or mm.numel() != n or hp.numel() != 128 * n:
            raise RuntimeError("pp_affinity_encode: tensors do not match the context's rows")
        hV = torch.empty(hp.shape, dtype=torch.float32, device=dev)
        _check(load().pp_affinity_encode(self.handle, ctx.handle, _ptr(rt), _ptr(sc), _ptr(mm), _ptr(hp), _ptr(hV),
                                         _stream(dev)), "pp_affinity_encode")
        return hV

    def predict(self, h_wt, h_mt, seg_offsets):
        dev = self.device
# ... 24 lines not shown
```

Baseline: 62210 residues/s.

## Run the last edge-update layer only over residues with live side-chain torsions

A new single-workgroup kernel builds a compacted list of live rows: real residues that have at least one chi angle and are not pinned. It builds this once at context prepare, and again per partial-sampling call with the fixed mask. During sampling the layer-1 fused edge update, which writes no h_E, launches only over those rows, through new LIVE template variants including a paired mixed-launch work table. Residues without torsions (Gly/Ala) and fixed ones no longer pay for that layer's edge MLP. The saturation flag in the node step is also restricted to live rows so dead rows cannot raise it. The risk is that any consumer of the skipped rows' layer-1 outputs now sees stale values, and the mixed-launch grid is sized from the CU count.

Result: faster. 64630 residues/s (median of 6 runs) (+3.9%).

```diff
diff --git a/include/packppi_hip.h b/include/packppi_hip.h
--- a/include/packppi_hip.h
+++ b/include/packppi_hip.h
@@ -156,6 +156,8 @@
 
 pp_status pp_ctx_saturated(pp_ctx *ctx, int *flags, void *stream);
 
+pp_status pp_ctx_live_rows(pp_ctx *ctx, int32_t *rows, int *count, void *stream);
+
 #ifdef PP_DIAG
 pp_status pp_debug_edge(pp_ctx *ctx, int layer, void *stream);
 pp_status pp_debug_nm(pp_ctx *ctx, int layer, void *stream);
diff --git a/packppi_amd/csrc/pp_api.hip b/packppi_amd/csrc/pp_api.hip
--- a/packppi_amd/csrc/pp_api.hip
+++ b/packppi_amd/csrc/pp_api.hip
@@ -94,6 +94,19 @@
     PP_HIP_CHECK(hipMemcpyAsync(&v, c->sat, sizeof(v), hipMemcpyDeviceToHost, s));
     PP_HIP_CHECK(hipStreamSynchronize(s));
     *flags = (int)v;
+    return PP_OK;
+}
+
+extern "C" pp_status pp_ctx_live_rows(pp_ctx *c, int32_t *rows, int *count, void *stream) {
+    if (!c || !rows || !count) FAIL(PP_ERR_INVALID, "pp_ctx_live_rows: null argument");
+    if (!c->plan->has_network) FAIL(PP_ERR_INVALID, "pp_ctx_live_rows: plan was created without network weights");
+    hipStream_t s = static_cast<hipStream_t>(stream);
+    PP_HIP_CHECK(hipSetDevice(c->plan->device));
+    int32_t cnt = 0;
+    PP_HIP_CHECK(hipMemcpyAsync(rows, c->live_rows[0], (size_t)c->N * sizeof(int32_t), hipMemcpyDeviceToDevice, s));
+    PP_HIP_CHECK(hipMemcpyAsync(&cnt, c->live_cnt[0], sizeof(cnt), hipMemcpyDeviceToHost, s));
+    PP_HIP_CHECK(hipStreamSynchronize(s));
+    *count = (int)cnt;
     return PP_OK;
 }
 
@@ -142,6 +155,7 @@
     std::unique_ptr<pp_plan, PlanDeleter> p(new (std::nothrow) pp_plan());
     if (!p) FAIL(PP_ERR_INVALID, "out of host memory");
     p->device = device;
+    p->num_cu = prop.multiProcessorCount > 0 ? prop.multiProcessorCount : 256;
     p->off = off;
     p->has_network = has_net;
     p->knn_ties = PP_KNN_TIES_ATEN_CPU;
@@ -358,6 +372,7 @@
         ALLOC(ptsN, N * 48); ALLOC(PAn, N * 128); ALLOC(PCn, N * 128);
         ALLOC(ptsE, N * 48); ALLOC(PAe, N * 128); ALLOC(PCe, N * 128);
         ALLOC(score, N * 4); ALLOC(chi_tmp, N * 4);
+        for (int k = 0; k < 2; k++) { ALLOC(live_rows[k], N + 2); ALLOC(live_mix[k], N); ALLOC(live_cnt[k], 1); }
     }
     ALLOC(xyz, N * 42); ALLOC(rec, N * 64); ALLOC(axes, N * 24); ALLOC(rec2, N * 64); ALLOC(axes2, N * 24); ALLOC(brad, N); ALLOC(per_res, N); ALLOC(dchi, N * 4);
     ALLOC(px, N * 4); ALLOC(pm, N * 4); ALLOC(pv, N * 4); ALLOC(pz, N * 4); ALLOC(pxeff, N * 4); ALLOC(pmask, N);
@@ -408,6 +423,7 @@
         flag_nonfinite(c, c->b.X, 42, 12, s_);
         if ((st = pp_launch_prepare(c, s_)) != PP_OK) return st;
         if ((st = pp_launch_edge_static(c, s_)) != PP_OK) return st;
+        if ((st = pp_launch_live_rows(c, 0, nullptr, s_)) != PP_OK) return st;
     }
     *out = owner.release();
     return PP_OK;
@@ -498,8 +514,15 @@
     return true;
 }
 
+static bool edge_live_on() {
+    static const char *e = getenv("PP_EDGE_LIVE");
+    static const bool on = !(e && atoi(e) == 0);
+    return on;
+}
+
 static pp_status run_network(pp_ctx *c, hipStream_t s, int step, int last_mode, float *chi, int mode, const float *noise,
-                             const StepParams *cur, const StepParams *next, const PPRng *rng = nullptr, const PPPin *pin = nullptr) {
+                             const StepParams *cur, const StepParams *next, const PPRng *rng = nullptr, const PPPin *pin = nullptr,
+                             const PPLive *live = nullptr) {
     pp_status st;
     for (int l = 0; l < 3; l++) {
         if (l == 0 || !pp_edge_fused()) {
@@ -514,7 +537,7 @@
             prof_disarm(c);
             if (st != PP_OK) return st;
             prof_arm(c, 1);
-            st = pp_launch_edge_update(c, l, l == 0 || !pp_edge_fused(), s);
+            st = pp_launch_edge_update(c, l, l == 0 || !pp_edge_fused(), s, l == 1 ? live : nullptr);
             prof_disarm(c);
             if (st != PP_OK) return st;
         } else {
@@ -680,6 +703,14 @@
     if ((st = pp_launch_node_embed(c, chi, steps[0], s)) != PP_OK) return st;
     static const bool dbg = PP_GETENV("PP_DEBUG") != nullptr;
     const auto h0 = std::chrono::steady_clock::now();
+    PPLive live = {nullptr, nullptr};
+    const bool use_live = edge_live_on() && pp_edge_fused() && c->prof_which < 0;
+    if (use_live) {
+        const int set = part ? 1 : 0;
+        if (part && (st = pp_launch_live_rows(c, 1, part->fixed, s)) != PP_OK) return st;
+        live.rows = c->live_rows[set];
+        live.mix = c->live_mix_set[set] ? c->live_mix[set] : nullptr;
+    }
     for (int j = 0; j < nsteps; j++) {
         PPPin pin = {nullptr, nullptr, nullptr, 0.f, 0};
         if (part) {
@@ -690,7 +721,7 @@
             pin.renoise = part->fix_mode == PP_FIX_RENOISE && j + 1 < nsteps ? 1 : 0;
         }
         if ((st = run_network(c, s, j, PP_NU_STEP, chi, mode, sde_noise, &steps[j], j + 1 < nsteps ? &steps[j + 1] : nullptr, rng,
-                              part ? &pin : nullptr)) != PP_OK) return st;
+                              part ? &pin : nullptr, use_live ? &live : nullptr)) != PP_OK) return st;
     }
     if (dbg) {
         const double us = std::chrono::duration<double, std::micro>(std::chrono::steady_clock::now() - h0).count();
diff --git a/packppi_amd/csrc/pp_edge.hip b/packppi_amd/csrc/pp_edge.hip
--- a/packppi_amd/csrc/pp_edge.hip
+++ b/packppi_amd/csrc/pp_edge.hip
@@ -14,7 +14,10 @@
 struct EdgeArgs {
     int N, K;
     float inv_K;
-    const float *rmask;
+    union {
+        const float *rmask;
+        const int32_t *live_rows;
+    };
     const int32_t *eidx;
     const float *mask_att;
     const float *frames;
@@ -240,7 +243,7 @@
     WSTAGE(C0 + 11 + 8 * (c) + 6, NCH, xbuf_get(xbuf, 2, lane, acc); mfma_tile32<false>(wslot, acc, out, lane))   \
     WSTAGE(C0 + 11 + 8 * (c) + 7, NCH, xbuf_get(xbuf, 3, lane, acc); mfma_tile32<false>(wslot, acc, out, lane))
 
-template <int S, bool ST0, bool FUSE, bool WB = true>
+template <int S, bool ST0, bool FUSE, bool WB = true, bool LIVE = false>
 __global__ void __launch_bounds__(ET, PP_EU_WGS)
 k_edge_update(EdgeArgs A) {
     extern __shared__ __attribute__((aligned(16))) float smem[];
@@ -248,10 +251,12 @@
     const int tid = threadIdx.x, lane = tid & 63;
     const int wave = __builtin_amdgcn_readfirstlane(tid >> 6);
     const int j = lane & 31, h = lane >> 5;
-    const int n = blockIdx.x;
+    static_assert(!LIVE || !WB, "a launch over the live rows alone leaves the other rows' h_E unwritten");
+    const int n = LIVE ? A.live_rows[blockIdx.x] : (int)blockIdx.x;
     const int K = A.K;
     const int jj = j < K ? j : K - 1;
-    if (A.rmask[n] == 0.f) {
+    if (LIVE && n < 0) return;
+    if (!LIVE && A.rmask[n] == 0.f) {
         if (WB && j < K) {
             f32x4v z = {0.f, 0.f, 0.f, 0.f};
             float *orow = A.hE_out + ((size_t)n * K + j) * 128 + 32 * wave;
@@ -479,7 +484,8 @@
              set(reinterpret_cast<const void *>(k_node_message<PP_NM_SLOTS, true>), NM_SMEM) &&
              set(reinterpret_cast<const void *>(k_edge_update<PP_EU_SLOTS, false, true>), EU_SMEM) &&
              set(reinterpret_cast<const void *>(k_edge_update<PP_EU_SLOTS, true, true>), EU_SMEM) &&
-             set(reinterpret_cast<const void *>(k_edge_update<PP_EU_SLOTS, false, true, false>), EU_SMEM);
+             set(reinterpret_cast<const void *>(k_edge_update<PP_EU_SLOTS, false, true, false>), EU_SMEM) &&
+             set(reinterpret_cast<const void *>(k_edge_update<PP_EU_SLOTS, false, true, false, true>), EU_SMEM);
     }
     return ok;
 }
@@ -517,12 +523,15 @@
     return PP_OK;
 }
 
-pp_status pp_launch_edge_update(pp_ctx *c, int layer, bool keep_hE, hipStream_t s) {
+pp_status pp_launch_edge_update(pp_ctx *c, int layer, bool keep_hE, hipStream_t s, const PPLive *live) {
     EDGE_ATTR_CHECK()
     if (layer < 0 || layer > 1) { pp_set_error("pp_launch_edge_update: layer must be 0 or 1"); return PP_ERR_INVALID; }
+    if (live && (layer != 1 || keep_hE)) { pp_set_error("pp_launch_edge_update: the live-row launch is layer 1's, without write-back"); return PP_ERR_INVALID; }
     EdgeArgs A = edge_args(c, layer, true);
+    if (live) A.live_rows = live->rows;
     if (layer == 0) PP_LAUNCH(c, (k_edge_update<PP_EU_SLOTS, true, true>), dim3(c->N), dim3(ET), EU_SMEM, s, A);
     else if (keep_hE) PP_LAUNCH(c, (k_edge_update<PP_EU_SLOTS, false, true>), dim3(c->N), dim3(ET), EU_SMEM, s, A);
+    else if (live) PP_LAUNCH(c, (k_edge_update<PP_EU_SLOTS, false, true, false, true>), dim3(c->N), dim3(ET), EU_SMEM, s, A);
     else PP_LAUNCH(c, (k_edge_update<PP_EU_SLOTS, false, true, false>), dim3(c->N), dim3(ET), EU_SMEM, s, A);
     PP_HIP_CHECK(hipGetLastError());
     return PP_OK;
diff --git a/packppi_amd/csrc/pp_edge_f16.hip b/packppi_amd/csrc/pp_edge_f16.hip
--- a/packppi_amd/csrc/pp_edge_f16.hip
+++ b/packppi_amd/csrc/pp_edge_f16.hip
@@ -67,7 +67,11 @@
 struct EdgeArgs {
     int N, K;
     float inv_K;
-    const float *rmask;
+    union {
+        const float *rmask;
+        const int32_t *live_rows;
+        const int2 *live_mix;
+    };
     const int32_t *eidx;
     const float *mask_att;
     const float *frames;
@@ -345,8 +349,10 @@
 #define GROUP_SETUP()                                                                          \
     int n[R];                                                                                  \
     bool live[R], inr[R];                                                                      \
+    int first = -1;                                                                            \
+    GROUP_SETUP_ROWS()
+#define GROUP_SETUP_ROWS()                                                                     \
     float rm_[R];                                                                              \
-    int first = -1;                                                                            \
     _Pragma("unroll") for (int r = 0; r < R; r++) {                                            \
         const int nr = res0 + r;                                                               \
         inr[r] = nr < A.N;                                                                     \
@@ -509,8 +515,8 @@
 #else
 #define TS(i)
 #endif
-template <int R, bool ST0, bool FUSE, bool LNS = false, bool WB = true>
-__device__ __forceinline__ void edge_update_body(const EdgeArgs &A, const int res0, float *smem) {
+template <int R, bool ST0, bool FUSE, bool LNS = false, bool WB = true, bool LIVE = false>
+__device__ __forceinline__ void edge_update_body(const EdgeArgs &A, const int res0, float *smem, const int2 lrow = {-1, -1}) {
     float *const xbuf = smem, *const x1buf = smem + R * XBUF_FLOATS, *const stat = x1buf + R * XBUF_FLOATS,
                  *const prm = stat + R * STAT_FLOATS;
     const int tid = threadIdx.x, lane = tid & 63;
@@ -519,10 +525,23 @@
     const int K = A.K;
     const int jj = j < K ? j : K - 1;
     unsigned sat = 0;
-    GROUP_SETUP()
+    int n[R];
+    bool live[R], inr[R];
+    int first = -1;
+    if constexpr (LIVE) {
+        static_assert(!WB, "a launch over the live rows alone leaves the other rows' h_E unwritten");
+#pragma unroll
+        for (int r = 0; r < R; r++) {
+            n[r] = r == 0 ? lrow.x : lrow.y;
+            inr[r] = live[r] = n[r] >= 0;
+        }
+        first = lrow.x;
+    } else {
+        GROUP_SETUP_ROWS()
+    }
 #pragma unroll
     for (int r = 0; r < R; r++)
-        if (inr[r] && !live[r]) {
+        if (!LIVE && inr[r] && !live[r]) {
             if (WB && j < K) {
                 f32x4v z = {0.f, 0.f, 0.f, 0.f};
                 float *orow = A.hE_out + ((size_t)n[r] * K + j) * 128 + 32 * wave;
@@ -731,18 +750,33 @@
 #endif
 }
 
-template <int R, bool ST0, bool FUSE, bool LNS = false, bool WB = true>
+template <int R, bool ST0, bool FUSE, bool LNS = false, bool WB = true, bool LIVE = false>
 __global__ void __launch_bounds__(ET, R == 1 ? PP_WGS : PP_WGS2)
 k_edge_update(EdgeArgs A) {
     extern __shared__ __attribute__((aligned(16))) float smem[];
-    edge_update_body<R, ST0, FUSE, LNS, WB>(A, blockIdx.x * R, smem);
-}
-
-template <bool ST0, bool FUSE, bool LNS = false, bool WB = true>
+    if constexpr (LIVE) {
+        int2 lrow = {-1, -1};
+        if constexpr (R == 2) lrow = *reinterpret_cast<const int2 *>(A.live_rows + 2 * blockIdx.x);
+        else lrow.x = A.live_rows[blockIdx.x];
+        if (lrow.x < 0) return;
+        edge_update_body<R, ST0, FUSE, LNS, WB, true>(A, 0, smem, lrow);
+    } else {
+        edge_update_body<R, ST0, FUSE, LNS, WB>(A, blockIdx.x * R, smem);
+    }
+}
+
+template <bool ST0, bool FUSE, bool LNS = false, bool WB = true, bool LIVE = false>
 __global__ void __launch_bounds__(ET, 2)
 k_edge_update_mix(EdgeArgs A) {
     extern __shared__ __attribute__((aligned(16))) float smem[];
     const int b = blockIdx.x;
+    if constexpr (LIVE) {
+        const int2 lrow = A.live_mix[b];
+        if (lrow.x < 0) return;
+        if (lrow.y >= 0) edge_update_body<2, ST0, FUSE, LNS, WB, true>(A, 0, smem, lrow);
+        else edge_update_body<1, ST0, FUSE, LNS, WB, true>(A, 0, smem, lrow);
+        return;
+    }
     int pair = -1, single = -1;
     if (A.mix_mode == 2) {
         const int ns = gridDim.x - A.n_pairs;
@@ -1014,12 +1048,14 @@
 template <int R> static edge_kernel_t nm_kernel(bool st0) {
     return st0 ? k_node_message<R, true> : k_node_message<R, false>;
 }
-template <int R> static edge_kernel_t eu_kernel(bool st0, bool lns, bool wb) {
+template <int R> static edge_kernel_t eu_kernel(bool st0, bool lns, bool wb, bool live = false) {
+    if (live) return lns ? k_edge_update<R, false, PP_FUSED, true, false, true> : k_edge_update<R, false, PP_FUSED, false, false, true>;
     if (!wb && !st0) return lns ? k_edge_update<R, false, PP_FUSED, true, false> : k_edge_update<R, false, PP_FUSED, false, false>;
     if (lns) return st0 ? k_edge_update<R, true, PP_FUSED, true> : k_edge_update<R, false, PP_FUSED, true>;
     return st0 ? k_edge_update<R, true, PP_FUSED> : k_edge_update<R, false, PP_FUSED>;
 }
-static edge_kernel_t mix_kernel(bool st0, bool lns, bool wb) {
+static edge_kernel_t mix_kernel(bool st0, bool lns, bool wb, bool live = false) {
+    if (live) return lns ? k_edge_update_mix<false, PP_FUSED, true, false, true> : k_edge_update_mix<false, PP_FUSED, false, false, true>;
     if (!wb && !st0) return lns ? k_edge_update_mix<false, PP_FUSED, true, false> : k_edge_update_mix<false, PP_FUSED, false, false>;
     if (lns) return st0 ? k_edge_update_mix<true, PP_FUSED, true> : k_edge_update_mix<false, PP_FUSED, true>;
     return st0 ? k_edge_update_mix<true, PP_FUSED> : k_edge_update_mix<false, PP_FUSED>;
@@ -1028,8 +1064,8 @@
 static edge_kernel_t nm_kernel_r(int R, bool st0) {
     return R == 1 ? nm_kernel<1>(st0) : nm_kernel<2>(st0);
 }
-static edge_kernel_t eu_kernel_r(int R, bool st0, bool lns = false, bool wb = true) {
-    return R == 1 ? eu_kernel<1>(st0, lns, wb) : eu_kernel<2>(st0, lns, wb);
+static edge_kernel_t eu_kernel_r(int R, bool st0, bool lns = false, bool wb = true, bool live = false) {
+    return R == 1 ? eu_kernel<1>(st0, lns, wb, live) : eu_kernel<2>(st0, lns, wb, live);
 }
 
 
@@ -1049,6 +1085,10 @@
                      set(reinterpret_cast<const void *>(eu_kernel_r(R, st0, true, true)), MAX_SMEM) &&
                      set(reinterpret_cast<const void *>(eu_kernel_r(R, st0, false, false)), MAX_SMEM) &&
                      set(reinterpret_cast<const void *>(eu_kernel_r(R, st0, true, false)), MAX_SMEM);
+        for (int R = 1; R <= PP_RMAX && ok; R++)
+            for (int lns = 0; lns < 2 && ok; lns++)
+                ok = set(reinterpret_cast<const void *>(eu_kernel_r(R, false, lns, false, true)), MAX_SMEM);
+        for (int lns = 0; lns < 2 && ok; lns++) ok = set(reinterpret_cast<const void *>(mix_kernel(false, lns, false, true)), MAX_SMEM);
         for (int st0 = 0; st0 < 2 && ok; st0++)
             for (int lns = 0; lns < 2 && ok; lns++)
                 ok = set(reinterpret_cast<const void *>(mix_kernel(st0, lns, true)), MAX_SMEM) &&
@@ -1133,22 +1173,30 @@
 extern "C" int pp_edge_variant(void) { return 1; }
 bool pp_edge_fused() { return PP_FUSED; }
 
-pp_status pp_launch_edge_update(pp_ctx *c, int layer, bool keep_hE, hipStream_t s) {
+pp_status pp_launch_edge_update(pp_ctx *c, int layer, bool keep_hE, hipStream_t s, const PPLive *live) {
     EDGE_ATTR_CHECK()
     if (layer < 0 || layer > 1) { pp_set_error("pp_launch_edge_update: layer must be 0 or 1"); return PP_ERR_INVALID; }
+    if (live && (layer != 1 || keep_hE || !PP_FUSED)) { pp_set_error("pp_launch_edge_update: the live-row launch is layer 1's, without write-back"); return PP_ERR_INVALID; }
     EdgeArgs A = edge_args(c, layer, true);
     const int R = pick_R(c->N);
+    const bool mixed = use_mix(c->N);
+    if (live) {
+        if (mixed && !live->mix) { pp_set_error("pp_launch_edge_update: the mixed launch has no live-row work table for this context"); return PP_ERR_INVALID; }
+        if (mixed) A.live_mix = live->mix;
+        else A.live_rows = live->rows;
+    }
     const bool lns = c->plan->ln_scale != nullptr;
     if (lns && !PP_FUSED) { pp_set_error("pp_launch_edge_update: a plan with LayerNorm operand scales needs the fused build"); return PP_ERR_UNSUPPORTED; }
-    if (use_mix(c->N)) {
+    if (mixed) {
         A.n_pairs = (c->N + 2) / 3;
         A.mix_mode = g_mix;
         const int singles = c->N - 2 * A.n_pairs > 0 ? c->N - 2 * A.n_pairs : 0;
-        PP_LAUNCH(c, mix_kernel(layer == 0, lns, keep_hE), dim3(A.n_pairs + singles), dim3(ET), eu_smem(2) > eu_smem(1) ? eu_smem(2) : eu_smem(1), s, A);
+        const int wgs = live ? (c->N < 2 * g_num_cu ? c->N : 2 * g_num_cu) : A.n_pairs + singles;
+        PP_LAUNCH(c, mix_kernel(layer == 0, lns, keep_hE, live != nullptr), dim3(wgs), dim3(ET), eu_smem(2) > eu_smem(1) ? eu_smem(2) : eu_smem(1), s, A);
         PP_HIP_CHECK(hipGetLastError());
         return PP_OK;
     }
-    PP_LAUNCH(c, eu_kernel_r(R, layer == 0, lns, keep_hE), dim3((c->N + R - 1) / R), dim3(ET), eu_smem(R), s, A);
+    PP_LAUNCH(c, eu_kernel_r(R, layer == 0, lns, keep_hE, live != nullptr), dim3((c->N + R - 1) / R), dim3(ET), eu_smem(R), s, A);
     PP_HIP_CHECK(hipGetLastError());
     return PP_OK;
 }
diff --git a/packppi_amd/csrc/pp_internal.h b/packppi_amd/csrc/pp_internal.h
--- a/packppi_amd/csrc/pp_internal.h
+++ b/packppi_amd/csrc/pp_internal.h
@@ -92,6 +92,7 @@
     float *bounds_lower, *bounds_upper;
     float clash_tol;
     bool clash_params_set;
+    int num_cu = 0;
 };
 
 #define PP_PI_D 3.14159265358979323846
@@ -153,6 +154,10 @@
     pp_rng_row *rng_tab;
     uint64_t *rng_keys;
     bool rng_tab_set = false;
+    int32_t *live_rows[2];
+    int2 *live_mix[2];
+    int32_t *live_cnt[2];
+    bool live_mix_set[2] = {false, false};
     unsigned *sat;
     int prof_which = -1;
     bool prof_armed = false;
@@ -264,6 +269,12 @@
     int renoise;
 };
 
+struct PPLive {
+    const int32_t *rows;
+    const int2 *mix;
+};
+
+pp_status pp_launch_live_rows(pp_ctx *c, int set, const uint8_t *fixed, hipStream_t s);
 pp_status pp_launch_rng_table(pp_ctx *c, bool keys_set, hipStream_t s);
 pp_status pp_launch_noise_seeded(pp_ctx *c, uint64_t seed, int step, float *noise, uint32_t *words, hipStream_t s);
 pp_status pp_launch_add_noise_seeded(pp_ctx *c, const float *chi0, float sigma, uint64_t seed, float *chi, hipStream_t s);
@@ -281,7 +292,7 @@
 #endif
 pp_status pp_launch_node_message(pp_ctx *c, int layer, hipStream_t s);
 bool pp_edge_fused();
-pp_status pp_launch_edge_update(pp_ctx *c, int layer, bool keep_hE, hipStream_t s);
+pp_status pp_launch_edge_update(pp_ctx *c, int layer, bool keep_hE, hipStream_t s, const PPLive *live = nullptr);
 pp_status pp_launch_atom14(pp_ctx *c, const float *chi, float *xyz, hipStream_t s);
 pp_status pp_launch_clash(pp_ctx *c, const float *xyz, float *per_res, float *dchi, hipStream_t s, bool use_candidates = false);
 pp_status pp_launch_proximal(pp_ctx *c, const float *chi, float lamda, int nsteps, float *traj,
diff --git a/packppi_amd/csrc/pp_node.hip b/packppi_amd/csrc/pp_node.hip
--- a/packppi_amd/csrc/pp_node.hip
+++ b/packppi_amd/csrc/pp_node.hip
@@ -588,6 +588,12 @@
         publish4(sm.e_hi, sm.e_lo, erow * NU_S32 + 28, nf4{ev[3][2], ev[3][3], 0.f, 0.f});
     }
     publish4(sm.a_hi, sm.a_lo, srow * NU_S128 + scol, s4);
+    unsigned satrows = 0xffffu;
+    if constexpr (MODE == PP_NU_STEP) {
+        const unsigned long long bs = __ballot(scm1 != 0.f);
+        const unsigned long long br = __ballot(rm != 0.f && (!PINNED || fixraw == 0));
+        satrows = (unsigned)((bs | (bs >> 16) | (bs >> 32) | (bs >> 48)) & br & 0xffffull);
+    }
     __syncthreads();
 
     nh8 bh[4], bl[4];
@@ -609,7 +615,8 @@
     publish4(sm.c_hi, sm.c_lo, r * NU_S512 + 16 * (4 * wv + (c)) + 4 * g,                                  \
              relu_sat(fold(cH, cL) + *reinterpret_cast<const nf4 *>(par + NU_P_FIB + 16 * (4 * wv + (c)) + 4 * g), satm));
     FFN_IN_TILE(0) FFN_IN_TILE(1) FFN_IN_TILE(2) FFN_IN_TILE(3)
-    if (!(satm < 65504.f)) atomicOr(A.sat, 2u);
+    const bool satrow = (satrows >> r) & 1u;
+    if (!(satm < 65504.f) && satrow) atomicOr(A.sat, 2u);
     __syncthreads();
     nh8 fh[2], fl[2];
     ldB(sm.c_hi, sm.c_lo, r * NU_S512 + 8 * g, 0, fh[0], fl[0]);
@@ -700,7 +707,7 @@
             NSTAGE_IF(45, w0, cH, mm3(AK, dh[0], dl[0], cH, cL))
         }
         if (w0) {
-            if (!(satm < 65504.f)) atomicOr(A.sat, 2u);
+            if (!(satm < 65504.f) && satrow) atomicOr(A.sat, 2u);
             const nf4 sc = fold(cH, cL) + *reinterpret_cast<const nf4 *>(par + NU_P_DB3);
             if (g == 0 && live) *reinterpret_cast<nf4 *>(A.score + (size_t)n * 4) = sc;
             if constexpr (MODE == PP_NU_STEP) {
diff --git a/packppi_amd/csrc/pp_prepare.hip b/packppi_amd/csrc/pp_prepare.hip
--- a/packppi_amd/csrc/pp_prepare.hip
+++ b/packppi_amd/csrc/pp_prepare.hip
@@ -352,3 +352,53 @@
     return PP_OK;
 #endif
 }
+
+#define LIVE_THREADS 1024
+__global__ void __launch_bounds__(LIVE_THREADS)
+k_live_rows(const float *__restrict__ rmask, const float *__restrict__ scm, const uint8_t *__restrict__ fixed, int N,
+            int32_t *__restrict__ rows, int2 *__restrict__ mix, int32_t *__restrict__ cnt) {
+    __shared__ int part[LIVE_THREADS];
+    const int t = threadIdx.x;
+    const int per = (N + LIVE_THREADS - 1) / LIVE_THREADS;
+    const int lo = min(t * per, N), hi = min(lo + per, N);
+    auto is_live = [&](int i) {
+        const float *m = scm + (size_t)i * 4;
+        return rmask[i] != 0.f && (m[0] != 0.f || m[1] != 0.f || m[2] != 0.f || m[3] != 0.f) && !(fixed && fixed[i] != 0);
+    };
+    int c = 0;
+    for (int i = lo; i < hi; i++) c += is_live(i) ? 1 : 0;
+    part[t] = c;
+    __syncthreads();
+    for (int d = 1; d < LIVE_THREADS; d <<= 1) {
+        const int v = t >= d ? part[t - d] : 0;
+        __syncthreads();
+        part[t] += v;
+        __syncthreads();
+    }
+    const int M = part[LIVE_THREADS - 1];
+    int o = part[t] - c;
+    for (int i = lo; i < hi; i++)
+        if (is_live(i)) rows[o++] = i;
+    for (int i = M + t; i < N + 2; i += LIVE_THREADS) rows[i] = -1;
+    if (mix) {
+        const int np = (M + 2) / 3, ns = max(M - 2 * np, 0);
+        __syncthreads();
+        for (int b = t; b < N; b += LIVE_THREADS) {
+            int2 e = make_int2(-1, -1);
+            if (b < np) e = make_int2(rows[2 * b], rows[2 * b + 1]);
+            else if (b - np < ns) e.x = rows[2 * np + b - np];
+            mix[b] = e;
+        }
+    }
+    if (t == 0) cnt[0] = M;
+}
+
+pp_status pp_launch_live_rows(pp_ctx *c, int set, const uint8_t *fixed, hipStream_t s) {
+    const int num_cu = c->plan->num_cu;
+    const bool want_mix = c->N > 2 * num_cu && c->N <= 3 * num_cu;
+    hipLaunchKernelGGL(k_live_rows, dim3(1), dim3(LIVE_THREADS), 0, s, c->b.residue_mask, c->b.SC_D_mask, fixed, c->N,
+                       c->live_rows[set], want_mix ? c->live_mix[set] : nullptr, c->live_cnt[set]);
+    c->live_mix_set[set] = want_mix;
+    PP_HIP_CHECK(hipGetLastError());
+    return PP_OK;
+}
diff --git a/packppi_amd/lib.py b/packppi_amd/lib.py
--- a/packppi_amd/lib.py
+++ b/packppi_amd/lib.py
@@ -16,7 +16,7 @@
            "pp_affinity_create", "pp_affinity_destroy", "pp_affinity_encode", "pp_affinity_predict",
            "pp_score_rows", "pp_so2_set_grids", "pp_so2_score", "pp_dsm_loss",
            "pp_ctx_set_rng_keys", "pp_noise_seeded", "pp_add_noise_seeded", "pp_sample_seeded",
-           "pp_sample_partial", "pp_proximal_pinned")
+           "pp_sample_partial", "pp_proximal_pinned", "pp_ctx_live_rows")
 
 
 FIX_MODES = {"hold": 0, "renoise": 1}
@@ -113,6 +113,7 @@
     lib.pp_sample_seeded.argtypes = [vp, vp, vp, i, i, C.c_uint64, vp]
     lib.pp_sample_partial.argtypes = [vp, vp, vp, vp, i, vp, i, i, C.c_uint64, vp, vp]
     lib.pp_proximal_pinned.argtypes = [vp, vp, vp, f, i, vp, vp, vp, vp, vp, vp, vp]
+    lib.pp_ctx_live_rows.argtypes = [vp, vp, C.POINTER(C.c_int), vp]
     _lib = lib
     return lib
 
@@ -478,6 +479,11 @@
         _check(load().pp_ctx_saturated(self.handle, C.byref(v), _stream(self.plan.device)), "pp_ctx_saturated")
         return int(v.value)
 
+    def live_rows(self):
+        rows, n = self._new(self.n_rows, dtype=torch.int32), C.c_int(0)
+        _check(load().pp_ctx_live_rows(self.handle, _ptr(rows), C.byref(n), _stream(self.plan.device)), "pp_ctx_live_rows")
+        return rows[:int(n.value)]
+
     def time_kernel(self, which: int, iters: int = 20) -> float:
         ms = C.c_float(0.0)
         _check(load().pp_time_kernel(self.handle, int(which), int(iters), C.byref(ms), _stream(self.plan.device)),
```
